# danpovey/quantization

Measured on AMD Instinct MI355X. Metric: vectors encoded/sec at dim=512, 8 codebooks; uint8 codes bit-exact vs ref, higher is better.
Workload: dtype f32 (products: exact 30-bit fixed point on the i8 MFMA); 1 GPU; Quantizer.encode, dim=512, bytes_per_frame=8, codebook_size=256, refine_indexes_iters=5, batch=65536 fp32 Gaussian vectors per GPU (BASELINE.json configs[1]), seeded synthetic codebooks; global_batch=65536, parallelism=batch-sharded x1, no collective

## Files before the change

include/mcq.h:

```cpp
#ifndef MCQ_H
#define MCQ_H

#include <stddef.h>
#include <stdint.h>

#ifdef __cplusplus
extern "C" {
#endif

#define MCQ_EINVAL (-1)
#define MCQ_EUNSUPPORTED (-2)
#define MCQ_EWORKSPACE (-3)

#define MCQ_ABI_VERSION 7
int mcq_abi_version(void);

int mcq_padded_dim(int D);

size_t mcq_prepared_bytes(int N, int K, int D);
size_t mcq_prepared_decode_bytes(int N, int K, int D);
size_t mcq_prepared_mean_offset(int N, int K, int D);
int mcq_prepare(const float *centers, float cscale_exp, const float *weight, const float *bias,
                int N, int K, int D, void *prepared, void *stream);

int mcq_prepare_dev(const float *centers, const float *scales_exp, const float *weight, const float *bias,
                    int N, int K, int D, void *prepared, void *stream);

int mcq_prepare_params(const float *centers, const float *centers_scale, const float *logits_scale, float speed,
                       const float *weight, const float *bias, int N, int K, int D, void *prepared,
                       float *scales_exp_out, void *stream);

size_t mcq_encode_workspace_bytes(long B, int N, int K, int D);
int mcq_encode(const float *x, long B, const void *prepared, float lscale_exp, int N, int K, int D,
               int refine_iters, uint8_t *out_u8, int64_t *out_i64, void *workspace,
               size_t workspace_bytes, void *stream);

#define MCQ_ENCODE_SKIP_FIXED_POINTS 1u
#define MCQ_ENCODE_LSCALE_FROM_PREPARED 2u
#define MCQ_ENCODE_X_FP16 4u
int mcq_encode_ex(const float *x, long B, const void *prepared, float lscale_exp, int N, int K, int D,
                  int refine_iters, uint8_t *out_u8, int64_t *out_i64, void *workspace,
                  size_t workspace_bytes, void *stream, unsigned flags);

int mcq_refine_indexes(const float *x, long B, const void *prepared, int N, int K, int D, int refine_iters,
                       const int64_t *idx_in, int64_t *idx_out, void *workspace, size_t workspace_bytes,
                       void *stream);

int mcq_decode(const void *codes, int code_bytes, int codes_per_row, long B, const void *prepared,
               int N, int K, int D, float *out, void *stream);

int mcq_decode_backward(const float *grad_out, const int64_t *idx, long B, int N, int K, int D, float *gC,
                        void *stream);

int mcq_logits_argmax(const float *x, long B, const void *prepared, float lscale_exp, int N, int K, int D,
                      float *logits_out, int64_t *argmax_out, void *workspace, size_t workspace_bytes,
                      void *stream, unsigned flags);

int mcq_logits_refine(const float *x, long B, const void *prepared, float lscale_exp, int N, int K, int D,
                      int refine_iters, float *logits_out, int64_t *idx_out, void *workspace, size_t workspace_bytes,
                      void *stream, unsigned flags);
int mcq_logits_refine_codes(const float *x, long B, const void *prepared, float lscale_exp, int N, int K, int D,
                            int refine_iters, float *logits_out, int64_t *idx_out, uint8_t *codes_out, void *workspace,
                            size_t workspace_bytes, void *stream, unsigned flags);

size_t mcq_loss_workspace_bytes(long B, int N, int K);
int mcq_loss_fwd(const float *logits, const int64_t *idx, long B, int N, int K, float *lse, float *chosen_sum,
                 float *prob_sum, float *count, void *workspace, size_t workspace_bytes, void *stream);

int mcq_loss_bwd(const float *logits, const int64_t *idx, const float *lse, long B, int N, int K,
                 const float *g_chosen, const float *g_prob, float *grad_logits, void *stream);

int mcq_loss_tail(const float *sums, const float *prob_sum, const float *count, int N, int K, float entropy_scale,
                  float *losses, float *g, float *g_prob, void *stream);

int mcq_recon_fwd(const float *x, const int64_t *idx, long B, const void *prepared, const float *mean, int N,
                  int K, int D, float *err, float *num_part, float *den_part, void *stream);


size_t mcq_weight_grad_workspace_bytes(long B, int M, int D);
int mcq_weight_grad(const float *G, const float *x, long B, int M, int D, const float *scale_dev, float *gW, float *gb,
                    void *workspace, size_t workspace_bytes, void *stream);
int mcq_adam_step(float *p, const float *g, float *m, float *v, long n, double lr, double beta1, double beta2, double eps,
                  double weight_decay, double bias_correction1, double bias_correction2_sqrt, void *stream);
int mcq_loss_head(const float *num_part, const float *den_part, long nparts, const float *chosen_n, int N, float batch,
                  float *head, void *stream);
int mcq_scales_exp(const float *centers_scale, const float *logits_scale, float speed, float *out2, void *stream);
int mcq_loss_head_tail(const float *num_part, const float *den_part, long nparts, const float *chosen_n, int N, float batch,
                       float *head, const float *prob_sum, const float *count, int K, float entropy_scale, float *losses,
                       float *g, float *g_prob, void *stream);

long mcq_decode_backward_waves(int N, int K, int D);
int mcq_decode_backward_u8_ex(const float *grad_out, const uint8_t *codes, long B, int N, int K, int D, float *gC,
                              const float *sa, const float *sb, float sc, const float *dotw, float *dot_part, void *stream);
long mcq_loss_bwd_waves(long B, int N, int K);
int mcq_loss_bwd_ex(const float *logits, const int64_t *idx, const float *lse, long B, int N, int K, const float *g_chosen,
                    const float *g_prob, float *grad_logits, const float *bias, float *dot_part, void *stream);
int mcq_grad_tail(const float *part_c, long n_c, const float *sa, const float *sb, float sc, const float *part_l, long n_l,
                  float speed, float *out_c, float *out_l, void *stream);

int mcq_jcl_prefix_fwd(const float *hp, const float *emb, const int64_t *idx, long B, int N, int K, int H,
                       float scale, float *A, void *stream);
int mcq_jcl_prefix_bwd(const float *A, const float *gA, long B, int N, int H, float scale, float *g_hp, float *gE,
                       void *stream);
int mcq_scatter_rows(const float *grad, long stride_b, long stride_n, const int64_t *idx, int idx_stride, long B,
                     int N, int K, int D, float *out, void *stream);

int mcq_decode_backward_u8(const float *grad_out, const uint8_t *codes, long B, int N, int K, int D, float *gC,
                           void *stream);

size_t mcq_logits_workspace_bytes(long B, int N, int D);
int mcq_logits(const float *x, long B, const void *prepared, float lscale_exp, int N, int K, int D,
               float *out, void *workspace, size_t workspace_bytes, void *stream);

int mcq_test_select(const float *scores, int cases, int per_lane, int cnt, float *out_v, int *out_p, void *stream);

int mcq_last_encode_launches(void);

int mcq_profile_encode(const float *x, long B, const void *prepared, float lscale_exp, int N, int K,
                       int D, int refine_iters, void *workspace, size_t workspace_bytes, void *stream,
                       float *ms_out, int *launches_out, int cap);
// ... 7 lines not shown
```

quantization_amd/_lib.py:

```python
import ctypes
import os

_HERE = os.path.dirname(os.path.abspath(__file__))
_ALT = os.environ.get("MCQ_LIB_PATH") if os.environ.get("MCQ_ALLOW_LIB_PATH") == "1" else None
LIB_PATH = _ALT or os.path.join(_HERE, "lib", "libmcq_hip.so")

SYMBOLS = (
    "mcq_abi_version", "mcq_padded_dim", "mcq_prepared_bytes", "mcq_prepared_decode_bytes", "mcq_prepared_mean_offset", "mcq_prepare", "mcq_prepare_dev", "mcq_prepare_params", "mcq_encode_workspace_bytes",
    "mcq_encode", "mcq_encode_ex", "mcq_refine_indexes", "mcq_decode", "mcq_decode_backward", "mcq_logits", "mcq_logits_workspace_bytes", "mcq_last_encode_launches", "mcq_test_select", "mcq_profile_encode", "mcq_profile_category_name",
    "mcq_logits_argmax", "mcq_logits_refine", "mcq_logits_refine_codes", "mcq_loss_workspace_bytes", "mcq_loss_fwd", "mcq_loss_bwd", "mcq_recon_fwd", "mcq_loss_tail",
    "mcq_jcl_prefix_fwd", "mcq_jcl_prefix_bwd", "mcq_scatter_rows", "mcq_decode_backward_u8",
    "mcq_weight_grad", "mcq_weight_grad_workspace_bytes", "mcq_adam_step", "mcq_loss_head", "mcq_loss_head_tail", "mcq_scales_exp",
    "mcq_decode_backward_waves", "mcq_decode_backward_u8_ex", "mcq_loss_bwd_waves", "mcq_loss_bwd_ex", "mcq_grad_tail",
)

MCQ_EINVAL, MCQ_EUNSUPPORTED, MCQ_EWORKSPACE = -1, -2, -3
_lib = None


class McqError(RuntimeError):
    pass


def lib():
    global _lib
    if _lib is not None:
        return _lib
    if not os.path.exists(LIB_PATH):
        raise McqError(f"{LIB_PATH} is missing: build it with `python -c 'import __graft_entry__ as g; g.build()'` "
                       "(hipcc --offload-arch=gfx950); quantization_amd has no CPU fallback")
    L = ctypes.CDLL(LIB_PATH)
    vp, f32, i32, i64, sz = ctypes.c_void_p, ctypes.c_float, ctypes.c_int, ctypes.c_long, ctypes.c_size_t
    L.mcq_abi_version.restype = i32
    L.mcq_padded_dim.restype = i32
    L.mcq_padded_dim.argtypes = [i32]
    L.mcq_prepared_bytes.restype = sz
    L.mcq_prepared_bytes.argtypes = [i32, i32, i32]
    L.mcq_prepared_decode_bytes.restype = sz
    L.mcq_prepared_decode_bytes.argtypes = [i32, i32, i32]
    L.mcq_prepare.restype = i32
    L.mcq_prepare.argtypes = [vp, f32, vp, vp, i32, i32, i32, vp, vp]
    L.mcq_prepare_dev.restype = i32
    L.mcq_prepare_dev.argtypes = [vp, vp, vp, vp, i32, i32, i32, vp, vp]
    L.mcq_prepare_params.restype = i32
    L.mcq_prepare_params.argtypes = [vp, vp, vp, f32, vp, vp, i32, i32, i32, vp, vp, vp]
    L.mcq_prepared_mean_offset.restype = sz
    L.mcq_prepared_mean_offset.argtypes = [i32, i32, i32]
    L.mcq_encode_workspace_bytes.restype = sz
    L.mcq_encode_workspace_bytes.argtypes = [i64, i32, i32, i32]
    L.mcq_encode.restype = i32
    L.mcq_encode.argtypes = [vp, i64, vp, f32, i32, i32, i32, i32, vp, vp, vp, sz, vp]
    L.mcq_encode_ex.restype = i32
    L.mcq_encode_ex.argtypes = [vp, i64, vp, f32, i32, i32, i32, i32, vp, vp, vp, sz, vp, ctypes.c_uint]
    L.mcq_refine_indexes.restype = i32
    L.mcq_refine_indexes.argtypes = [vp, i64, vp, i32, i32, i32, i32, vp, vp, vp, sz, vp]
    L.mcq_decode.restype = i32
    L.mcq_decode.argtypes = [vp, i32, i32, i64, vp, i32, i32, i32, vp, vp]
    L.mcq_decode_backward.restype = i32
    L.mcq_decode_backward.argtypes = [vp, vp, i64, i32, i32, i32, vp, vp]
    L.mcq_logits.restype = i32
    L.mcq_logits.argtypes = [vp, i64, vp, f32, i32, i32, i32, vp, vp, sz, vp]
    L.mcq_test_select.restype = i32
    L.mcq_test_select.argtypes = [vp, i32, i32, i32, vp, vp, vp]
    L.mcq_logits_workspace_bytes.restype = sz
    L.mcq_logits_workspace_bytes.argtypes = [i64, i32, i32]
    L.mcq_logits_argmax.restype = i32
    L.mcq_logits_argmax.argtypes = [vp, i64, vp, f32, i32, i32, i32, vp, vp, vp, sz, vp, ctypes.c_uint]
    L.mcq_logits_refine.restype = i32
    L.mcq_logits_refine.argtypes = [vp, i64, vp, f32, i32, i32, i32, i32, vp, vp, vp, sz, vp, ctypes.c_uint]
    L.mcq_logits_refine_codes.restype = i32
    L.mcq_logits_refine_codes.argtypes = [vp, i64, vp, f32, i32, i32, i32, i32, vp, vp, vp, vp, sz, vp, ctypes.c_uint]
    L.mcq_loss_workspace_bytes.restype = sz
    L.mcq_loss_workspace_bytes.argtypes = [i64, i32, i32]
    L.mcq_loss_fwd.restype = i32
    L.mcq_loss_fwd.argtypes = [vp, vp, i64, i32, i32, vp, vp, vp, vp, vp, sz, vp]
    L.mcq_loss_bwd.restype = i32
    L.mcq_loss_bwd.argtypes = [vp, vp, vp, i64, i32, i32, vp, vp, vp, vp]
    L.mcq_loss_tail.restype = i32
    L.mcq_loss_tail.argtypes = [vp, vp, vp, i32, i32, f32, vp, vp, vp, vp]
    L.mcq_recon_fwd.restype = i32
    L.mcq_recon_fwd.argtypes = [vp, vp, i64, vp, vp, i32, i32, i32, vp, vp, vp, vp]
    L.mcq_jcl_prefix_fwd.restype = i32
    L.mcq_jcl_prefix_fwd.argtypes = [vp, vp, vp, i64, i32, i32, i32, f32, vp, vp]
    L.mcq_jcl_prefix_bwd.restype = i32
    L.mcq_jcl_prefix_bwd.argtypes = [vp, vp, i64, i32, i32, f32, vp, vp, vp]
    L.mcq_decode_backward_u8.restype = i32
    L.mcq_decode_backward_u8.argtypes = [vp, vp, i64, i32, i32, i32, vp, vp]
    L.mcq_scatter_rows.restype = i32
    L.mcq_scatter_rows.argtypes = [vp, i64, i64, vp, i32, i64, i32, i32, i32, vp, vp]
    L.mcq_weight_grad.restype = i32
    L.mcq_weight_grad.argtypes = [vp, vp, i64, i32, i32, vp, vp, vp, vp, sz, vp]
    L.mcq_weight_grad_workspace_bytes.restype = sz
    L.mcq_weight_grad_workspace_bytes.argtypes = [i64, i32, i32]
    f64 = ctypes.c_double
    L.mcq_adam_step.restype = i32
    L.mcq_adam_step.argtypes = [vp, vp, vp, vp, i64, f64, f64, f64, f64, f64, f64, f64, vp]
    L.mcq_loss_head.restype = i32
    L.mcq_loss_head.argtypes = [vp, vp, i64, vp, i32, f32, vp, vp]
    L.mcq_loss_head_tail.restype = i32
# ... 30 lines not shown
```

quantization_amd/csrc/mcq_api.hip:

```cpp
#include "../../include/mcq.h"
#include "mcq_kernels.h"
#include "mcq_fix_kernels.h"
#include "mcq_loss_kernels.h"
#include "mcq_tf_kernels.h"
#include "mcq_pass16_kernels.h"
#include "mcq_train_kernels.h"

#include <cstdlib>
#include <vector>

using namespace mcq;

namespace {

inline int round_up16(int d) { return (d + 15) & ~15; }
inline size_t align256(size_t v) { return (v + 255) & ~size_t(255); }
inline bool is_pow2(int v) { return v > 0 && (v & (v - 1)) == 0; }

int k_cutoff(int K, int L) {
    int kc = (K <= 16) ? 8 : 16;
    while (L >= 4) { L /= 4; kc *= 2; }
    return kc < 128 ? kc : 128;
}

struct Prepared {
    const float *C, *Q, *bias, *scales, *G, *mean, *wmu;
    const int8_t *Cf, *Wf;
    const int *Ce, *We;
};

struct PreparedLayout {
    size_t offC, offQ, offCf, offCe, offWf, offWe, offWmu, offBias, offScales, offMean, offCMean, offG, total;
};

PreparedLayout prepared_layout(int N, int K, int D) {
    const size_t nk = (size_t)N * K, Dp = round_up16(D);
    const size_t planes = fix_plane_bytes((long)nk, D), exps = (size_t)fix_round_rows((long)nk) * 4;
    PreparedLayout l;
    l.offC = 0;
    l.offQ = align256(l.offC + nk * Dp * 4);
    l.offCf = align256(l.offQ + nk * 4);
    l.offCe = align256(l.offCf + planes);
    l.offWf = align256(l.offCe + exps);
    l.offWe = align256(l.offWf + planes);
    l.offWmu = align256(l.offWe + exps);
    l.offBias = align256(l.offWmu + nk * 4);
    l.offScales = align256(l.offBias + nk * 4);
    l.offMean = align256(l.offScales + 8);
    l.offCMean = align256(l.offMean + Dp * 4);
    l.offG = align256(l.offCMean + (size_t)N * Dp * 4);
    l.total = align256(l.offG + nk * nk * 4);
    static_assert(kFixTile == 128, "");
    if (l.total < l.offBias + (nk + kFixTile) * 4) l.total = align256(l.offBias + (nk + kFixTile) * 4);
    return l;
}

Prepared prepared_view(const void *p, int N, int K, int D) {
    const PreparedLayout l = prepared_layout(N, K, D);
    const char *b = static_cast<const char *>(p);
    return Prepared{reinterpret_cast<const float *>(b + l.offC), reinterpret_cast<const float *>(b + l.offQ),
                    reinterpret_cast<const float *>(b + l.offBias), reinterpret_cast<const float *>(b + l.offScales),
                    reinterpret_cast<const float *>(b + l.offG), reinterpret_cast<const float *>(b + l.offMean),
                    reinterpret_cast<const float *>(b + l.offWmu),
                    reinterpret_cast<const int8_t *>(b + l.offCf), reinterpret_cast<const int8_t *>(b + l.offWf),
                    reinterpret_cast<const int *>(b + l.offCe), reinterpret_cast<const int *>(b + l.offWe)};
}

template <typename CT>
struct WorkspaceT {
    CT *idx, *idxB, *idxC, *final_idx;
    int *map[2], *cnt;
    float *E, *R, *xx, *XC;
    float *gterms;
    int8_t *xf;
    int *xe;
    float *tabs[2];
    TfLists tf;
};

int tf_levels(int N) { int v = 0; while ((1 << v) < N) ++v; return v; }

size_t tf_tab_floats(int N, int K) {
    const int nlev = tf_levels(N);
    size_t best = 0;
    for (int v = 2; v < nlev; ++v) {
        const size_t groups = (size_t)N >> (v + 1);
        for (int u = 1; u < v; ++u) {
            const size_t per = (size_t)1 << (v - u), kc = k_cutoff(K, 1 << u);
            const size_t f = groups * per * per * kc * kc;
            best = f > best ? f : best;
        }
    }
    return best;
}

inline size_t code_bytes_of(int K) { return K > 256 ? 2 : 1; }

size_t workspace_per_vector(int N, int K, int D) {
    const size_t cb = code_bytes_of(K);
    return 4 * cb * (size_t)N + 8 + 8 + 4 * (size_t)N + 4 * (size_t)N * K + (size_t)tf_levels(N) * N * (16 * cb + 2 * 16 + 4 * 16) + 64 +
           2 * 4 * tf_tab_floats(N, K) + 4 * (size_t)fix_round_cols(D) + 4 + 4 * (size_t)N * N;
}
size_t workspace_slack(int D) { return 48 * 256 + (size_t)kFixTile * (4 * (size_t)fix_round_cols(D) + 4); }

long default_chunk(int N, int K, int D) {
    long c = (long)(((size_t)2 << 30) / workspace_per_vector(N, K, D));
    c = c > 65536 ? 65536 : c;
    c = c < 1024 ? 1024 : c;
    return c & ~127L;
}

template <typename CT>
WorkspaceT<CT> carve(void *ws, long Bc, int N, int K, int D) {
    char *p = static_cast<char *>(ws);
    size_t off = 0;
    auto take = [&](size_t bytes) { char *q = p + off; off = align256(off + bytes); return q; };
    WorkspaceT<CT> w;
    w.idx = reinterpret_cast<CT *>(take((size_t)Bc * N * sizeof(CT)));
    w.idxB = reinterpret_cast<CT *>(take((size_t)Bc * N * sizeof(CT)));
    w.idxC = reinterpret_cast<CT *>(take((size_t)Bc * N * sizeof(CT)));
    w.final_idx = reinterpret_cast<CT *>(take((size_t)Bc * N * sizeof(CT)));
    for (int i = 0; i < 2; ++i) w.map[i] = reinterpret_cast<int *>(take((size_t)Bc * 4));
    w.cnt = reinterpret_cast<int *>(take(64 * 4));
    w.E = reinterpret_cast<float *>(take((size_t)Bc * 4));
    w.R = reinterpret_cast<float *>(take((size_t)Bc * N * 4));
    w.xx = reinterpret_cast<float *>(take((size_t)Bc * 4));
    w.gterms = reinterpret_cast<float *>(take((size_t)Bc * N * N * 4));
    w.XC = reinterpret_cast<float *>(take((size_t)Bc * N * K * 4));
    w.xf = reinterpret_cast<int8_t *>(take(fix_plane_bytes(Bc, D)));
    w.xe = reinterpret_cast<int *>(take((size_t)fix_round_rows(Bc) * 4));
    const int nlev = tf_levels(N);
    w.tf.ent = nullptr;
    w.tf.out_i64 = nullptr;
    w.tf.out_u8 = nullptr;
    w.tf.erG = w.tf.erXC = w.tf.erxx = nullptr;
    w.tf.erE = w.tf.erR = nullptr;
    w.tf.erK = 0;
    for (int v = 0; v < kTfLevels; ++v) {
        w.tf.kc[v] = k_cutoff(K, 1 << v);
        w.tf.pos[v] = nullptr;
        w.tf.S[v] = nullptr;
        if (v >= nlev) continue;
        const int kc = w.tf.kc[v];
        if (v == 0) w.tf.ent = reinterpret_cast<uint8_t *>(take((size_t)Bc * N * kc * sizeof(CT)));
        else w.tf.pos[v] = reinterpret_cast<uint8_t *>(take((size_t)Bc * (N >> v) * kc * 2));
        w.tf.S[v] = reinterpret_cast<float *>(take((size_t)Bc * (N >> v) * kc * 4));
    }
    const size_t tf = tf_tab_floats(N, K);
    for (int i = 0; i < 2; ++i) w.tabs[i] = tf ? reinterpret_cast<float *>(take((size_t)Bc * tf * 4)) : nullptr;
    return w;
}

bool domain_ok(int N, int K, int D) {
    return is_pow2(K) && K >= 16 && K <= 1024 && is_pow2(N) && N <= 64 && (long)N * K <= 16384 && D >= 1 && D <= 16384;
}
int domain_err(int N, int K, int D = 1) {
    return (K < 16 || K > 1024 || N > 64 || (long)N * K > 16384 || D > 16384) ? MCQ_EUNSUPPORTED : MCQ_EINVAL;
}

struct Prof {
    hipStream_t stream;
    int only = -1;
    std::vector<hipEvent_t> ev;
    std::vector<int> cat, first, last;
    int open = -1;
    void begin(int category) {
        if (only >= 0 && category != only) { open = -1; return; }
        if (ev.empty() || open != (int)ev.size() - 1) {
            hipEvent_t e;
            (void)hipEventCreate(&e);
            (void)hipEventRecord(e, stream);
            ev.push_back(e);
        }
        open = (int)ev.size() - 1;
    }
    void untimed() { open = -1; }
    void end(int category) {
        if (only >= 0 && category != only) { open = -1; return; }
        hipEvent_t e;
        (void)hipEventCreate(&e);
        (void)hipEventRecord(e, stream);
        ev.push_back(e);
        first.push_back(open);
        last.push_back((int)ev.size() - 1);
        cat.push_back(category);
        open = (int)ev.size() - 1;
    }
};

thread_local int g_last_launches = 0;

#define MCQ_LAUNCH_CHECK()                               \
    do {                                                 \
        hipError_t e_ = hipGetLastError();               \
        if (e_ != hipSuccess) return (int)e_;            \
        ++g_last_launches;                               \
    } while (0)

FixRowsArgs fix_rows_args(const float *src, int xh, long R, int D, long ld, int8_t *planes, int *exps, float *xx,
                          const float *bias_src = nullptr, float *bias_dst = nullptr, const float *sub = nullptr,
                          long sub_per = 0, long sub_ld = 0, const float *dot_vec = nullptr, float *dot_out = nullptr) {
    return FixRowsArgs{src, xh, R, fix_round_rows(R), D, ld, fix_round_cols(D), planes, exps, xx, bias_src, bias_dst,
                       sub, sub_per, sub_ld, dot_vec, dot_out};
}

int launch_fix_rows(const float *src, int xh, long R, int D, long ld, int8_t *planes, int *exps, float *xx, hipStream_t st,
                    const float *sub = nullptr) {
    const FixRowsArgs a = fix_rows_args(src, xh, R, D, ld, planes, exps, xx, nullptr, nullptr, sub, 0, 0);
    hipLaunchKernelGGL(k_fix_rows<4>, dim3((unsigned)(a.Rp / 4)), dim3(256), 0, st, a);
    MCQ_LAUNCH_CHECK();
    return 0;
}

int launch_fix_rows2(const FixRowsArgs &a, const FixRowsArgs &b, hipStream_t st) {
    const unsigned na = (unsigned)(a.Rp / 4), nb = (unsigned)(b.Rp / 4);
    hipLaunchKernelGGL(k_fix_rows2<4>, dim3(na + nb), dim3(256), 0, st, a, b, na);
    MCQ_LAUNCH_CHECK();
    return 0;
}

template <int MODE>
int launch_fgemm(FixGemm g, hipStream_t st) {
    static bool allowed[64] = {};
    int dev = 0;
    if (hipGetDevice(&dev) != hipSuccess || dev < 0 || dev >= 64) dev = 63;
    if (!allowed[dev] || dev == 63) {
        const hipError_t attr = hipFuncSetAttribute(reinterpret_cast<const void *>(&k_fgemm<MODE>),
                                                    hipFuncAttributeMaxDynamicSharedMemorySize, kFixLds);
        if (attr != hipSuccess) return (int)attr;
        allowed[dev] = true;
    }
    const long MT = g.RA / kFixTile, NT = g.RB / kFixTile;
    const int H = (MODE == FG_LOGITS && g.K > kFixTile) ? g.K / kFixTile : 1;
    const long big = g.walk_rows ? NT : MT, small_units = (g.walk_rows ? MT : NT) / H;
    long units = (big + 7) / 8 * small_units;
    if (units > 32) units = 32;
    hipLaunchKernelGGL((k_fgemm<MODE>), dim3((unsigned)(8 * units)), dim3(512), kFixLds, st, g);
    MCQ_LAUNCH_CHECK();
    return 0;
}

int launch_xc(const int8_t *xf, const int *xe, long B, const int8_t *Cf, const int *Ce, long nk, int D, float *out,
              hipStream_t st) {
    FixGemm g{};
    g.A = xf; g.ea = xe; g.RA = fix_round_rows(B); g.M = B;
    g.B = Cf; g.eb = Ce; g.RB = fix_round_rows(nk); g.N = nk;
    g.Dq = fix_round_cols(D);
    g.walk_rows = 0;
    g.out = out; g.ldo = nk;
    return launch_fgemm<FG_STORE>(g, st);
}

int launch_logits(const int8_t *xf, const int *xe, long B, const Prepared &P, int N, int K, int D, float lscale,
                  const float *lscale_ptr, float *logits, void *idx, hipStream_t st) {
    const long nk = (long)N * K;
    FixGemm g{};
    g.A = P.Wf; g.ea = P.We; g.RA = fix_round_rows(nk); g.M = nk;
    g.B = xf; g.eb = xe; g.RB = fix_round_rows(B); g.N = B;
    g.Dq = fix_round_cols(D);
    g.walk_rows = 1;
    g.bias = P.bias; g.wmu = P.wmu; g.lscale = lscale; g.lscale_ptr = lscale_ptr;
    g.logits = logits; g.ldo = nk; g.idx = idx; g.idx_wide = K > 256 ? 1 : 0; g.K = K; g.ncb = N;
    return launch_fgemm<FG_LOGITS>(g, st);
}

template <int K>
int launch_tf_stage0_k(int N, const float *G, const float *XC, const tf_code_of<K> *idx, const float *R, const float *Q, long B,
                       int keep, tf_code_of<K> *ent, float *S, tf_code_of<K> *fin, const int *nact, const int *map, hipStream_t st) {
    const dim3 grid((unsigned)(((B + 3) / 4) * N)), block(256);
#define MCQ_S0_CASE(NN) \
    case NN: hipLaunchKernelGGL((k_tf_stage0<K, NN>), grid, block, 0, st, G, XC, idx, R, Q, B, keep, ent, S, fin, nact, map); break;
    switch (N) {
        MCQ_S0_CASE(1) MCQ_S0_CASE(2) MCQ_S0_CASE(4) MCQ_S0_CASE(8) MCQ_S0_CASE(16) MCQ_S0_CASE(32) MCQ_S0_CASE(64)
        default: return MCQ_EUNSUPPORTED;
    }
#undef MCQ_S0_CASE
    MCQ_LAUNCH_CHECK();
    return 0;
}

int launch_tf_stage0(int K, int N, const float *G, const float *XC, const uint16_t *idx, const float *R, const float *Q,
                     long B, int keep, uint16_t *ent, float *S, uint16_t *fin, const int *nact, const int *map, hipStream_t st) {
    switch (K) {
        case 512: return launch_tf_stage0_k<512>(N, G, XC, idx, R, Q, B, keep, ent, S, fin, nact, map, st);
        case 1024: return launch_tf_stage0_k<1024>(N, G, XC, idx, R, Q, B, keep, ent, S, fin, nact, map, st);
        default: return MCQ_EUNSUPPORTED;
    }
}

int launch_tf_stage0(int K, int N, const float *G, const float *XC, const uint8_t *idx, const float *R, const float *Q,
                     long B, int keep, uint8_t *ent, float *S, uint8_t *fin, const int *nact, const int *map, hipStream_t st) {
    if (K == 16 && N >= 4 && keep <= 16) {
        const dim3 grid((unsigned)((B * (N / 4) + 3) / 4)), block(256);
#define MCQ_S16_CASE(NN) \
    case NN: hipLaunchKernelGGL((k_tf_stage0_k16<NN>), grid, block, 0, st, G, XC, idx, R, Q, B, keep, ent, S, nact, map); break;
        switch (N) {
            MCQ_S16_CASE(4) MCQ_S16_CASE(8) MCQ_S16_CASE(16) MCQ_S16_CASE(32) MCQ_S16_CASE(64)
            default: return MCQ_EUNSUPPORTED;
        }
#undef MCQ_S16_CASE
        MCQ_LAUNCH_CHECK();
        return 0;
    }
    switch (K) {
        case 16: return launch_tf_stage0_k<16>(N, G, XC, idx, R, Q, B, keep, ent, S, fin, nact, map, st);
        case 32: return launch_tf_stage0_k<32>(N, G, XC, idx, R, Q, B, keep, ent, S, fin, nact, map, st);
        case 64: return launch_tf_stage0_k<64>(N, G, XC, idx, R, Q, B, keep, ent, S, fin, nact, map, st);
        case 128: return launch_tf_stage0_k<128>(N, G, XC, idx, R, Q, B, keep, ent, S, fin, nact, map, st);
        case 256: return launch_tf_stage0_k<256>(N, G, XC, idx, R, Q, B, keep, ent, S, fin, nact, map, st);
        default: return MCQ_EUNSUPPORTED;
    }
}

template <typename CT>
int launch_tf_er(int N, const float *G, const float *XC, const CT *idx, const float *xx, long B, int K, float *E, float *R,
                 float *gterms, const int *nact, const int *map, hipStream_t st) {
    const dim3 grid((unsigned)((B + 3) / 4)), block(256);
    const bool direct = B <= 8192;
#define MCQ_ER_CASE(NN)                                                                                                  \
    case NN:                                                                                                             \
        if (!direct) {                                                                                                   \
            hipLaunchKernelGGL((k_tf_gram_terms<NN, CT>), dim3((unsigned)(((B + 4 * (64 / NN) - 1) / (4 * (64 / NN))) * NN)), block, 0, st, G, idx, \
                               B, K, gterms, nact);                                                                      \
            MCQ_LAUNCH_CHECK();                                                                                          \
        }                                                                                                                \
        hipLaunchKernelGGL((k_tf_er<NN, CT>), grid, block, 0, st, gterms, XC, idx, xx, B, K, E, R, nact, map,              \
                           direct ? G : static_cast<const float *>(nullptr));                                           \
        break;
    switch (N) {
        MCQ_ER_CASE(1) MCQ_ER_CASE(2) MCQ_ER_CASE(4) MCQ_ER_CASE(8) MCQ_ER_CASE(16) MCQ_ER_CASE(32) MCQ_ER_CASE(64)
        default: return MCQ_EUNSUPPORTED;
    }
#undef MCQ_ER_CASE
    MCQ_LAUNCH_CHECK();
    return 0;
}

int launch_tf_up(int kh, int kc, const TfLists &L, long B, int N, int u, int ntab, int per, const float *in, float *out,
                 const int *nact, hipStream_t st) {
    const dim3 grid((unsigned)(B * ntab)), block(64);
#define MCQ_UP_CASE(A, C) \
    if (kh == A && kc == C) { hipLaunchKernelGGL((k_tf_up<A, C>), grid, block, 0, st, L, B, N, u, ntab, per, in, out, nact); MCQ_LAUNCH_CHECK(); return 0; }
    MCQ_UP_CASE(16, 32) MCQ_UP_CASE(32, 32) MCQ_UP_CASE(32, 64) MCQ_UP_CASE(8, 16) MCQ_UP_CASE(16, 16)
#undef MCQ_UP_CASE
    return MCQ_EUNSUPPORTED;
}

template <typename CT>
int launch_tf_comb(int kh, int kc, const float *E, const TfLists &L, long B, int N, int v, int keep, const float *tabs,
                   CT *fin, const int *nact, hipStream_t st) {
    const dim3 grid((unsigned)(B * (N >> (v + 1)))), block(64);
#define MCQ_COMB_CASE(A, C)                                                                                                        \
    if (kh == A && kc == C) {                                                                                                     \
        if (fin) hipLaunchKernelGGL((k_tf_comb<A, C, true, CT>), grid, block, 0, st, E, L, B, N, v, keep, tabs, fin, nact);       \
        else hipLaunchKernelGGL((k_tf_comb<A, C, false, CT>), grid, block, 0, st, E, L, B, N, v, keep, tabs, fin, nact);          \
        MCQ_LAUNCH_CHECK();                                                                                                       \
        return 0;                                                                                                                 \
    }
    MCQ_COMB_CASE(16, 32) MCQ_COMB_CASE(32, 32) MCQ_COMB_CASE(32, 64) MCQ_COMB_CASE(64, 64)
    if constexpr (sizeof(CT) == 1) { MCQ_COMB_CASE(8, 16) MCQ_COMB_CASE(16, 16) }
#undef MCQ_COMB_CASE
    return MCQ_EUNSUPPORTED;
}

enum { CAT_LOGITS = 0, CAT_XX = 1, CAT_STAGE0 = 2, CAT_XC = 3, CAT_LEVEL0 = 4, CAT_LEVEL1 = 5, CAT_TABLES = 6, CAT_COMBINE = 7,
       CAT_TABLES_UP = 8, CAT_COMBINE_UP = 9, CAT_ER = 10, CAT_LEVEL1_FUSED = 11, CAT_TAIL = 12, CAT_COUNT = 13 };
const char *const kCatNames[CAT_COUNT] = {
    "logits_product_argmax",
    "frames_to_limbs",
    "stage0_tables",
    "xc_product",
    "combine_level0",
    "combine_level1",
    "tables_level1",
    "combine_level2",
    "tables_upper_levels",
    "combine_upper_levels",
    "residual_energies",
    "level1_combines_and_tables",
    "encode_tail",
};

#define MCQ_TF_LAUNCH2(SMALLK, BIGK, grid, block, ...)                                                       \
    do {                                                                                                     \
        bool s_ = false;                                                                                     \
        if constexpr (sizeof(CT) == 1) {                                                                     \
            if (small) { hipLaunchKernelGGL(SMALLK, grid, block, 0, st, __VA_ARGS__); s_ = true; }           \
        }                                                                                                    \
        if (!s_) hipLaunchKernelGGL(BIGK, grid, block, 0, st, __VA_ARGS__);                                  \
    } while (0)
inline bool pass16_enabled() {
    static const bool on = !(getenv("MCQ_PASS16") && atoi(getenv("MCQ_PASS16")) == 0);
    return on;
}

template <typename CT>
int run_tf_combines(const float *G, const CT *idx_cur, CT *idx_new, const WorkspaceT<CT> &w, const TfLists &L, long B, int N,
                    int K, const int *nact, hipStream_t st, Prof *prof) {
    const bool small = (K == 16);
    const int nlev = tf_levels(N);
    {
        const int keep = (N == 2) ? 1 : L.kc[1];
        CT *fin = (N == 2) ? idx_new : nullptr;
        const dim3 grid((unsigned)(B * (N / 2)));
        if (prof) prof->begin(CAT_LEVEL0);
        bool done0 = false;
        if constexpr (sizeof(CT) == 1) {
            if (!small) {
                hipLaunchKernelGGL(k_tf_pair0s, grid, dim3(64), 0, st, G, idx_cur, w.E, L, B, N, K, keep, fin, nact);
                done0 = true;
            }
        }
        if (!done0) MCQ_TF_LAUNCH2((k_tf_pair0<8, CT>), (k_tf_pair0<16, CT>), grid, dim3(64), G, idx_cur, w.E, L, B, N, K, keep, fin, nact);
        MCQ_LAUNCH_CHECK();
        if (prof) prof->end(CAT_LEVEL0);
    }
    const bool fuse_l1 = (N >= 8);
    const bool fuse_l3 = fuse_l1 && N == 16 && small;
    if (fuse_l1) {
        const int keep = L.kc[2];
        const int groups2 = N >> 3, per1 = 2, ntab1 = groups2 * per1 * per1;
        const unsigned pair_blocks = (unsigned)(B * (N / 4)), tab_blocks = (unsigned)(B * ntab1);
        const int ntab3 = fuse_l3 ? 16 : 1, per3 = fuse_l3 ? 4 : 1;
        const dim3 grid(pair_blocks + tab_blocks + (fuse_l3 ? (unsigned)(B * ntab3) : 0u));
        if (prof) prof->begin(CAT_LEVEL1_FUSED);
        MCQ_TF_LAUNCH2((k_tf_level1<8, 8, CT>), (k_tf_level1<16, 16, CT>), grid, dim3(64), G, idx_cur, w.E, L, B, N, K, keep, ntab1, per1, w.tabs[0],
                       nact, pair_blocks, tab_blocks, ntab3, per3, w.tabs[1]);
        MCQ_LAUNCH_CHECK();
        if (prof) prof->end(CAT_LEVEL1_FUSED);
    } else if (N >= 4) {
        const int keep = (N == 4) ? 1 : L.kc[2];
        CT *fin = (N == 4) ? idx_new : nullptr;
        const dim3 grid((unsigned)(B * (N / 4)));
        if (prof) prof->begin(CAT_LEVEL1);
        MCQ_TF_LAUNCH2((k_tf_pair1<8, 8, CT>), (k_tf_pair1<16, 16, CT>), grid, dim3(64), G, idx_cur, w.E, L, B, N, K, keep, fin, nact);
        MCQ_LAUNCH_CHECK();
        if (prof) prof->end(CAT_LEVEL1);
    }
    for (int v = 2; v < nlev; ++v) {
        const int groups = N >> (v + 1);
        const bool last = (v == nlev - 1);
        const int keep = last ? 1 : L.kc[v + 1];
        CT *fin = last ? idx_new : nullptr;
        const int per1 = 1 << (v - 1), ntab1 = groups * per1 * per1;
        const int cat_tab = (v == 2) ? CAT_TABLES : CAT_TABLES_UP, cat_comb = (v == 2) ? CAT_COMBINE : CAT_COMBINE_UP;
        if (!(fuse_l1 && v == 2) && !(fuse_l3 && v == 3)) {
            if (prof) prof->begin(cat_tab);
            MCQ_TF_LAUNCH2((k_tf_table1<8, 8, CT>), (k_tf_table1<16, 16, CT>), dim3((unsigned)(B * ntab1)), dim3(64), G, idx_cur, L, B, N, K, ntab1, per1,
                           w.tabs[0], nact);
            MCQ_LAUNCH_CHECK();
            if (prof) prof->end(cat_tab);
        }
        if (N == 16 && v == 3) {
            if (prof) prof->begin(cat_comb);
            const float *t3 = fuse_l3 ? w.tabs[1] : w.tabs[0];
            MCQ_TF_LAUNCH2((k_tf_comb3<8, 16, 16, CT>), (k_tf_comb3<16, 32, 32, CT>), dim3((unsigned)B), dim3(256), idx_cur, w.E, L, B, N, t3, idx_new, nact);
            MCQ_LAUNCH_CHECK();
            if (prof) prof->end(cat_comb);
            continue;
        }
        int cur = 0;
        for (int u = 2; u < v; ++u) {
            const int per = 1 << (v - u), ntab = groups * per * per;
            if (prof) prof->begin(cat_tab);
            const int rc = launch_tf_up(L.kc[u - 1], L.kc[u], L, B, N, u, ntab, per, w.tabs[cur], w.tabs[cur ^ 1], nact, st);
            if (rc) return rc;
            if (prof) prof->end(cat_tab);
            cur ^= 1;
        }
        if (prof) prof->begin(cat_comb);
        const int rc = launch_tf_comb<CT>(L.kc[v - 1], L.kc[v], w.E, L, B, N, v, keep, w.tabs[cur], fin, nact, st);
        if (rc) return rc;
        if (prof) prof->end(cat_comb);
    }
    return 0;
}
#undef MCQ_TF_LAUNCH2

template <typename CT>
int run_encode_t(const float *x, long B, const void *prepared, float lscale, int N, int K, int D, int iters,
                 uint8_t *out_u8, int64_t *out_i64, void *workspace, size_t workspace_bytes, hipStream_t st,
                 Prof *prof, const int64_t *init_idx, unsigned flags, float *logits_out,
                 uint8_t *codes_also ) {
    g_last_launches = 0;
    if (!domain_ok(N, K, D)) return domain_err(N, K, D);
    if (B < 0 || iters < 0 || iters > 60 || (out_u8 == nullptr) == (out_i64 == nullptr)) return MCQ_EINVAL;
    if (sizeof(CT) > 1 && (out_u8 != nullptr || codes_also != nullptr)) return MCQ_EINVAL;
    if (B == 0) return 0;
    if (!x || !prepared || !workspace) return MCQ_EINVAL;
    const size_t per = workspace_per_vector(N, K, D), slack = workspace_slack(D);
    if (workspace_bytes < slack + per) return MCQ_EWORKSPACE;
    long chunk = (long)((workspace_bytes - slack) / per);
    if (chunk > B) chunk = B;
    if (chunk < B && chunk < 128) return MCQ_EWORKSPACE;
    if (chunk < B) chunk &= ~127L;
    const Prepared P = prepared_view(prepared, N, K, D);
    const int pack = (out_u8 != nullptr && K == 16 && N >= 2) ? 2 : 1;
    const bool skip = (flags & MCQ_ENCODE_SKIP_FIXED_POINTS) != 0 && iters >= 2;

    for (long lo = 0; lo < B; lo += chunk) {
        const long Bc = (B - lo < chunk) ? (B - lo) : chunk;
        const WorkspaceT<CT> w = carve<CT>(workspace, Bc, N, K, D);
        const int xh = (flags & MCQ_ENCODE_X_FP16) ? 1 : 0;
        const float *xc = xh ? reinterpret_cast<const float *>(reinterpret_cast<const uint16_t *>(x) + lo * D) : x + lo * D;
        int rc;
        if (init_idx == nullptr || iters > 0) {
            if (prof) prof->begin(CAT_XX);
            rc = launch_fix_rows(xc, xh, Bc, D, D, w.xf, w.xe, w.xx, st, P.mean);
            if (rc) return rc;
            if (prof) prof->end(CAT_XX);
        }
        if (init_idx != nullptr) {
            hipLaunchKernelGGL(k_import_indexes<CT>, dim3((unsigned)((Bc * N + 255) / 256)), dim3(256), 0, st,
                               init_idx + lo * N, Bc * N, K, w.idx);
            MCQ_LAUNCH_CHECK();
            if (prof) prof->untimed();
        } else {
            if (prof) prof->begin(CAT_LOGITS);
            rc = launch_logits(w.xf, w.xe, Bc, P, N, K, D, lscale,
                               (flags & MCQ_ENCODE_LSCALE_FROM_PREPARED) ? P.scales + 1 : nullptr,
                               logits_out ? logits_out + lo * N * K : nullptr, w.idx, st);
            if (rc) return rc;
            if (prof) prof->end(CAT_LOGITS);
        }
        if (iters > 0) {
            if (prof) prof->begin(CAT_XC);
            rc = launch_xc(w.xf, w.xe, Bc, P.Cf, P.Ce, (long)N * K, D, w.XC, st);
            if (rc) return rc;
            if (prof) prof->end(CAT_XC);
        }
        int iters_left = iters;
        CT *idx_cur = w.idx, *idx_new = skip ? w.idxB : w.idx, *idx_pk = w.idxC;
        const int *map_cur = nullptr, *nact = nullptr;
        int *map_nxt = w.map[0], *map_spare = w.map[1];
        if (skip) {
            hipError_t e = hipMemsetAsync(w.cnt, 0, 64 * sizeof(int), st);
            if (e != hipSuccess) return (int)e;
            if (prof) prof->untimed();
        }
        bool wrote_direct = false;
        if constexpr (sizeof(CT) == 1) {
            if (K == 16 && (N == 16 || N == 8) && iters > 0 && !skip && prof == nullptr && pass16_enabled()) {
                static bool allowed16[64] = {};
                int dev = 0;
                if (hipGetDevice(&dev) != hipSuccess || dev < 0 || dev >= 64) dev = 63;
                if (!allowed16[dev] || dev == 63) {
                    hipError_t attr = hipFuncSetAttribute(reinterpret_cast<const void *>(&k_tf_pass16<16>),
                                                          hipFuncAttributeMaxDynamicSharedMemorySize, p16_lds_bytes<16>());
                    if (attr == hipSuccess)
                        attr = hipFuncSetAttribute(reinterpret_cast<const void *>(&k_tf_pass16<8>),
                                                   hipFuncAttributeMaxDynamicSharedMemorySize, p16_lds_bytes<8>());
                    if (attr != hipSuccess) return (int)attr;
                    allowed16[dev] = true;
                }
                Pass16Args a;
                a.G = P.G; a.XC = w.XC; a.xx = w.xx; a.Q = P.Q; a.idx = w.idx; a.B = Bc; a.iters = iters;
                const bool direct_out = pack == 1;
                a.out_i64 = (direct_out && out_i64) ? out_i64 + lo * N : nullptr;
                a.out_u8 = direct_out ? (out_u8 ? out_u8 + lo * N : (codes_also ? codes_also + lo * N : nullptr)) : nullptr;
                const long wgs = (Bc + kP16Waves - 1) / kP16Waves;
                if (N == 16)
                    hipLaunchKernelGGL(k_tf_pass16<16>, dim3((unsigned)(wgs < 256 ? wgs : 256)), dim3(64 * kP16Waves), p16_lds_bytes<16>(), st, a);
                else
                    hipLaunchKernelGGL(k_tf_pass16<8>, dim3((unsigned)(wgs < 512 ? wgs : 512)), dim3(64 * kP16Waves), p16_lds_bytes<8>(), st, a);
                MCQ_LAUNCH_CHECK();
                if (direct_out) continue;
                iters_left = 0;
            }
        }
        const bool er_in_emit = !skip && (N == 4 || N == 8 || N == 16);
        bool er_ready = false;
        for (int it = 0; it < iters_left; ++it) {
            if (!er_ready) {
                if (prof) prof->begin(CAT_ER);
                rc = launch_tf_er<CT>(N, P.G, w.XC, idx_cur, w.xx, Bc, K, w.E, w.R, w.gterms, nact, map_cur, st);
                if (rc) return rc;
                if (prof) prof->end(CAT_ER);
            }
            er_ready = false;
            if (prof) prof->begin(CAT_STAGE0);
            rc = launch_tf_stage0(K, N, P.G, w.XC, idx_cur, w.R, P.Q, Bc, (N == 1) ? 1 : w.tf.kc[0], reinterpret_cast<CT *>(w.tf.ent),
                                  w.tf.S[0], (N == 1) ? idx_new : static_cast<CT *>(nullptr), nact, map_cur, st);
            if (rc) return rc;
            if (prof) prof->end(CAT_STAGE0);
            if (N >= 2) {
                TfLists L = w.tf;
                if (er_in_emit && it + 1 < iters) {
                    L.erG = P.G; L.erXC = w.XC; L.erxx = w.xx; L.erE = w.E; L.erR = w.R; L.erK = K;
                    er_ready = true;
                }
                const bool direct_out = (it + 1 == iters) && !skip && pack == 1;
                if (direct_out) {
                    L.out_i64 = out_i64 ? out_i64 + lo * N : nullptr;
                    L.out_u8 = out_u8 ? out_u8 + lo * N : (codes_also ? codes_also + lo * N : nullptr);
                    wrote_direct = true;
                }
                rc = run_tf_combines<CT>(P.G, idx_cur, idx_new, w, L, Bc, N, K, nact, st, prof);
                if (rc) return rc;
            }
            if (skip) {
                const int last = (it + 1 == iters) ? 1 : 0;
                if (prof) prof->begin(CAT_TAIL);
                hipLaunchKernelGGL(k_compact<CT>, dim3((unsigned)((Bc + 255) / 256)), dim3(256), 0, st, idx_cur, idx_new,
                                   map_cur, nact, Bc, N, last, w.final_idx, idx_pk, map_nxt, w.cnt + it);
                MCQ_LAUNCH_CHECK();
                if (prof) prof->end(CAT_TAIL);
                CT *t = idx_cur; idx_cur = idx_pk; idx_pk = t;
                int *old_map = const_cast<int *>(map_cur);
                map_cur = map_nxt;
                map_nxt = old_map ? old_map : map_spare;
                nact = w.cnt + it;
            }
        }
        if (wrote_direct) continue;
        const CT *result = (skip && iters > 0) ? w.final_idx : w.idx;
        const long outn = (out_i64 != nullptr) ? Bc * N : Bc * (N / pack);
        if (prof) prof->begin(CAT_TAIL);
        hipLaunchKernelGGL(k_finalize<CT>, dim3((unsigned)((outn + 255) / 256)), dim3(256), 0, st, result, Bc, N, pack,
                           out_u8 ? out_u8 + lo * (N / pack) : nullptr, out_i64 ? out_i64 + lo * N : nullptr,
                           codes_also ? codes_also + lo * N : nullptr);
        MCQ_LAUNCH_CHECK();
        if (prof) prof->end(CAT_TAIL);
    }
    return 0;
}

int run_encode(const float *x, long B, const void *prepared, float lscale, int N, int K, int D, int iters,
               uint8_t *out_u8, int64_t *out_i64, void *workspace, size_t workspace_bytes, hipStream_t st,
               Prof *prof, const int64_t *init_idx = nullptr, unsigned flags = 0, float *logits_out = nullptr,
               uint8_t *codes_also = nullptr) {
    if (K > 256)
        return run_encode_t<uint16_t>(x, B, prepared, lscale, N, K, D, iters, out_u8, out_i64, workspace, workspace_bytes, st, prof,
                                      init_idx, flags, logits_out, codes_also);
    return run_encode_t<uint8_t>(x, B, prepared, lscale, N, K, D, iters, out_u8, out_i64, workspace, workspace_bytes, st, prof,
                                 init_idx, flags, logits_out, codes_also);
}

int db_cw_of(int D, int K) {
    if ((D & 3) != 0) return 1;
    if (K >= 64) return 4;
    return D >= 1024 ? 4 : (D >= 512 ? 2 : 1);
}
int db_cw(const void *g, const void *out, int D, int K, long gsb, long gsn, const void *dotw = nullptr) {
    const bool al = ((D & 3) == 0) && ((gsb & 3) == 0) && ((gsn & 3) == 0) && ((reinterpret_cast<uintptr_t>(g) & 15) == 0) &&
                    ((reinterpret_cast<uintptr_t>(out) & 15) == 0) && ((reinterpret_cast<uintptr_t>(dotw) & 15) == 0);
    return al ? db_cw_of(D, K) : 1;
}
int db_chunks(int D, int cw) { return (D + 64 * cw - 1) / (64 * cw); }

template <typename IdxT>
int launch_decode_backward(const float *g, const IdxT *idx, long B, int N, int K, int D, float *out, long gsb, long gsn,
                           int idx_stride, hipStream_t st, const float *sa = nullptr, const float *sb = nullptr, float sc = 1.0f,
                           const float *dotw = nullptr, float *dot_part = nullptr) {
    const int cw = db_cw(g, out, D, K, gsb, gsn, dotw), chunks = db_chunks(D, cw);
    const long rowgroups = ((long)N * K + 3) / 4;
    long blocks;
    if (chunks <= 8 && (8 % chunks) == 0) blocks = ((rowgroups + (8 / chunks) - 1) / (8 / chunks)) * 8;
    else blocks = ((long)N * K * chunks + 3) / 4;
    const dim3 grid((unsigned)blocks), block(256);
    if (cw == 4) hipLaunchKernelGGL((k_decode_backward<IdxT, 4>), grid, block, 0, st, g, idx, B, N, K, D, chunks, out, gsb, gsn, idx_stride, sa, sb, sc, dotw, dot_part);
    else if (cw == 2) hipLaunchKernelGGL((k_decode_backward<IdxT, 2>), grid, block, 0, st, g, idx, B, N, K, D, chunks, out, gsb, gsn, idx_stride, sa, sb, sc, dotw, dot_part);
    else hipLaunchKernelGGL((k_decode_backward<IdxT, 1>), grid, block, 0, st, g, idx, B, N, K, D, chunks, out, gsb, gsn, idx_stride, sa, sb, sc, dotw, dot_part);
    hipError_t e = hipGetLastError();
    return e == hipSuccess ? 0 : (int)e;
}
}

extern "C" {

int mcq_abi_version(void) { return MCQ_ABI_VERSION; }

int mcq_padded_dim(int D) { return round_up16(D); }

size_t mcq_prepared_bytes(int N, int K, int D) {
    if (N <= 0 || K <= 0 || D <= 0) return 0;
    return prepared_layout(N, K, D).total;
}

static int prepare_impl(const float *centers, float cscale_exp, const float *scales_dev, const float *weight,
                        const float *bias, int N, int K, int D, void *prepared, void *stream, const float *raw_cs = nullptr,
                        const float *raw_ls = nullptr, float speed = 0.f, float *scales_out2 = nullptr) {
    if (!domain_ok(N, K, D)) return domain_err(N, K, D);
    if (!centers || !prepared || ((weight == nullptr) != (bias == nullptr))) return MCQ_EINVAL;
    hipStream_t st = static_cast<hipStream_t>(stream);
    const PreparedLayout l = prepared_layout(N, K, D);
    char *b = static_cast<char *>(prepared);
    const long rows = (long)N * K;
    const int Dp = round_up16(D);
    const unsigned grid = (unsigned)((rows + 3) / 4);
    hipLaunchKernelGGL(k_prepare_rows, dim3(grid), dim3(256), 0, st, centers, cscale_exp, 1, rows, D, Dp,
                       reinterpret_cast<float *>(b + l.offC), static_cast<float *>(nullptr) , scales_dev,
                       (scales_dev || raw_cs) ? reinterpret_cast<float *>(b + l.offScales) : static_cast<float *>(nullptr), raw_cs,
                       raw_ls, speed, scales_out2);
    hipError_t e = hipGetLastError();
    if (e != hipSuccess) return (int)e;
    if (!weight) return 0;
    const float *C = reinterpret_cast<const float *>(b + l.offC);
    float *cmean = reinterpret_cast<float *>(b + l.offCMean);
    hipLaunchKernelGGL(k_centers_mean, dim3((unsigned)(Dp / 16)), dim3(1024), 0, st, C, N, K, Dp,
                       reinterpret_cast<float *>(b + l.offMean), cmean);
    e = hipGetLastError();
// ... 232 lines not shown
    if (B == 0) return 0;
    if (!A || !gA || !g_hp || !gE) return MCQ_EINVAL;
    hipLaunchKernelGGL(k_jcl_prefix_bwd, dim3((unsigned)((B + 3) / 4)), dim3(256), 0, static_cast<hipStream_t>(stream), A,
                       gA, B, N, H, scale, g_hp, gE);
    hipError_t e = hipGetLastError();
    return e == hipSuccess ? 0 : (int)e;
}

namespace {
struct LogitsWs {
    uint8_t *idx8;
    int8_t *xf;
    int *xe;
    size_t total;
};
LogitsWs logits_ws(void *ws, long B, int N, int D) {
    char *p = static_cast<char *>(ws);
    LogitsWs w;
    size_t off = 0;
    w.idx8 = reinterpret_cast<uint8_t *>(p + off);
    off = align256(off + (size_t)B * N);
    w.xf = reinterpret_cast<int8_t *>(p + off);
    off = align256(off + fix_plane_bytes(B, D));
    w.xe = reinterpret_cast<int *>(p + off);
    off = align256(off + (size_t)fix_round_rows(B) * 4);
    w.total = off;
    return w;
}
}

size_t mcq_logits_workspace_bytes(long B, int N, int D) {
    if (B <= 0 || N <= 0 || D <= 0) return 256;
    return logits_ws(nullptr, B, N, D).total;
}

int mcq_logits(const float *x, long B, const void *prepared, float lscale_exp, int N, int K, int D, float *out,
               void *workspace, size_t workspace_bytes, void *stream) {
    if (!domain_ok(N, K, D)) return MCQ_EUNSUPPORTED;
    if (B == 0) return 0;
    if (!x || !prepared || !out || B < 0 || !workspace) return MCQ_EINVAL;
    if (workspace_bytes < mcq_logits_workspace_bytes(B, N, D)) return MCQ_EWORKSPACE;
    hipStream_t st = static_cast<hipStream_t>(stream);
    const Prepared P = prepared_view(prepared, N, K, D);
    const LogitsWs w = logits_ws(workspace, B, N, D);
    int rc = launch_fix_rows(x, 0, B, D, D, w.xf, w.xe, nullptr, st, P.mean);
    if (rc) return rc;
    return launch_logits(w.xf, w.xe, B, P, N, K, D, lscale_exp, nullptr, out, nullptr, st);
}

int mcq_logits_argmax(const float *x, long B, const void *prepared, float lscale_exp, int N, int K, int D,
                      float *logits_out, int64_t *argmax_out, void *workspace, size_t workspace_bytes, void *stream,
                      unsigned flags) {
    if (!domain_ok(N, K, D) || K > 256) return MCQ_EUNSUPPORTED;
    if (B < 0) return MCQ_EINVAL;
    if (B == 0) return 0;
    if (!x || !prepared || !logits_out || !argmax_out || !workspace) return MCQ_EINVAL;
    if (workspace_bytes < mcq_logits_workspace_bytes(B, N, D)) return MCQ_EWORKSPACE;
    hipStream_t st = static_cast<hipStream_t>(stream);
    const Prepared P = prepared_view(prepared, N, K, D);
    const LogitsWs w = logits_ws(workspace, B, N, D);
    int rc = launch_fix_rows(x, (flags & MCQ_ENCODE_X_FP16) ? 1 : 0, B, D, D, w.xf, w.xe, nullptr, st, P.mean);
    if (rc) return rc;
    rc = launch_logits(w.xf, w.xe, B, P, N, K, D, lscale_exp,
                       (flags & MCQ_ENCODE_LSCALE_FROM_PREPARED) ? P.scales + 1 : nullptr, logits_out, w.idx8, st);
    if (rc) return rc;
    hipLaunchKernelGGL(k_export_indexes, dim3((unsigned)((B * N + 255) / 256)), dim3(256), 0, st, w.idx8, B * N, argmax_out);
    MCQ_LAUNCH_CHECK();
    return 0;
}

int mcq_logits_refine(const float *x, long B, const void *prepared, float lscale_exp, int N, int K, int D, int refine_iters,
                      float *logits_out, int64_t *idx_out, void *workspace, size_t workspace_bytes, void *stream,
                      unsigned flags) {
    return mcq_logits_refine_codes(x, B, prepared, lscale_exp, N, K, D, refine_iters, logits_out, idx_out, nullptr, workspace,
                                   workspace_bytes, stream, flags);
}

int mcq_logits_refine_codes(const float *x, long B, const void *prepared, float lscale_exp, int N, int K, int D, int refine_iters,
                            float *logits_out, int64_t *idx_out, uint8_t *codes_out, void *workspace, size_t workspace_bytes,
                            void *stream, unsigned flags) {
    if (K > 256) return MCQ_EUNSUPPORTED;
    if (B > 0 && (!logits_out || !idx_out)) return MCQ_EINVAL;
    return run_encode(x, B, prepared, lscale_exp, N, K, D, refine_iters, nullptr, idx_out, workspace, workspace_bytes,
                      static_cast<hipStream_t>(stream), nullptr, nullptr, flags & ~MCQ_ENCODE_SKIP_FIXED_POINTS, logits_out,
                      codes_out);
}

namespace {
long loss_rows_per_chunk(long B) {
    long r = (B + 1023) / 1024;
    r = r < 64 ? 64 : r;
    return (r + 15) / 16 * 16;
}
long loss_chunks(long B) { const long r = loss_rows_per_chunk(B); return (B + r - 1) / r; }
}

size_t mcq_loss_workspace_bytes(long B, int N, int K) {
    if (B <= 0) return 256;
    return (size_t)loss_chunks(B) * N * (2 * (size_t)K + 1) * sizeof(float) + 256;
}

int mcq_loss_fwd(const float *logits, const int64_t *idx, long B, int N, int K, float *lse, float *chosen_sum,
                 float *prob_sum, float *count, void *workspace, size_t workspace_bytes, void *stream) {
    if (!is_pow2(K) || K < 16 || K > 256 || N < 1) return MCQ_EUNSUPPORTED;
    if (B <= 0) return MCQ_EINVAL;
    if (!logits || !idx || !lse || !chosen_sum || !prob_sum || !count || !workspace) return MCQ_EINVAL;
    if (workspace_bytes < mcq_loss_workspace_bytes(B, N, K)) return MCQ_EWORKSPACE;
    hipStream_t st = static_cast<hipStream_t>(stream);
    const long rpc = loss_rows_per_chunk(B), chunks = loss_chunks(B);
    float *pp = static_cast<float *>(workspace);
    float *pc = pp + chunks * N * K;
    float *ph = pc + chunks * N * K;
    const dim3 grid((unsigned)(chunks * N)), block(64 * kLossWaves);
#define MCQ_LOSS_CASE(KK)                                                                                             \
    case KK: hipLaunchKernelGGL((k_loss_fwd<KK>), grid, block, 0, st, logits, idx, B, N, rpc, lse, pp, pc, ph); break;
    switch (K) {
        MCQ_LOSS_CASE(16) MCQ_LOSS_CASE(32) MCQ_LOSS_CASE(64) MCQ_LOSS_CASE(128) MCQ_LOSS_CASE(256)
        default: return MCQ_EUNSUPPORTED;
    }
#undef MCQ_LOSS_CASE
    MCQ_LAUNCH_CHECK();
    hipLaunchKernelGGL(k_loss_reduce, dim3((unsigned)N), dim3(256), 0, st, pp, pc, ph, chunks, N, K, prob_sum, count,
                       chosen_sum);
    MCQ_LAUNCH_CHECK();
    return 0;
}

int mcq_loss_bwd(const float *logits, const int64_t *idx, const float *lse, long B, int N, int K, const float *g_chosen,
                 const float *g_prob, float *grad_logits, void *stream) {
    if (!is_pow2(K) || K < 16 || K > 256 || N < 1) return MCQ_EUNSUPPORTED;
    if (B <= 0) return MCQ_EINVAL;
    if (!logits || !idx || !lse || !g_chosen || !g_prob || !grad_logits) return MCQ_EINVAL;
    hipStream_t st = static_cast<hipStream_t>(stream);
    const int rpw = K < 64 ? 64 / K : 1;
    const long rows = B * N;
    const dim3 grid((unsigned)((rows + (long)kLossWaves * rpw - 1) / ((long)kLossWaves * rpw))), block(64 * kLossWaves);
#define MCQ_LOSS_CASE(KK)                                                                                             \
    case KK: hipLaunchKernelGGL((k_loss_bwd<KK>), grid, block, 0, st, logits, idx, lse, B, N, g_chosen, g_prob, grad_logits); break;
    switch (K) {
        MCQ_LOSS_CASE(16) MCQ_LOSS_CASE(32) MCQ_LOSS_CASE(64) MCQ_LOSS_CASE(128) MCQ_LOSS_CASE(256)
        default: return MCQ_EUNSUPPORTED;
    }
#undef MCQ_LOSS_CASE
    MCQ_LAUNCH_CHECK();
    return 0;
}

int mcq_loss_tail(const float *sums, const float *prob_sum, const float *count, int N, int K, float entropy_scale,
                  float *losses, float *g, float *g_prob, void *stream) {
    if (!is_pow2(K) || K < 16 || K > 256 || N < 1) return MCQ_EUNSUPPORTED;
    if (!sums || !prob_sum || !count || !losses || !g || !g_prob) return MCQ_EINVAL;
    hipLaunchKernelGGL(k_loss_tail, dim3(1), dim3(256), 0, static_cast<hipStream_t>(stream), sums, prob_sum, count, N, K,
                       entropy_scale, losses, g, g_prob);
    MCQ_LAUNCH_CHECK();
    return 0;
}

int mcq_recon_fwd(const float *x, const int64_t *idx, long B, const void *prepared, const float *mean, int N, int K,
                  int D, float *err, float *num_part, float *den_part, void *stream) {
    if (!domain_ok(N, K, D) || K > 256) return MCQ_EUNSUPPORTED;
    if (B <= 0) return MCQ_EINVAL;
    if (!x || !idx || !prepared || !mean || !err || !num_part || !den_part) return MCQ_EINVAL;
    const Prepared P = prepared_view(prepared, N, K, D);
    hipLaunchKernelGGL(k_recon_fwd, dim3((unsigned)((B + 3) / 4)), dim3(256), 0, static_cast<hipStream_t>(stream), x, idx, B,
                       P.C, mean, N, K, D, round_up16(D), err, num_part, den_part);
    MCQ_LAUNCH_CHECK();
    return 0;
// ... 117 lines not shown
int mcq_loss_bwd_ex(const float *logits, const int64_t *idx, const float *lse, long B, int N, int K, const float *g_chosen,
                    const float *g_prob, float *grad_logits, const float *bias, float *dot_part, void *stream) {
    if (!is_pow2(K) || K < 16 || K > 256 || N < 1) return MCQ_EUNSUPPORTED;
    if (B <= 0) return MCQ_EINVAL;
    if (!logits || !idx || !lse || !g_chosen || !g_prob || !grad_logits || !bias || !dot_part) return MCQ_EINVAL;
    hipStream_t st = static_cast<hipStream_t>(stream);
    const int rpw = K < 64 ? 64 / K : 1;
    const long rows = B * N;
    const dim3 grid((unsigned)((rows + (long)kLossWaves * rpw - 1) / ((long)kLossWaves * rpw))), block(64 * kLossWaves);
#define MCQ_LOSS_CASE(KK)                                                                                             \
    case KK: hipLaunchKernelGGL((k_loss_bwd<KK>), grid, block, 0, st, logits, idx, lse, B, N, g_chosen, g_prob, grad_logits, bias, dot_part); break;
    switch (K) {
        MCQ_LOSS_CASE(16) MCQ_LOSS_CASE(32) MCQ_LOSS_CASE(64) MCQ_LOSS_CASE(128) MCQ_LOSS_CASE(256)
        default: return MCQ_EUNSUPPORTED;
    }
#undef MCQ_LOSS_CASE
    MCQ_LAUNCH_CHECK();
    return 0;
}

int mcq_grad_tail(const float *part_c, long n_c, const float *sa, const float *sb, float sc, const float *part_l, long n_l,
                  float speed, float *out_c, float *out_l, void *stream) {
    if (n_c < 0 || n_l < 0 || (n_c > 0 && !part_c) || (n_l > 0 && !part_l)) return MCQ_EINVAL;
    hipLaunchKernelGGL(k_grad_tail, dim3(1), dim3(1024), 0, static_cast<hipStream_t>(stream), part_c, n_c, sa, sb, sc, part_l, n_l,
                       speed, out_c, out_l);
    MCQ_LAUNCH_CHECK();
    return 0;
}

int mcq_last_encode_launches(void) { return g_last_launches; }

int mcq_test_select(const float *scores, int cases, int per_lane, int cnt, float *out_v, int *out_p, void *stream) {
    if (!scores || !out_v || !out_p || cases <= 0 || cnt < 1 || cnt > 64) return MCQ_EINVAL;
    hipStream_t st = static_cast<hipStream_t>(stream);
    switch (per_lane) {
        case 1: hipLaunchKernelGGL((k_test_select<1>), dim3(cases), dim3(64), 0, st, scores, cnt, out_v, out_p); break;
        case 4: hipLaunchKernelGGL((k_test_select<4>), dim3(cases), dim3(64), 0, st, scores, cnt, out_v, out_p); break;
        case 16: hipLaunchKernelGGL((k_test_select<16>), dim3(cases), dim3(64), 0, st, scores, cnt, out_v, out_p); break;
        case -4: hipLaunchKernelGGL((k_test_select<4, kSlotMajor>), dim3(cases), dim3(64), 0, st, scores, cnt, out_v, out_p); break;
        case -16: hipLaunchKernelGGL((k_test_select<16, kSlotMajor>), dim3(cases), dim3(64), 0, st, scores, cnt, out_v, out_p); break;
        case -1004: hipLaunchKernelGGL((k_test_select<4, kAnyOrder>), dim3(cases), dim3(64), 0, st, scores, cnt, out_v, out_p); break;
        default: return MCQ_EINVAL;
    }
    hipError_t e = hipGetLastError();
    return e == hipSuccess ? 0 : (int)e;
}

#ifdef MCQ_STAMPS
int mcq_debug_stamps(unsigned long long *host_dst, long count, int clear) {
    const long total = (long)kStampKernels * kStampWaves * kStampSlots;
    if (count > total) count = total;
    if (hipDeviceSynchronize() != hipSuccess) return MCQ_EINVAL;
    if (host_dst && count > 0 &&
        hipMemcpyFromSymbol(host_dst, HIP_SYMBOL(g_stamps), (size_t)count * 8, 0, hipMemcpyDeviceToHost) != hipSuccess) return MCQ_EINVAL;
    if (clear) {
        void *p = nullptr;
        if (hipGetSymbolAddress(&p, HIP_SYMBOL(g_stamps)) != hipSuccess || hipMemset(p, 0, (size_t)total * 8) != hipSuccess) return MCQ_EINVAL;
    }
    return (int)kStampSlots;
}
#endif

const char *mcq_profile_category_name(int category) {
    return (category >= 0 && category < CAT_COUNT) ? kCatNames[category] : nullptr;
}

int mcq_profile_encode(const float *x, long B, const void *prepared, float lscale_exp, int N, int K, int D,
                       int refine_iters, void *workspace, size_t workspace_bytes, void *stream, float *ms_out,
                       int *launches_out, int cap) {
    hipStream_t st = static_cast<hipStream_t>(stream);
    const bool wide = K > 256;
    const size_t need = (size_t)B * N * (wide ? 8 : 1);
    uint8_t *dummy = nullptr;
    if (!ms_out || cap <= 0) return MCQ_EINVAL;
    const hipError_t me = hipMalloc(reinterpret_cast<void **>(&dummy), need ? need : 1);
    if (me != hipSuccess) return (int)me;
    for (int i = 0; i < cap; ++i) { ms_out[i] = 0.f; if (launches_out) launches_out[i] = 0; }
    int rc = 0;
    for (int only = 0; only < CAT_COUNT && rc == 0; ++only) {
        Prof prof;
        prof.stream = st;
        prof.only = only;
        rc = run_encode(x, B, prepared, lscale_exp, N, K, D, refine_iters, wide ? nullptr : dummy,
                        wide ? reinterpret_cast<int64_t *>(dummy) : nullptr, workspace, workspace_bytes, st, &prof);
        (void)hipStreamSynchronize(st);
        for (size_t i = 0; rc == 0 && i < prof.cat.size(); ++i) {
            float ms = 0.f;
            (void)hipEventElapsedTime(&ms, prof.ev[prof.first[i]], prof.ev[prof.last[i]]);
            if (prof.cat[i] < cap) { ms_out[prof.cat[i]] += ms; if (launches_out) launches_out[prof.cat[i]] += 1; }
        }
        for (hipEvent_t e : prof.ev) (void)hipEventDestroy(e);
    }
    (void)hipFree(dummy);
    return rc == 0 ? CAT_COUNT : rc;
}

}
```

quantization_amd/csrc/mcq_kernels.h:

```cpp
#pragma once
#include <hip/hip_runtime.h>
#include <stdint.h>
#include <type_traits>

namespace mcq {

typedef float f32x4 __attribute__((ext_vector_type(4)));

constexpr int kWave = 64;
constexpr int kBigPos = 0x7fffffff;

__device__ __forceinline__ int lane_id() { return threadIdx.x & 63; }

__device__ __forceinline__ float wave_sum_butterfly(float p) {
#pragma unroll
    for (int m = 32; m >= 1; m >>= 1) p = p + __shfl_xor(p, m, 64);
    return p;
}

template <int CTRL>
__device__ __forceinline__ float dpp_f(float x) {
    return __int_as_float(__builtin_amdgcn_update_dpp(0, __float_as_int(x), CTRL, 0xf, 0xf, true));
}
template <int CTRL>
// ... 375 lines not shown
    wave_lds_fence();
    out_v = __uint_as_float(ev);
    out_p = (int)ep;
    dst = lane;
    if constexpr (LAYOUT == kAnyOrder) {
        const int mine = has ? out_p : kBigPos;
        int r = 0;
        for (int j = 0; j < nsel; ++j) r += (__builtin_amdgcn_readlane(mine, j) < mine) ? 1 : 0;
        dst = r;
    }
    return nsel;
}

template <int VPL, int LAYOUT = kLaneMajor>
__global__ void __launch_bounds__(64)
k_test_select(const float *__restrict__ scores, int cnt, float *__restrict__ out_v, int *__restrict__ out_p) {
    __shared__ u64 scratch[kSelectLdsU64];
    const float *sc = scores + (size_t)blockIdx.x * 64 * VPL;
    float v[VPL];
    int p[VPL];
#pragma unroll
    for (int i = 0; i < VPL; ++i) {
        p[i] = (LAYOUT == kSlotMajor) ? 64 * i + lane_id() : VPL * lane_id() + i;
        v[i] = sc[p[i]];
    }
    bool has;
    int dst, op;
    float ov;
    const int nsel = wave_select_set<VPL, LAYOUT>(v, p, cnt, 64 * VPL, scratch, has, dst, ov, op);
    if (has) {
        out_v[(size_t)blockIdx.x * 64 + dst] = ov;
        out_p[(size_t)blockIdx.x * 64 + dst] = op;
    }
    if (lane_id() >= nsel && lane_id() < cnt) {
        out_v[(size_t)blockIdx.x * 64 + lane_id()] = INFINITY;
        out_p[(size_t)blockIdx.x * 64 + lane_id()] = 64 * VPL - 1;
    }
}

__global__ void k_prepare_rows(const float *__restrict__ src, float scale, int apply_scale, long rows, int D,
                               int Dp, float *__restrict__ dst, float *__restrict__ Q,
                               const float *__restrict__ scale_ptr ,
                               float *__restrict__ scales_out ,
                               const float *__restrict__ raw_cs = nullptr, const float *__restrict__ raw_ls = nullptr,
                               float speed = 0.f, float *__restrict__ scales_out2 = nullptr) {
    const long row = (long)blockIdx.x * (blockDim.x >> 6) + (threadIdx.x >> 6);
    if (row >= rows) return;
    const int lane = lane_id();
    if (scale_ptr) {
        scale = *scale_ptr;
        if (scales_out && row == 0 && lane < 2) scales_out[lane] = scale_ptr[lane];
    }
    if (raw_cs) {
        scale = expf(*raw_cs * speed);
        if (row == 0 && lane == 0) {
            const float ls = expf(*raw_ls * speed);
            if (scales_out) { scales_out[0] = scale; scales_out[1] = ls; }
            if (scales_out2) { scales_out2[0] = scale; scales_out2[1] = ls; }
        }
    }
    const float *s = src + row * D;
    float *d = dst + row * Dp;
    float part = 0.f;
    for (int q = lane; q < Dp / 4; q += 64) {
        f32x4 o;
#pragma unroll
        for (int c = 0; c < 4; ++c) {
            const int k = 4 * q + c;
            float val = (k < D) ? s[k] : 0.f;
            if (apply_scale) val = scale * val;
            o[c] = val;
            part = fmaf(val, val, part);
        }
        *reinterpret_cast<f32x4 *>(d + 4 * q) = o;
    }
    part = wave_sum_butterfly(part);
    if (Q != nullptr && lane == 0) Q[row] = part;
}


template <typename CT>
__global__ void k_compact(const CT *__restrict__ idx_old, const CT *__restrict__ idx_new,
                          const int *__restrict__ map_cur, const int *__restrict__ nact, long B, int N, int last,
                          CT *__restrict__ final_idx, CT *__restrict__ idx_packed, int *__restrict__ map_next,
                          int *__restrict__ cnt_next) {
    const long s = (long)blockIdx.x * blockDim.x + threadIdx.x;
    if (nact) B = *nact;
    if (s >= B) return;
    const int orig = map_cur ? map_cur[s] : (int)s;
    bool changed = false;
    if (!last)
        for (int n = 0; n < N; ++n) changed = changed || (idx_old[s * N + n] != idx_new[s * N + n]);
    if (changed) {
        const int slot = atomicAdd(cnt_next, 1);
        for (int n = 0; n < N; ++n) idx_packed[(long)slot * N + n] = idx_new[s * N + n];
        map_next[slot] = orig;
    } else {
        for (int n = 0; n < N; ++n) final_idx[(long)orig * N + n] = idx_new[s * N + n];
    }
}

template <typename CT>
__global__ void k_finalize(const CT *__restrict__ idx, long B, int N, int pack, uint8_t *__restrict__ out_u8,
                           int64_t *__restrict__ out_i64, uint8_t *__restrict__ codes_also) {
    const long i = (long)blockIdx.x * blockDim.x + threadIdx.x;
    if (out_i64 != nullptr) {
        if (i < B * N) {
            out_i64[i] = idx[i];
            if (codes_also) codes_also[i] = (uint8_t)idx[i];
        }
    } else {
        const int per = N / pack;
        if (i < B * per) {
            if (pack == 1) out_u8[i] = (uint8_t)idx[i];
            else out_u8[i] = (uint8_t)(idx[2 * i] + 16 * idx[2 * i + 1]);
        }
    }
}

template <typename CT>
__global__ void k_import_indexes(const int64_t *__restrict__ in, long n, int K, CT *__restrict__ out) {
    const long i = (long)blockIdx.x * blockDim.x + threadIdx.x;
    if (i < n) {
        long v = in[i];
        v = v < 0 ? 0 : (v > K - 1 ? K - 1 : v);
        out[i] = (CT)v;
    }
}

template <typename CodeT>
__global__ void k_decode(const CodeT *__restrict__ codes, int per_row, long B, const float *__restrict__ C, int N,
                         int K, int D, int Dp, float *__restrict__ out) {
    const long b = (long)blockIdx.x * (blockDim.x >> 6) + (threadIdx.x >> 6);
    if (b >= B) return;
    const int lane = lane_id();
    const int rep = N / per_row;
    const CodeT *cb = codes + b * per_row;
    float *ob = out + b * D;
    const bool vec_ok = ((D & 3) == 0) && ((reinterpret_cast<uintptr_t>(out) & 15) == 0);
    for (int q = lane; q < Dp / 4; q += 64) {
        f32x4 t = (f32x4){0.f, 0.f, 0.f, 0.f};
        for (int n = 0; n < N; ++n) {
            long code = (long)cb[n / rep];
            int digit = n % rep;
            for (int d = 0; d < digit; ++d) code /= K;
            const int k = (int)(code % K) & (K - 1);
            const f32x4 c = *reinterpret_cast<const f32x4 *>(C + ((long)n * K + k) * Dp + 4 * q);
            t = (n == 0) ? c : t + c;
        }
        if (vec_ok && 4 * q + 3 < D) {
            *reinterpret_cast<f32x4 *>(ob + 4 * q) = t;
        } else {
#pragma unroll
            for (int c = 0; c < 4; ++c)
                if (4 * q + c < D) ob[4 * q + c] = t[c];
        }
    }
}

template <typename CodeT, int CH, int LPV>
__global__ void __launch_bounds__(256)
k_decode_sliced(const CodeT *__restrict__ codes, long B, const float *__restrict__ C, int N, int K, int D, int Dp,
                float *__restrict__ out) {
    constexpr int VPW = 64 / LPV;
    const int slice = blockIdx.x & 7;
    const long vb = blockIdx.x >> 3;
    const int wave = threadIdx.x >> 6, lane = threadIdx.x & 63;
    const int v = lane / LPV, q = lane % LPV;
    const long b = (vb * 4 + wave) * VPW + v;
    const int off = slice * (LPV * 4) + 4 * q;
    if (b >= B || off >= Dp) return;
    const CodeT *cb = codes + b * N;
    const float *Cq = C + off;
    f32x4 t = (f32x4){0.f, 0.f, 0.f, 0.f};
    for (int n0 = 0; n0 < N; n0 += CH) {
        f32x4 rows[CH];
#pragma unroll
        for (int j = 0; j < CH; ++j) {
            const int n = (n0 + j < N) ? n0 + j : N - 1;
            const int k = (int)cb[n] & (K - 1);
            rows[j] = *reinterpret_cast<const f32x4 *>(Cq + ((long)n * K + k) * Dp);
// ... 275 lines not shown
```

quantization_amd/csrc/mcq_pass16_kernels.h:

```cpp
#pragma once
#include "mcq_tf_kernels.h"

namespace mcq {

struct Pass16Args {
    const float *G;
    const float *XC;
    const float *xx;
    const float *Q;
    uint8_t *idx;
    long B;
    int iters;
    int64_t *out_i64;
    uint8_t *out_u8;
};

constexpr int kP16Waves = 8;
template <int N> constexpr int p16_blocks() { return N * (N - 1) / 2; }
template <int N> constexpr int p16_gram_floats() { return p16_blocks<N>() * 256 + 2 * N * 16; }
constexpr int kP16Ent0 = 0;
constexpr int kP16Pos1 = 128;
constexpr int kP16Pos2 = 256;
constexpr int kP16Pos3 = 384;
constexpr int kP16S0 = 512;
// ... 2 lines not shown
constexpr int kP16S3 = 1536;
constexpr int kP16T1 = 1664;
constexpr int kP16T2 = 1952;
constexpr int kP16Sel = 3040;
constexpr int kP16Scratch = 4096;
template <int N> constexpr int p16_lds_bytes() { return p16_gram_floats<N>() * 4 + kP16Waves * kP16Scratch; }
static_assert(kP16Sel + kSelectLdsU64 * 8 <= kP16Scratch && kP16T2 + 16 * 17 * 4 <= kP16Sel && kP16T1 + 8 * 9 * 4 <= kP16T2, "");

__device__ __forceinline__ int shfl_i(int v, int src) { return __builtin_amdgcn_ds_bpermute(src << 2, v); }

template <int N>
__device__ __forceinline__ int p16_blk(int n, int m) { return ((n * (2 * N - 1 - n)) / 2 + m - n - 1) * 256; }

template <int N>
__device__ __forceinline__ float p16_g(const float *Gt, int n, int i, int m, int j) {
    const bool lt = n < m;
    const int lo = lt ? n : m, hi = lt ? m : n, a = lt ? i : j, b = lt ? j : i;
    return Gt[p16_blk<N>(lo, hi) + a * 16 + b];
}

__device__ __forceinline__ float p16_leaf(const float *blk, int ea, int eb, int on, int om) {
    const float g = blk[ea * 16 + eb], u = blk[ea * 16 + om], v = blk[on * 16 + eb], w = blk[on * 16 + om];
    return ((g - u) - v) + w;
}

template <int N>
__device__ __forceinline__ float p16_t1(const float *Gt, const uint8_t *ent0, const uint8_t *pos1, int e, int X, int Y, int i, int j) {
    const unsigned pi = *reinterpret_cast<const uint16_t *>(pos1 + (X * 8 + i) * 2), pj = *reinterpret_cast<const uint16_t *>(pos1 + (Y * 8 + j) * 2);
    const int i0 = pi & 0xff, i1 = pi >> 8, j0 = pj & 0xff, j1 = pj >> 8;
    const int ea0 = ent0[(2 * X) * 8 + i0], ea1 = ent0[(2 * X + 1) * 8 + i1], eb0 = ent0[(2 * Y) * 8 + j0], eb1 = ent0[(2 * Y + 1) * 8 + j1];
    const int on0 = __builtin_amdgcn_readlane(e, 2 * X), on1 = __builtin_amdgcn_readlane(e, 2 * X + 1);
    const int om0 = __builtin_amdgcn_readlane(e, 2 * Y), om1 = __builtin_amdgcn_readlane(e, 2 * Y + 1);
    const float d00 = p16_leaf(Gt + p16_blk<N>(2 * X, 2 * Y), ea0, eb0, on0, om0);
    const float d01 = p16_leaf(Gt + p16_blk<N>(2 * X, 2 * Y + 1), ea0, eb1, on0, om1);
    const float d10 = p16_leaf(Gt + p16_blk<N>(2 * X + 1, 2 * Y), ea1, eb0, on1, om0);
    const float d11 = p16_leaf(Gt + p16_blk<N>(2 * X + 1, 2 * Y + 1), ea1, eb1, on1, om1);
    return ((d00 + d01) + d10) + d11;
}

template <int N>
__global__ void __launch_bounds__(64 * kP16Waves)
k_tf_pass16(Pass16Args a) {
    static_assert(N == 16 || N == 8, "");
    constexpr int NK = N * 16, XS = NK / 64, NT = N * N / 64;
    extern __shared__ __attribute__((aligned(16))) float p16_smem[];
    float *Gt = p16_smem;
    float *Gd = Gt + p16_blocks<N>() * 256;
    float *Qs = Gd + NK;
    const int tid = threadIdx.x, lane = tid & 63;
    const int wave = __builtin_amdgcn_readfirstlane(tid >> 6);
    char *ws = reinterpret_cast<char *>(Qs + NK) + wave * kP16Scratch;
    uint8_t *ent0 = reinterpret_cast<uint8_t *>(ws + kP16Ent0), *pos1 = reinterpret_cast<uint8_t *>(ws + kP16Pos1);
    uint8_t *pos2 = reinterpret_cast<uint8_t *>(ws + kP16Pos2), *pos3 = reinterpret_cast<uint8_t *>(ws + kP16Pos3);
    float *S0 = reinterpret_cast<float *>(ws + kP16S0), *S1 = reinterpret_cast<float *>(ws + kP16S1);
    float *S2 = reinterpret_cast<float *>(ws + kP16S2), *S3 = reinterpret_cast<float *>(ws + kP16S3);
    float *T1a = reinterpret_cast<float *>(ws + kP16T1), *T2a = reinterpret_cast<float *>(ws + kP16T2);
    u64 *sel = reinterpret_cast<u64 *>(ws + kP16Sel);

    {
        const unsigned vrow = (unsigned)(lane >> 2), vpart = (unsigned)(lane & 3);
        int cnt = 0;
        for (int n = 0; n < N - 1; ++n)
            for (int m = n + 1; m < N; ++m, ++cnt) {
                if ((cnt & (kP16Waves - 1)) != wave) continue;
                const unsigned go = (((unsigned)(n * 16) + vrow) * (unsigned)NK + (unsigned)(m * 16) + 4u * vpart) * 4u;
                const unsigned d = (unsigned)(size_t)Gt + (unsigned)cnt * 1024u;
                asm volatile("s_mov_b32 m0, %[d]\n\ts_nop 0\n\tglobal_load_lds_dwordx4 %[vo], %[p]" : : [vo] "v"(go), [p] "s"(a.G), [d] "s"(d) : "memory");
            }
        if (tid < NK) {
            Gd[tid] = a.G[(size_t)tid * NK + tid];
            Qs[tid] = a.Q[tid];
        }
        asm volatile("s_waitcnt vmcnt(0)" ::: "memory");
        __syncthreads();
    }

    const int q4 = lane >> 4, k16 = lane & 15;
    for (long b = (long)blockIdx.x * kP16Waves + wave; b < a.B; b += (long)gridDim.x * kP16Waves) {
        float xcv[XS];
#pragma unroll
        for (int r = 0; r < XS; ++r) xcv[r] = a.XC[(size_t)b * NK + 64 * r + lane];
        int e = lane < N ? (int)a.idx[b * N + lane] & 15 : 0;
        const float xxb = a.xx[b];
        for (int pass = 0; pass < a.iters; ++pass) {
            float E, Rv;
            {
                float gt[NT];
#pragma unroll
                for (int j = 0; j < NT; ++j) {
                    const int t = lane + 64 * j, m = t / N, m2 = t % N;
                    const int om = shfl_i(e, m), om2 = shfl_i(e, m2);
                    const bool dg = m == m2;
                    const float gd = Gd[m * 16 + om];
                    const float go = p16_g<N>(Gt, m, om, dg ? (m ^ 1) : m2, om2);
                    gt[j] = dg ? gd : go;
                }
                const int qrow = (lane < N ? lane : 0) * 16 + e;
                float xt = 0.f;
#pragma unroll
                for (int r = 0; r < XS; ++r) {
                    const float v = shfl_f(xcv[r], qrow & 63);
                    xt = ((qrow >> 6) == r) ? v : xt;
                }
                xt = lane < N ? xt : 0.f;
                float gp = gt[0];
#pragma unroll
                for (int j = 1; j < NT; ++j) gp = gp + gt[j];
                const float gsum = wave_sum_butterfly(gp), xsum = wave_sum_butterfly(xt);
                E = (gsum - 2.0f * xsum) + xxb;
                const int n = lane < N ? lane : 0;
                float col = 0.f, gnn = 0.f;
#pragma unroll
                for (int m = 0; m < N; ++m) {
                    const float v = shfl_f(gt[(m * N) / 64], (m * N + n) & 63);
                    col = (m == 0) ? v : col + v;
                    if (m == n) gnn = v;
                }
                const float xo = col - xt;
                Rv = (E - 2.0f * xo) + gnn;
            }
#pragma unroll
            for (int r = 0; r < N / 4; ++r) {
                const int n = 4 * r + q4;
                float t = 0.f;
                bool started = false;
#pragma unroll
                for (int m = 0; m < N; ++m) {
                    const int om = __builtin_amdgcn_readlane(e, m);
                    const bool use = m != n;
                    const float gv = p16_g<N>(Gt, m, om, use ? n : (n ^ 1), k16);
                    const float sum = t + gv;
                    t = use ? (started ? sum : gv) : t;
                    started = started || use;
                }
                const float X = t - xcv[r];
                const float Rn = shfl_f(Rv, n);
                const float sv = (Rn + Qs[64 * r + lane]) + 2.0f * X;
                const uint32_t hi = ord32(sv), lo = (uint32_t)k16;
                const u64 key = ((u64)hi << 32) | lo;
                int rnk = 0;
#define MCQ_ROR(rr)                                                                                                     \
    {                                                                                                                   \
        const u64 o = ((u64)(uint32_t)dpp_i<0x120 + rr>((int)hi) << 32) | (uint32_t)dpp_i<0x120 + rr>((int)lo);         \
        rnk += (o < key) ? 1 : 0;                                                                                       \
    }
                MCQ_ROR(1) MCQ_ROR(2) MCQ_ROR(3) MCQ_ROR(4) MCQ_ROR(5) MCQ_ROR(6) MCQ_ROR(7) MCQ_ROR(8)
                MCQ_ROR(9) MCQ_ROR(10) MCQ_ROR(11) MCQ_ROR(12) MCQ_ROR(13) MCQ_ROR(14) MCQ_ROR(15)
#undef MCQ_ROR
                const bool take = rnk < 8;
                const u64 tm = __ballot(take);
                const uint32_t rowbits = (uint32_t)(tm >> (lane & 48)) & 0xffffu;
                const int dst = __popc(rowbits & ((1u << k16) - 1u));
                if (take) {
                    ent0[n * 8 + dst] = (uint8_t)k16;
                    S0[n * 8 + dst] = sv;
                }
            }
            wave_lds_fence();
            const int i8 = lane >> 3, j8 = lane & 7;
            for (int g = 0; g < N / 2; ++g) {
                const int n = 2 * g, m = n + 1;
                const int on = __builtin_amdgcn_readlane(e, n), om = __builtin_amdgcn_readlane(e, m);
                const float d = p16_leaf(Gt + p16_blk<N>(n, m), ent0[n * 8 + i8], ent0[m * 8 + j8], on, om);
                float sv[1] = {((S0[n * 8 + i8] + S0[m * 8 + j8]) - E) + 2.0f * d};
                int sp[1] = {lane};
                bool has;
// ... 48 lines not shown
                int sp[4];
                const float sx = S2[P * 16 + i16];
#pragma unroll
                for (int v = 0; v < 4; ++v) {
                    sv[v] = ((sx + S2[Q2 * 16 + jb + v]) - E) + 2.0f * part[v];
                    sp[v] = 4 * lane + v;
                }
                if constexpr (N == 8) {
                    float bv = INFINITY;
                    int bp = kBigPos;
#pragma unroll
                    for (int v = 0; v < 4; ++v) lexmin(bv, bp, sv[v], sp[v]);
                    wave_lexmin(bv, bp);
                    win = __builtin_amdgcn_readfirstlane(bp);
                    if (win > 255) win = 255;
                } else {
                    bool has;
                    int dst, op;
                    float ov;
                    wave_select_set<4>(sv, sp, 16, 256, sel, has, dst, ov, op);
                    if (has) {
                        pos3[(q * 16 + dst) * 2] = (uint8_t)(op >> 4);
                        pos3[(q * 16 + dst) * 2 + 1] = (uint8_t)(op & 15);
                        S3[q * 16 + dst] = ov;
                    }
                }
            }
            wave_lds_fence();
            if constexpr (N == 16) {
                const unsigned pi3 = *reinterpret_cast<const uint16_t *>(pos3 + i16 * 2);
                const uint64_t pj3 = *reinterpret_cast<const uint64_t *>(pos3 + (16 + jb) * 2);
                float part[4];
#pragma unroll
                for (int t2 = 0; t2 < 4; ++t2) {
                    const int xc = t2 >> 1, yc = t2 & 1;
                    const unsigned pa = *reinterpret_cast<const uint16_t *>(pos2 + (xc * 16 + i16) * 2);
                    const uint64_t pb = *reinterpret_cast<const uint64_t *>(pos2 + ((2 + yc) * 16 + jb) * 2);
                    float p2[4];
#pragma unroll
                    for (int tb = 0; tb < 4; ++tb) {
                        const int aa = tb >> 1, cc = tb & 1;
                        T1a[i8 * 9 + j8] = p16_t1<N>(Gt, ent0, pos1, e, 2 * xc + aa, 4 + 2 * yc + cc, i8, j8);
                        wave_lds_fence();
                        const int ri = (int)((pa >> (8 * aa)) & 0xffu);
#pragma unroll
                        for (int v = 0; v < 4; ++v) {
                            const int rj = (int)((pb >> (16 * v + 8 * cc)) & 0xffull);
                            const float val = T1a[ri * 9 + rj];
                            p2[v] = (tb == 0) ? val : p2[v] + val;
                        }
                        wave_lds_fence();
                    }
#pragma unroll
                    for (int v = 0; v < 4; ++v) T2a[i16 * 17 + jb + v] = p2[v];
                    wave_lds_fence();
                    const int ri = (int)((pi3 >> (8 * xc)) & 0xffu);
#pragma unroll
                    for (int v = 0; v < 4; ++v) {
                        const int rj = (int)((pj3 >> (16 * v + 8 * yc)) & 0xffull);
                        const float val = T2a[ri * 17 + rj];
                        part[v] = (t2 == 0) ? val : part[v] + val;
                    }
                    wave_lds_fence();
                }
                float bv = INFINITY;
                int bp = kBigPos;
                const float sx = S3[i16];
#pragma unroll
                for (int v = 0; v < 4; ++v) lexmin(bv, bp, ((sx + S3[16 + jb + v]) - E) + 2.0f * part[v], 4 * lane + v);
                wave_lexmin(bv, bp);
                win = __builtin_amdgcn_readfirstlane(bp);
                if (win > 255) win = 255;
            }
            {
                int en = 0;
                if (lane < N) {
                    const int n = lane;
                    int p = (n >> (N == 16 ? 3 : 2)) ? (win & 15) : (win >> 4);
                    if constexpr (N == 16) p = pos3[((n >> 3) * 16 + p) * 2 + ((n >> 2) & 1)];
                    p = pos2[((n >> 2) * 16 + p) * 2 + ((n >> 1) & 1)];
                    p = pos1[((n >> 1) * 8 + p) * 2 + (n & 1)];
                    en = ent0[n * 8 + p];
                }
                e = en;
            }
            wave_lds_fence();
        }
        if (lane < N) {
            a.idx[b * N + lane] = (uint8_t)e;
            if (a.out_i64) a.out_i64[b * N + lane] = e;
            if (a.out_u8) a.out_u8[b * N + lane] = (uint8_t)e;
        }
    }
}

}
```

quantization_amd/csrc/mcq_tf_kernels.h:

```cpp
#pragma once
#include "mcq_kernels.h"

#include <type_traits>

namespace mcq {

constexpr int kTfLevels = 6;

template <int K>
using tf_code_of = std::conditional_t<(K > 256), uint16_t, uint8_t>;

struct TfLists {
    uint8_t *ent;
    uint8_t *pos[kTfLevels];
    float *S[kTfLevels];
    int kc[kTfLevels];
    int64_t *out_i64;
    uint8_t *out_u8;
    const float *erG, *erXC, *erxx;
    float *erE, *erR;
    int erK;
};

__device__ __forceinline__ float shfl_f(float v, int src) {
    return __int_as_float(__builtin_amdgcn_ds_bpermute(src << 2, __float_as_int(v)));
}

#ifdef MCQ_STAMPS
constexpr int kStampSlots = 8, kStampWaves = 1 << 14, kStampKernels = 4;
__device__ unsigned long long g_stamps[kStampKernels * kStampWaves * kStampSlots];
struct Stamps {
    unsigned long long t[kStampSlots];
    __device__ __forceinline__ Stamps() { for (int i = 0; i < kStampSlots; ++i) t[i] = 0; t[0] = __builtin_amdgcn_s_memtime(); }
    __device__ __forceinline__ void at(int k) { asm volatile("s_waitcnt vmcnt(0) lgkmcnt(0)" ::: "memory"); t[k] = __builtin_amdgcn_s_memtime(); }
    __device__ __forceinline__ void flush(int kernel, unsigned wg, int every) {
        if (wg % (unsigned)every != 0 || (threadIdx.x & 63) != 0 || (threadIdx.x >> 6) != 0) return;
        const unsigned slot = (wg / (unsigned)every) & (kStampWaves - 1);
        unsigned long long *d = g_stamps + ((size_t)kernel * kStampWaves + slot) * kStampSlots;
        t[kStampSlots - 1] = __builtin_amdgcn_s_memtime();
        for (int i = 0; i < kStampSlots; ++i) d[i] = t[i];
    }
};
#else
struct Stamps {
    __device__ __forceinline__ void at(int) {}
    __device__ __forceinline__ void flush(int, unsigned, int) {}
};
#endif


template <int N, typename CT = uint8_t>
__global__ void __launch_bounds__(256)
k_tf_gram_terms(const float *__restrict__ G, const CT *__restrict__ idx, long B, int K, float *__restrict__ gterms,
                const int *__restrict__ nact) {
    constexpr int VW = 64 / N;
    if (nact) B = *nact;
    const int m = (int)(blockIdx.x % N);
    const long b = ((long)(blockIdx.x / N) * 4 + (threadIdx.x >> 6)) * VW + lane_id() / N;
    const int m2 = lane_id() % N;
    if (b >= B) return;
    const CT *id = idx + b * N;
    const int NK = N * K;
    gterms[(b * N + m) * N + m2] = G[((size_t)(m * K + id[m]) << __builtin_ctz((unsigned)NK)) + m2 * K + id[m2]];
}

template <int N, bool FROM_REG, typename CT = uint8_t>
__device__ __forceinline__ void tf_er_wave(long b, long bx, const CT *__restrict__ id, int e_reg,
                                           const float *__restrict__ gterms, const float *__restrict__ Gdirect,
                                           const float *__restrict__ XC, const float *__restrict__ xx, int K,
                                           float *__restrict__ E_out, float *__restrict__ R_out) {
    constexpr int NT = (N * N + 63) / 64;
    const int lane = lane_id();
    const int NK = N * K;
#define MCQ_ER_CODE(m) (FROM_REG ? __builtin_amdgcn_ds_bpermute((m) << 2, e_reg) : (int)id[FROM_REG ? 0 : (m)])
    float gt[NT];
#pragma unroll
    for (int j = 0; j < NT; ++j) {
        const int t = lane + 64 * j;
        const int tc = t < N * N ? t : 0;
        const float g = Gdirect ? Gdirect[(size_t)((tc / N) * K + MCQ_ER_CODE(tc / N)) * NK + (tc % N) * K + MCQ_ER_CODE(tc % N)]
                                : gterms[b * (N * N) + tc];
        gt[j] = t < N * N ? g : 0.f;
    }
    const int lm = lane < N ? lane : 0;
    const int clm = MCQ_ER_CODE(lm);
#undef MCQ_ER_CODE
    const float xt = lane < N ? XC[(size_t)bx * NK + lm * K + clm] : 0.f;
    const float xxb = xx[bx];
    float gp = gt[0];
#pragma unroll
    for (int j = 1; j < NT; ++j) gp = gp + gt[j];
    const float gsum = wave_sum_butterfly(gp), xsum = wave_sum_butterfly(xt);
    const float E = (gsum - 2.0f * xsum) + xxb;
    const int n = lane < N ? lane : 0;
    float col = 0.f, gnn = 0.f;
#pragma unroll
    for (int m = 0; m < N; ++m) {
        const float v = shfl_f(gt[(m * N) / 64], (m * N + n) & 63);
        col = (m == 0) ? v : col + v;
        if (m == n) gnn = v;
    }
    const float xo = col - xt;
    const float Rv = (E - 2.0f * xo) + gnn;
    if (lane < N) R_out[b * N + lane] = Rv;
    if (lane == 0) E_out[b] = E;
}

template <int N, typename CT = uint8_t>
__global__ void __launch_bounds__(256)
k_tf_er(const float *__restrict__ gterms, const float *__restrict__ XC, const CT *__restrict__ idx,
        const float *__restrict__ xx, long B, int K, float *__restrict__ E_out, float *__restrict__ R_out,
        const int *__restrict__ nact, const int *__restrict__ map, const float *__restrict__ Gdirect) {
    if (nact) B = *nact;
    const long b = (long)blockIdx.x * 4 + (threadIdx.x >> 6);
    if (b >= B) return;
    const long bx = map ? (long)map[b] : b;
    tf_er_wave<N, false, CT>(b, bx, idx + b * N, 0, gterms, Gdirect, XC, xx, K, E_out, R_out);
}

template <int K, int N>
__global__ void __launch_bounds__(256)
k_tf_stage0(const float *__restrict__ G, const float *__restrict__ XC, const tf_code_of<K> *__restrict__ idx,
            const float *__restrict__ R, const float *__restrict__ Q, long B, int keep,
            tf_code_of<K> *__restrict__ ent_out, float *__restrict__ S_out, tf_code_of<K> *__restrict__ idx_final ,
            const int *__restrict__ nact, const int *__restrict__ map) {
    using CT = tf_code_of<K>;
    constexpr int CB = (int)sizeof(CT);
    constexpr int VPL = (K >= 64) ? K / 64 : 1;
    constexpr int NK = N * K;
    constexpr int CH = (N - 1 < 8) ? (N > 1 ? N - 1 : 1) : 8;
    __shared__ u64 sel[4][kSelectLdsU64];
    Stamps stp;
    if (nact) B = *nact;
    int n;
    long b;
    if constexpr (N > 8) {
        const unsigned per_phase = gridDim.x / (N / 8);
        const unsigned ph = blockIdx.x / per_phase, r = blockIdx.x - ph * per_phase;
        n = (int)(r & 7u) + 8 * (int)ph;
        b = (long)(r >> 3) * 4 + (threadIdx.x >> 6);
    } else {
        n = blockIdx.x & (N - 1);
        b = (long)(blockIdx.x / N) * 4 + (threadIdx.x >> 6);
    }
    if (b >= B) return;
    const int lane = lane_id();
    const bool act = VPL * lane < K;
    const int k0 = act ? VPL * lane : 0;
    const CT *id = idx + b * N;
    const float *xc = XC + ((size_t)(map ? (long)map[b] : b) * NK + n * K + k0);
    const float *q = Q + n * K + k0;
    float xcv[VPL], qv[VPL];
    if constexpr (VPL == 4) {
        const f32x4 x4 = __builtin_nontemporal_load(reinterpret_cast<const f32x4 *>(xc)), q4 = *reinterpret_cast<const f32x4 *>(q);
#pragma unroll
        for (int i = 0; i < 4; ++i) { xcv[i] = x4[i]; qv[i] = q4[i]; }
    } else if constexpr (VPL % 4 == 0) {
#pragma unroll
        for (int i4 = 0; i4 < VPL / 4; ++i4) {
            const f32x4 x4 = reinterpret_cast<const f32x4 *>(xc)[i4], q4 = reinterpret_cast<const f32x4 *>(q)[i4];
#pragma unroll
            for (int i = 0; i < 4; ++i) { xcv[4 * i4 + i] = x4[i]; qv[4 * i4 + i] = q4[i]; }
        }
    } else {
#pragma unroll
        for (int i = 0; i < VPL; ++i) { xcv[i] = xc[i]; qv[i] = q[i]; }
    }
    const float Rv = R[(long)__builtin_amdgcn_readfirstlane((int)b) * N + n];
    __builtin_amdgcn_sched_barrier(0);
    unsigned long long iw[N * CB >= 8 ? N * CB / 8 : 1];
    if constexpr (N * CB >= 8) {
        const unsigned long long *ip =
            reinterpret_cast<const unsigned long long *>(idx) + (size_t)__builtin_amdgcn_readfirstlane((int)b) * (N * CB / 8);
#pragma unroll
        for (int q8 = 0; q8 < N * CB / 8; ++q8) iw[q8] = ip[q8];
    }
    auto code = [&](int m) -> int {
        if constexpr (N * CB >= 8) return (int)((iw[(m * CB) >> 3] >> (8 * ((m * CB) & 7))) & (CB == 1 ? 0xffull : 0xffffull));
        else return (int)id[m];
    };
    float t[VPL];
#pragma unroll
    for (int i = 0; i < VPL; ++i) t[i] = 0.f;
#pragma unroll
    for (int j0 = 0; j0 < N - 1; j0 += CH) {
        float gv[CH][VPL];
#pragma unroll
        for (int u = 0; u < CH; ++u) {
            const int j = j0 + u < N - 1 ? j0 + u : N - 2;
            const int m = j < n ? j : j + 1;
            const float *p = G + ((size_t)(m * K + code(m)) * NK + n * K + k0);
            if constexpr (VPL % 4 == 0) {
#pragma unroll
                for (int i4 = 0; i4 < VPL / 4; ++i4) {
                    const f32x4 t4 = reinterpret_cast<const f32x4 *>(p)[i4];
#pragma unroll
                    for (int i = 0; i < 4; ++i) gv[u][4 * i4 + i] = t4[i];
                }
            } else {
#pragma unroll
                for (int i = 0; i < VPL; ++i) gv[u][i] = p[i];
            }
        }
#pragma unroll
        for (int u = 0; u < CH; ++u)
            if (j0 + u < N - 1) {
#pragma unroll
                for (int i = 0; i < VPL; ++i) t[i] = (j0 + u == 0) ? gv[u][i] : t[i] + gv[u][i];
            }
    }
    float sv[VPL];
    int sp[VPL];
#pragma unroll
    for (int i = 0; i < VPL; ++i) {
        const float X = t[i] - xcv[i];
        sv[i] = act ? (Rv + qv[i]) + 2.0f * X : INFINITY;
        sp[i] = act ? k0 + i : kBigPos;
    }
    stp.at(1);
    float ov;
    int op, dst;
    bool has;
    wave_select_set<VPL>(sv, sp, keep, K, sel[threadIdx.x >> 6], has, dst, ov, op);
    stp.at(2);
    stp.flush(0, blockIdx.x, 16);
    if (N == 1) {
        if (lane == 0) idx_final[b] = (CT)op;
        return;
    }
    if (has) {
        ent_out[(b * N + n) * keep + dst] = (CT)op;
        S_out[(b * N + n) * keep + dst] = ov;
    }
}

template <int N>
__global__ void __launch_bounds__(256)
k_tf_stage0_k16(const float *__restrict__ G, const float *__restrict__ XC, const uint8_t *__restrict__ idx,
                const float *__restrict__ R, const float *__restrict__ Q, long B, int keep,
                uint8_t *__restrict__ ent_out, float *__restrict__ S_out, const int *__restrict__ nact,
                const int *__restrict__ map) {
    static_assert(N >= 4, "");
    constexpr int K = 16, NK = N * K, NG = N / 4;
    if (nact) B = *nact;
    const long w = (long)blockIdx.x * 4 + (threadIdx.x >> 6);
    const long b = w / NG;
    const int n0 = 4 * (int)(w % NG);
    if (b >= B) return;
    const int lane = lane_id();
    const int n = n0 + (lane >> 4), k = lane & 15;
    const float xcv = XC[(size_t)(map ? (long)map[b] : b) * NK + n0 * K + lane];
    const float qv = Q[n0 * K + lane];
    const float Rv = R[b * N + n];
    const long bu = __builtin_amdgcn_readfirstlane((int)b);
    unsigned long long iw[N >= 8 ? N / 8 : 1];
    if constexpr (N >= 8) {
        const unsigned long long *ip = reinterpret_cast<const unsigned long long *>(idx) + (size_t)bu * (N / 8);
#pragma unroll
        for (int q8 = 0; q8 < N / 8; ++q8) iw[q8] = ip[q8];
    } else {
        iw[0] = (unsigned long long)reinterpret_cast<const uint32_t *>(idx)[bu];
    }
    auto code = [&](int m) -> int { return (int)((iw[m >> 3] >> (8 * (m & 7))) & 0xffull) & (K - 1); };
    constexpr int CH = N < 8 ? N : 8;
    float t = 0.f;
    bool started = false;
#pragma unroll
    for (int m0 = 0; m0 < N; m0 += CH) {
        float gv[CH];
#pragma unroll
        for (int u = 0; u < CH; ++u) gv[u] = G[(size_t)((m0 + u) * K + code(m0 + u)) * NK + n0 * K + lane];
#pragma unroll
        for (int u = 0; u < CH; ++u) {
            const bool use = (m0 + u) != n;
            const float sum = t + gv[u];
            t = use ? (started ? sum : gv[u]) : t;
            started = started || use;
        }
    }
    const float X = t - xcv;
    const float sv = (Rv + qv) + 2.0f * X;
    const uint32_t hi = ord32(sv), lo = (uint32_t)k;
    const u64 key = ((u64)hi << 32) | lo;
    int rnk = 0;
#define MCQ_ROR(r)                                                                                                      \
    {                                                                                                                   \
        const u64 o = ((u64)(uint32_t)dpp_i<0x120 + r>((int)hi) << 32) | (uint32_t)dpp_i<0x120 + r>((int)lo);           \
        rnk += (o < key) ? 1 : 0;                                                                                       \
    }
    MCQ_ROR(1) MCQ_ROR(2) MCQ_ROR(3) MCQ_ROR(4) MCQ_ROR(5) MCQ_ROR(6) MCQ_ROR(7) MCQ_ROR(8)
    MCQ_ROR(9) MCQ_ROR(10) MCQ_ROR(11) MCQ_ROR(12) MCQ_ROR(13) MCQ_ROR(14) MCQ_ROR(15)
#undef MCQ_ROR
    const bool take = rnk < keep;
    const u64 tm = __ballot(take);
    const uint32_t rowbits = (uint32_t)(tm >> (lane & 48)) & 0xffffu;
    const int dst = __popc(rowbits & ((1u << k) - 1u));
    if (take) {
        ent_out[(b * N + n) * keep + dst] = (uint8_t)k;
        S_out[(b * N + n) * keep + dst] = sv;
    }
}

template <int KC, typename CT = uint8_t>
__device__ __forceinline__ void tf_leaf(const float *__restrict__ G, int NK, int K, int n, int m,
                                        const CT *__restrict__ en, const CT *__restrict__ em, int old_n,
                                        int old_m, float (&d)[KC * KC / 64]) {
    constexpr int VPL = KC * KC / 64;
    const int lane = lane_id();
    const int i = (VPL * lane) / KC, j0 = (VPL * lane) % KC;
    const uint32_t rown = (uint32_t)(n * K), colm = (uint32_t)(m * K);
    const int nksh = __builtin_ctz((unsigned)NK);
    const int bl = lane < 2 * KC ? lane : 2 * KC;
    const CT *bp = bl < KC ? en + bl : em + (bl < 2 * KC ? bl - KC : 0);
    int e_i = en[i], e_b = *bp;
    uint32_t w4 = 0;
    int ej[VPL];
    constexpr bool kPacked = (VPL == 4 && sizeof(CT) == 1);
    if constexpr (kPacked) {
        w4 = *reinterpret_cast<const uint32_t *>(em + j0);
        asm volatile("" : "+v"(e_i), "+v"(e_b), "+v"(w4));
    } else {
#pragma unroll
        for (int v = 0; v < VPL; ++v) ej[v] = em[j0 + v];
        asm volatile("" : "+v"(e_i), "+v"(e_b), "+v"(ej[0]));
    }
    const uint32_t si = rown + (uint32_t)e_i;
    const uint32_t br = bl < KC ? rown + (uint32_t)e_b : rown + (uint32_t)old_n;
    const uint32_t bc = (bl >= KC && bl < 2 * KC) ? colm + (uint32_t)e_b : colm + (uint32_t)old_m;
    float g[VPL];
    if constexpr (kPacked) {
#pragma unroll
        for (int v = 0; v < 4; ++v) g[v] = G[(si << nksh) + colm + ((w4 >> (8 * v)) & 0xffu)];
    } else {
#pragma unroll
        for (int v = 0; v < VPL; ++v) g[v] = G[(si << nksh) + colm + (uint32_t)ej[v]];
    }
    const float bv = G[(br << nksh) + bc];
    const float u = shfl_f(bv, i), w = shfl_f(bv, 2 * KC);
#pragma unroll
    for (int v = 0; v < VPL; ++v) {
        const float vj = shfl_f(bv, KC + j0 + v);
        d[v] = ((g[v] - u) - vj) + w;
    }
}

__device__ __attribute__((noinline)) void tf_er_next(const float *G, const float *XC, const float *xx, int K, float *E, float *R,
                                                     long b, int N, int e) {
    if (N == 8) tf_er_wave<8, true, uint8_t>(b, b, nullptr, e, nullptr, G, XC, xx, K, E, R);
    else if (N == 4) tf_er_wave<4, true, uint8_t>(b, b, nullptr, e, nullptr, G, XC, xx, K, E, R);
    else if (N == 16) tf_er_wave<16, true, uint8_t>(b, b, nullptr, e, nullptr, G, XC, xx, K, E, R);
}

template <typename CT>
__device__ __forceinline__ void tf_emit(const TfLists &L, long b, int N, int nlev, int win, CT *__restrict__ idx_out) {
    const int n = lane_id();
    int e = 0;
    if (n < N) {
        int v = nlev - 1;
        int g = n >> v;
        int p = (g & 1) ? win % L.kc[v] : win / L.kc[v];
        while (v > 0) {
            const int child = (n >> (v - 1)) & 1;
            p = L.pos[v][((b * (N >> v) + g) * L.kc[v] + p) * 2 + child];
            --v;
            g = n >> v;
        }
        e = reinterpret_cast<const CT *>(L.ent)[(b * N + n) * L.kc[0] + p];
        idx_out[b * N + n] = (CT)e;
        if (L.out_i64) L.out_i64[b * N + n] = e;
        if (L.out_u8) L.out_u8[b * N + n] = (uint8_t)e;
    }
    if (L.erE) tf_er_next(L.erG, L.erXC, L.erxx, L.erK, L.erE, L.erR, b, N, e);
}

template <int VPL, typename CT = uint8_t, int LAYOUT = kLaneMajor>
__device__ __forceinline__ void tf_finish(const float (&sv)[VPL], const int (&sp)[VPL], int keep, int KCin, u64 *scratch,
                                          const TfLists &L, int vout , long b, int N,
                                          int gout, CT *__restrict__ idx_final) {
    if (idx_final != nullptr) {
        float bv = INFINITY;
        int bp = kBigPos;
#pragma unroll
        for (int i = 0; i < VPL; ++i) lexmin(bv, bp, sv[i], sp[i]);
        wave_lexmin(bv, bp);
        int win = __builtin_amdgcn_readfirstlane(bp);
        if (win > KCin * KCin - 1) win = KCin * KCin - 1;
        tf_emit(L, b, N, vout, win, idx_final);
        return;
    }
    float ov;
    int op, dst;
    bool has;
    wave_select_set<VPL, LAYOUT>(sv, sp, keep, KCin * KCin, scratch, has, dst, ov, op);
    if (has) {
        const long o = (b * (N >> vout) + gout) * keep + dst;
        L.pos[vout][2 * o] = (uint8_t)(op / KCin);
        L.pos[vout][2 * o + 1] = (uint8_t)(op % KCin);
        L.S[vout][o] = ov;
    }
}

template <int KC, typename CT = uint8_t>
__global__ void __launch_bounds__(64)
k_tf_pair0(const float *__restrict__ G, const CT *__restrict__ idx, const float *__restrict__ E, TfLists L, long B,
           int N, int K, int keep, CT *__restrict__ idx_final, const int *__restrict__ nact) {
    constexpr int VPL = KC * KC / 64;
    __shared__ u64 scratch[kSelectLdsU64];
    Stamps stp;
    if (nact) B = *nact;
    const int Gout = N >> 1;
    const int g = (int)(blockIdx.x & (unsigned)(Gout - 1));
    const long b = (long)(blockIdx.x >> __builtin_ctz((unsigned)Gout));
    if (b >= B) return;
    const int lane = lane_id();
    const int n = 2 * g, m = n + 1;
    const CT *en = reinterpret_cast<const CT *>(L.ent) + (b * N + n) * KC, *em = reinterpret_cast<const CT *>(L.ent) + (b * N + m) * KC;
    const int i = (VPL * lane) / KC, j0 = (VPL * lane) % KC;
    const float Eb = E[b];
    const float se = L.S[0][(b * N + n) * KC + i];
    float so[VPL];
#pragma unroll
    for (int v = 0; v < VPL; ++v) so[v] = L.S[0][(b * N + m) * KC + j0 + v];
    float d[VPL];
    stp.at(1);
    tf_leaf<KC, CT>(G, N * K, K, n, m, en, em, idx[b * N + n], idx[b * N + m], d);
    float sv[VPL];
    int sp[VPL];
#pragma unroll
    for (int v = 0; v < VPL; ++v) {
        sv[v] = ((se + so[v]) - Eb) + 2.0f * d[v];
        sp[v] = VPL * lane + v;
    }
    stp.at(2);
    tf_finish<VPL, CT>(sv, sp, keep, KC, scratch, L, 1, b, N, g, idx_final);
    stp.at(3);
    stp.flush(1, blockIdx.x, 64);
}

__global__ void __launch_bounds__(64)
k_tf_pair0s(const float *__restrict__ G, const uint8_t *__restrict__ idx, const float *__restrict__ E, TfLists L, long B,
            int N, int K, int keep, uint8_t *__restrict__ idx_final, const int *__restrict__ nact) {
    constexpr int KC = 16, VPL = 4;
    __shared__ u64 scratch[kSelectLdsU64];
    Stamps stp;
    if (nact) B = *nact;
    const int Gout = N >> 1;
    const int g = (int)(blockIdx.x & (unsigned)(Gout - 1));
    const long b = (long)(blockIdx.x >> __builtin_ctz((unsigned)Gout));
    if (b >= B) return;
    const int lane = lane_id();
    const int n = 2 * g, m = n + 1;
    const int q4 = lane >> 4, c = lane & 15;
    const uint8_t *en = L.ent + (b * N + n) * KC, *em = en + KC;
    const float *Sn = L.S[0] + (b * N + n) * KC, *Sm = Sn + KC;
    const uint32_t *enw = reinterpret_cast<const uint32_t *>(en);
    uint32_t rw[VPL];
#pragma unroll
    for (int v = 0; v < VPL; ++v) rw[v] = enw[v];
    int e_j = em[c];
    int e_b = en[c];
    int old_n = idx[b * N + n], old_m = idx[b * N + m];
    const float sn_c = Sn[c], so = Sm[c];
    const float Eb = E[b];
    asm volatile("" : "+v"(e_j), "+v"(e_b), "+v"(old_n), "+v"(old_m));
    stp.at(1);
    const int nksh = __builtin_ctz((unsigned)(N * K));
    const uint32_t rown = (uint32_t)(n * K), colm = (uint32_t)(m * K);
    float gq[VPL];
#pragma unroll
    for (int v = 0; v < VPL; ++v) {
        const uint32_t e_i = (rw[v] >> (8 * q4)) & 0xffu;
        gq[v] = G[((rown + e_i) << nksh) + colm + (uint32_t)e_j];
    }
    const uint32_t br = lane < KC ? rown + (uint32_t)e_b : rown + (uint32_t)old_n;
    const uint32_t bc = (lane >= KC && lane < 2 * KC) ? colm + (uint32_t)e_j : colm + (uint32_t)old_m;
    const float bv = G[(br << nksh) + bc];
    const float vj = shfl_f(bv, KC + c), w = shfl_f(bv, 2 * KC);
    float sv[VPL];
    int sp[VPL];
#pragma unroll
    for (int v = 0; v < VPL; ++v) {
        const int i = 4 * v + q4;
        const float u = shfl_f(bv, i), se = shfl_f(sn_c, i);
        const float d = ((gq[v] - u) - vj) + w;
        sv[v] = ((se + so) - Eb) + 2.0f * d;
        sp[v] = 64 * v + lane;
    }
    stp.at(2);
    tf_finish<VPL, uint8_t, kSlotMajor>(sv, sp, keep, KC, scratch, L, 1, b, N, g, idx_final);
    stp.at(3);
    stp.flush(1, blockIdx.x, 64);
}

template <int KCH, int KC, typename CT = uint8_t>
__device__ __forceinline__ void tf_table1(const float *__restrict__ G, const CT *__restrict__ idx, const TfLists &L,
                                          long b, int N, int K, int X, int Y, float *leaf ,
                                          float (&t)[KC * KC / 64], Stamps &stp) {
    constexpr int VPLH = KCH * KCH / 64, VPL = KC * KC / 64, MH = KCH * KCH;
    const int lane = lane_id();
    const CT *id = idx + b * N;
    const CT *ent = reinterpret_cast<const CT *>(L.ent);
    const int G1 = N >> 1;
    const uint8_t *px = L.pos[1] + ((b * G1 + X) * KC) * 2, *py = L.pos[1] + ((b * G1 + Y) * KC) * 2;
    if constexpr (KCH == 16 && KC == 16) {
        constexpr int RS = KCH + 1, BO = KCH * RS;
        constexpr int LS = BO + 36;
        CT *cent = reinterpret_cast<CT *>(leaf + 4 * LS);
        uint8_t *crank = reinterpret_cast<uint8_t *>(cent + 64);
        const int NK = N * K;
        const int nksh = __builtin_ctz((unsigned)NK);
        const int w = lane >> 4, c = lane & 15;
        const int cb = (w < 2) ? 2 * X + w : 2 * Y + (w - 2);
        int mypos = (w < 2 ? px : py)[2 * c + (w & 1)];
        int myent = ent[(b * N + cb) * KCH + c];
        int oldv = id[cb];
        asm volatile("" : "+v"(mypos), "+v"(myent), "+v"(oldv));
        stp.at(1);
        int oldq[4];
#pragma unroll
        for (int qq = 0; qq < 4; ++qq) oldq[qq] = __builtin_amdgcn_readlane(oldv, 16 * qq);
        uint32_t m = 1u << mypos;
        m |= (uint32_t)dpp_i<0x121>((int)m);
        m |= (uint32_t)dpp_i<0x122>((int)m);
        m |= (uint32_t)dpp_i<0x124>((int)m);
        m |= (uint32_t)dpp_i<0x128>((int)m);
        crank[lane] = (uint8_t)__popc(m & ((1u << mypos) - 1u));
        if ((m >> c) & 1u) cent[w * 16 + __popc(m & ((1u << c) - 1u))] = (CT)myent;
        uint32_t mq[4];
        mq[0] = (uint32_t)__builtin_amdgcn_readlane((int)m, 0);
        mq[1] = (uint32_t)__builtin_amdgcn_readlane((int)m, 16);
        mq[2] = (uint32_t)__builtin_amdgcn_readlane((int)m, 32);
        mq[3] = (uint32_t)__builtin_amdgcn_readlane((int)m, 48);
        wave_lds_fence();
        int na_[4], nc_[4];
        uint32_t rown_[4], colm_[4];
        float bv[4];
#pragma unroll
        for (int tb = 0; tb < 4; ++tb) {
            const int a = tb >> 1, cc = tb & 1;
            const int n = 2 * X + a, mcb = 2 * Y + cc;
            na_[tb] = __popc(mq[a]);
            nc_[tb] = __popc(mq[2 + cc]);
            rown_[tb] = (uint32_t)(n * K);
            colm_[tb] = (uint32_t)(mcb * K);
            const bool isu = lane < na_[tb], isv = lane >= na_[tb] && lane < na_[tb] + nc_[tb];
            const uint32_t br = rown_[tb] + (uint32_t)(isu ? cent[a * 16 + lane] : oldq[a]);
            const uint32_t bc = colm_[tb] + (uint32_t)(isv ? cent[(2 + cc) * 16 + (lane - na_[tb])] : oldq[2 + cc]);
            bv[tb] = G[isu ? (bc << nksh) + br : (br << nksh) + bc];
        }
        float g[4][4];
        int rr[4][4];
#pragma unroll
        for (int tb = 0; tb < 4; ++tb) {
            const int a = tb >> 1, cc = tb & 1;
            const int na = na_[tb], nc = nc_[tb];
            const float rnc = 1.0f / (float)nc;
#pragma unroll
            for (int it = 0; it < 4; ++it) {
                const int q = lane + 64 * it;
                rr[tb][it] = -1;
                g[tb][it] = 0.f;
                if (64 * it < na * nc) {
                    const int qc = q < na * nc ? q : 0;
                    int ra = (int)((float)qc * rnc);
                    ra -= (ra * nc > qc);
                    ra += ((ra + 1) * nc <= qc);
                    const int rc = qc - ra * nc;
                    g[tb][it] = G[((rown_[tb] + (uint32_t)cent[a * 16 + ra]) << nksh) + colm_[tb] + (uint32_t)cent[(2 + cc) * 16 + rc]];
                    rr[tb][it] = q < na * nc ? ra * 16 + rc : -1;
                }
            }
        }
        stp.at(2);
#pragma unroll
// ... 92 lines not shown


constexpr int tf_leaf_lds_floats(int KCH, int code_bytes = 1) { return 4 * (KCH * (KCH + 1) + 36) + 16 + 16 * code_bytes; }

template <int KCH, int KC, typename CT = uint8_t>
__device__ __forceinline__ void tf_pair1_body(unsigned bid, float *leaf, const float *__restrict__ G, const CT *__restrict__ idx,
                                              const float *__restrict__ E, const TfLists &L, long B, int N, int K, int keep,
                                              CT *__restrict__ idx_final, const int *__restrict__ nact) {
    constexpr int VPL = KC * KC / 64;
    static_assert(tf_leaf_lds_floats(KCH, sizeof(CT)) * 4 >= kSelectLdsU64 * 8, "");
    u64 *scratch = reinterpret_cast<u64 *>(leaf);
    Stamps stp;
    if (nact) B = *nact;
    const int Gout = N >> 2;
    const int g = (int)(bid & (unsigned)(Gout - 1));
    const long b = (long)(bid >> __builtin_ctz((unsigned)Gout));
    if (b >= B) return;
    const int lane = lane_id();
    const int X = 2 * g, Y = X + 1, G1 = N >> 1;
    const int i = (VPL * lane) / KC, j0 = (VPL * lane) % KC;
    const float Eb = E[b];
    const float se = L.S[1][(b * G1 + X) * KC + i];
    float so[VPL];
#pragma unroll
    for (int v = 0; v < VPL; ++v) so[v] = L.S[1][(b * G1 + Y) * KC + j0 + v];
    float t[VPL];
    tf_table1<KCH, KC, CT>(G, idx, L, b, N, K, X, Y, leaf, t, stp);
    float sv[VPL];
    int sp[VPL];
#pragma unroll
    for (int v = 0; v < VPL; ++v) {
        sv[v] = ((se + so[v]) - Eb) + 2.0f * t[v];
        sp[v] = VPL * lane + v;
    }
    wave_lds_fence();
    tf_finish<VPL, CT>(sv, sp, keep, KC, scratch, L, 2, b, N, g, idx_final);
    stp.at(4);
    stp.flush(2, bid, 64);
}

template <int KCH, int KC, typename CT = uint8_t>
__global__ void __launch_bounds__(64)
k_tf_pair1(const float *__restrict__ G, const CT *__restrict__ idx, const float *__restrict__ E, TfLists L, long B,
           int N, int K, int keep, CT *__restrict__ idx_final, const int *__restrict__ nact) {
    __shared__ __attribute__((aligned(16))) float leaf[tf_leaf_lds_floats(KCH, sizeof(CT))];
    tf_pair1_body<KCH, KC, CT>(blockIdx.x, leaf, G, idx, E, L, B, N, K, keep, idx_final, nact);
}

template <int KCH, int KC, typename CT = uint8_t>
__device__ __forceinline__ void tf_table1_body(unsigned bid, float *leaf, const float *__restrict__ G, const CT *__restrict__ idx,
                                               const TfLists &L, long B, int N, int K, int ntab, int per, float *__restrict__ tabs,
                                               const int *__restrict__ nact) {
    constexpr int VPL = KC * KC / 64;
    Stamps stp;
    if (nact) B = *nact;
    const int t = (int)(bid & (unsigned)(ntab - 1));
    const long b = (long)(bid >> __builtin_ctz((unsigned)ntab));
    if (b >= B) return;
    const int lane = lane_id();
    const int psh = __builtin_ctz((unsigned)per);
    const int c = t & (per - 1), a = (t >> psh) & (per - 1), g = t >> (2 * psh);
    const int X = 2 * g * per + a, Y = (2 * g + 1) * per + c;
    float tv[VPL];
    tf_table1<KCH, KC, CT>(G, idx, L, b, N, K, X, Y, leaf, tv, stp);
    float *dst = tabs + ((size_t)(b * ntab + t) * (KC * KC) + VPL * lane);
    if constexpr (VPL == 4) {
        __builtin_nontemporal_store((f32x4){tv[0], tv[1], tv[2], tv[3]}, reinterpret_cast<f32x4 *>(dst));
    } else {
#pragma unroll
        for (int v = 0; v < VPL; ++v) dst[v] = tv[v];
    }
    stp.at(4);
    stp.flush(3, bid, 64);
}

template <int KCH, int KC, typename CT = uint8_t>
__global__ void __launch_bounds__(64)
k_tf_table1(const float *__restrict__ G, const CT *__restrict__ idx, TfLists L, long B, int N, int K, int ntab,
            int per, float *__restrict__ tabs, const int *__restrict__ nact) {
    __shared__ __attribute__((aligned(16))) float leaf[tf_leaf_lds_floats(KCH, sizeof(CT))];
    tf_table1_body<KCH, KC, CT>(blockIdx.x, leaf, G, idx, L, B, N, K, ntab, per, tabs, nact);
}

template <int KCH, int KC, typename CT = uint8_t>
__global__ void __launch_bounds__(64)
k_tf_level1(const float *__restrict__ G, const CT *__restrict__ idx, const float *__restrict__ E, TfLists L, long B, int N,
            int K, int keep, int ntab, int per, float *__restrict__ tabs, const int *__restrict__ nact, unsigned pair_blocks,
            unsigned tab_blocks, int ntab2, int per2, float *__restrict__ tabs2) {
    __shared__ __attribute__((aligned(16))) float leaf[tf_leaf_lds_floats(KCH, sizeof(CT))];
    if (blockIdx.x < pair_blocks) tf_pair1_body<KCH, KC, CT>(blockIdx.x, leaf, G, idx, E, L, B, N, K, keep, nullptr, nact);
    else if (blockIdx.x < pair_blocks + tab_blocks) tf_table1_body<KCH, KC, CT>(blockIdx.x - pair_blocks, leaf, G, idx, L, B, N, K, ntab, per, tabs, nact);
    else tf_table1_body<KCH, KC, CT>(blockIdx.x - pair_blocks - tab_blocks, leaf, G, idx, L, B, N, K, ntab2, per2, tabs2, nact);
}

template <int KH>
constexpr int tf_tab_stride() { return KH * (KH + 1); }

template <int KH, int COUNT>
__device__ __forceinline__ void tf_load_tables(const float *__restrict__ src, float *dst) {
    constexpr int M = KH * KH, RS = KH + 1, TS = tf_tab_stride<KH>();
    const int lane = lane_id();
    if constexpr ((COUNT * M) % 256 == 0 && KH % 4 == 0) {
        constexpr int IT = COUNT * M / 256;
        constexpr int BATCH = IT < 8 ? IT : 8;
#pragma unroll
        for (int i0 = 0; i0 < IT; i0 += BATCH) {
            f32x4 r[BATCH];
#pragma unroll
            for (int i = 0; i < BATCH; ++i)
                if (i0 + i < IT) r[i] = __builtin_nontemporal_load(reinterpret_cast<const f32x4 *>(src) + lane + 64 * (i0 + i));
#pragma unroll
            for (int i = 0; i < BATCH; ++i)
                if (i0 + i < IT) {
                    const int e = 4 * (lane + 64 * (i0 + i));
                    float *d = dst + (e / M) * TS + ((e % M) / KH) * RS + (e % KH);
#pragma unroll
                    for (int c = 0; c < 4; ++c) d[c] = r[i][c];
                }
        }
    } else {
        constexpr int TOT = COUNT * M;
        constexpr int IT = (TOT + 63) / 64;
        float r[IT];
#pragma unroll
        for (int i = 0; i < IT; ++i) r[i] = (lane + 64 * i < TOT) ? src[lane + 64 * i] : 0.f;
#pragma unroll
        for (int i = 0; i < IT; ++i) {
            const int e = lane + 64 * i;
            if (e < TOT) dst[(e / M) * TS + ((e % M) / KH) * RS + (e % KH)] = r[i];
        }
    }
}

template <int KH, int KC>
__device__ __forceinline__ void tf_up(const float *t00, const float *t01, const float *t10, const float *t11,
                                      const uint8_t *__restrict__ px, const uint8_t *__restrict__ py,
                                      float (&t)[KC * KC / 64]) {
    constexpr int VPL = KC * KC / 64;
    const int lane = lane_id();
    const int i = (VPL * lane) / KC, j0 = (VPL * lane) % KC;
    const int i0 = px[2 * i], i1 = px[2 * i + 1];
#pragma unroll
    for (int v = 0; v < VPL; ++v) {
        const int jj0 = py[2 * (j0 + v)], jj1 = py[2 * (j0 + v) + 1];
        t[v] = ((t00[i0 * (KH + 1) + jj0] + t01[i0 * (KH + 1) + jj1]) + t10[i1 * (KH + 1) + jj0]) + t11[i1 * (KH + 1) + jj1];
    }
}

template <int KH, int KC>
__global__ void __launch_bounds__(64)
k_tf_up(TfLists L, long B, int N, int u, int ntab, int per, const float *__restrict__ tabs_in, float *__restrict__ tabs_out,
        const int *__restrict__ nact) {
    constexpr int VPL = KC * KC / 64, MH = KH * KH, TS = tf_tab_stride<KH>();
    __shared__ __attribute__((aligned(16))) float th[4 * TS];
    if (nact) B = *nact;
    const int t = (int)(blockIdx.x & (unsigned)(ntab - 1));
    const long b = (long)(blockIdx.x >> __builtin_ctz((unsigned)ntab));
    if (b >= B) return;
    const int lane = lane_id();
    const int psh = __builtin_ctz((unsigned)per);
    const int c = t & (per - 1), a = (t >> psh) & (per - 1), g = t >> (2 * psh);
    const int X = 2 * g * per + a, Y = (2 * g + 1) * per + c;
    const int Gu = N >> u;
    const size_t cbase = (size_t)b * (4 * ntab) + (size_t)g * (4 * per * per);
#pragma unroll
    for (int i = 0; i < 2; ++i)
#pragma unroll
        for (int j = 0; j < 2; ++j)
            tf_load_tables<KH, 1>(tabs_in + (cbase + (size_t)(2 * a + i) * (2 * per) + (2 * c + j)) * MH, th + (2 * i + j) * TS);
    wave_lds_fence();
    float tv[VPL];
    tf_up<KH, KC>(th, th + TS, th + 2 * TS, th + 3 * TS, L.pos[u] + ((b * Gu + X) * KC) * 2, L.pos[u] + ((b * Gu + Y) * KC) * 2, tv);
    float *dst = tabs_out + ((size_t)(b * ntab + t) * (KC * KC) + VPL * lane);
#pragma unroll
    for (int v = 0; v < VPL; ++v) __builtin_nontemporal_store(tv[v], dst + v);
}

template <int KH, int KC, bool LAST, typename CT = uint8_t>
__global__ void __launch_bounds__(64)
k_tf_comb(const float *__restrict__ E, TfLists L, long B, int N, int v, int keep, const float *__restrict__ tabs,
          CT *__restrict__ idx_final, const int *__restrict__ nact) {
    constexpr int MH = KH * KH, RS = KH + 1, TS = tf_tab_stride<KH>();
    constexpr int VPL = (KC * KC / 64 <= 16) ? KC * KC / 64 : 16;
    constexpr int CHUNKS = KC * KC / (64 * VPL);
    constexpr int LDSF = (4 * TS * 4 >= kSelectLdsU64 * 8) ? 4 * TS : kSelectLdsU64 * 2;
    __shared__ __attribute__((aligned(16))) float th[LDSF];
    u64 *scratch = reinterpret_cast<u64 *>(th);
    __shared__ u64 sel2_store[(KC * KC / 64 > 16) ? kSelectLdsU64 : 1];
    u64 *sel2 = sel2_store;
    if (nact) B = *nact;
    const int Gout = N >> (v + 1);
    const int h = (int)(blockIdx.x & (unsigned)(Gout - 1));
    const long b = (long)(blockIdx.x >> __builtin_ctz((unsigned)Gout));
    if (b >= B) return;
    const int lane = lane_id();
    const int P = 2 * h, Q = P + 1, Gv = N >> v;
    tf_load_tables<KH, 4>(tabs + ((size_t)b * Gout + h) * 4 * MH, th);
    const float Eb = E[b];
    const uint8_t *px = L.pos[v] + ((b * Gv + P) * KC) * 2, *py = L.pos[v] + ((b * Gv + Q) * KC) * 2;
    const float *Sx = L.S[v] + (b * Gv + P) * KC, *Sy = L.S[v] + (b * Gv + Q) * KC;
    wave_lds_fence();
    if constexpr (CHUNKS == 1 && !LAST) {
        const int i = (VPL * lane) / KC, j0 = (VPL * lane) % KC;
        const float se = Sx[i];
        float t[VPL];
        tf_up<KH, KC>(th, th + TS, th + 2 * TS, th + 3 * TS, px, py, t);
        float sv[VPL];
        int sp[VPL];
#pragma unroll
        for (int u = 0; u < VPL; ++u) {
            sv[u] = ((se + Sy[j0 + u]) - Eb) + 2.0f * t[u];
            sp[u] = VPL * lane + u;
        }
        wave_lds_fence();
        tf_finish<VPL, CT>(sv, sp, keep, KC, scratch, L, v + 1, b, N, h, idx_final);
    } else if (!LAST) {
        static_assert(CHUNKS <= 4, "");
        float cv[4];
        int cp[4];
#pragma unroll
        for (int c = 0; c < 4; ++c) { cv[c] = INFINITY; cp[c] = kBigPos; }
        for (int c = 0; c < CHUNKS; ++c) {
            const int p0 = 64 * VPL * c + VPL * lane;
            const int i = p0 / KC, j0 = p0 % KC;
            const int i0 = px[2 * i], i1 = px[2 * i + 1];
            const float se = Sx[i];
            float sv[VPL];
            int sp[VPL];
#pragma unroll
            for (int u = 0; u < VPL; ++u) {
                const int jj0 = py[2 * (j0 + u)], jj1 = py[2 * (j0 + u) + 1];
                const float t = ((th[i0 * RS + jj0] + th[TS + i0 * RS + jj1]) + th[2 * TS + i1 * RS + jj0]) + th[3 * TS + i1 * RS + jj1];
                sv[u] = ((se + Sy[j0 + u]) - Eb) + 2.0f * t;
                sp[u] = p0 + u;
            }
            float ov;
            int op, dst;
            bool got;
            wave_select_set<VPL>(sv, sp, keep, KC * KC, sel2, got, dst, ov, op);
#pragma unroll
            for (int q = 0; q < 4; ++q)
                if (q == c) { cv[q] = got ? ov : INFINITY; cp[q] = got ? op : kBigPos; }
        }
        tf_finish<4, CT, kAnyOrder>(cv, cp, keep, KC, sel2, L, v + 1, b, N, h, nullptr);
    } else {
        float bv = INFINITY;
        int bp = kBigPos;
        for (int c = 0; c < CHUNKS; ++c) {
            const int p0 = 64 * VPL * c + VPL * lane;
            const int i = p0 / KC, j0 = p0 % KC;
            const int i0 = px[2 * i], i1 = px[2 * i + 1];
            const float se = Sx[i];
#pragma unroll
            for (int u = 0; u < VPL; ++u) {
                const int jj0 = py[2 * (j0 + u)], jj1 = py[2 * (j0 + u) + 1];
                const float t = ((th[i0 * RS + jj0] + th[TS + i0 * RS + jj1]) + th[2 * TS + i1 * RS + jj0]) + th[3 * TS + i1 * RS + jj1];
                lexmin(bv, bp, ((se + Sy[j0 + u]) - Eb) + 2.0f * t, p0 + u);
            }
        }
        wave_lexmin(bv, bp);
        if (bp > KC * KC - 1) bp = KC * KC - 1;
        tf_emit(L, b, N, v + 1, bp, idx_final);
    }
}

template <int KC1, int KC2, int KC3, typename CT = uint8_t>
__global__ void __launch_bounds__(256)
k_tf_comb3(const CT *__restrict__ idx, const float *__restrict__ E, TfLists L, long B, int N,
           const float *__restrict__ tabs, CT *__restrict__ idx_final, const int *__restrict__ nact) {
    constexpr int VPL2 = KC2 * KC2 / 64, M1 = KC1 * KC1;
    constexpr int PW = KC3 * KC3 / 4, VPLW = PW / 64;
    constexpr int RS1 = KC1 + 1, TS1 = tf_tab_stride<KC1>(), RS2 = KC2 + 1, TS2 = KC2 * RS2;
    __shared__ __attribute__((aligned(16))) float t1[16 * TS1];
    __shared__ __attribute__((aligned(16))) float t2[4 * TS2];
    __shared__ float wv[4];
    __shared__ int wp[4];
    (void)idx;
    if (nact) B = *nact;
    const long b = blockIdx.x;
    if (b >= B) return;
    const int lane = lane_id(), w = threadIdx.x >> 6;
    const int G2 = N >> 2;
    const int xc = w >> 1, yc = w & 1;
    constexpr int NB2 = 2 * VPL2;
    const int i2 = (VPL2 * lane) / KC2, j2 = (VPL2 * lane) % KC2;
    const uint8_t *px2 = L.pos[2] + ((b * G2 + xc) * KC2) * 2, *py2 = L.pos[2] + ((b * G2 + 2 + yc) * KC2) * 2;
    const unsigned pxw2 = *reinterpret_cast<const uint16_t *>(px2 + 2 * i2);
    uint32_t pyw2[NB2 / 4];
#pragma unroll
    for (int u = 0; u < NB2 / 4; ++u) pyw2[u] = reinterpret_cast<const uint32_t *>(py2 + 2 * j2)[u];
    const uint8_t *px = L.pos[3] + ((b * 2 + 0) * KC3) * 2, *py = L.pos[3] + ((b * 2 + 1) * KC3) * 2;
    const float *Sx = L.S[3] + (b * 2 + 0) * KC3, *Sy = L.S[3] + (b * 2 + 1) * KC3;
    const int p0 = w * PW + VPLW * lane;
    const int i3 = p0 / KC3, j3 = p0 % KC3;
    const unsigned pxw3 = *reinterpret_cast<const uint16_t *>(px + 2 * i3);
    unsigned pyw3[VPLW];
    float sy3[VPLW];
#pragma unroll
    for (int v = 0; v < VPLW; ++v) {
        pyw3[v] = *reinterpret_cast<const uint16_t *>(py + 2 * (j3 + v));
        sy3[v] = Sy[j3 + v];
    }
    const float sx3 = Sx[i3];
    const float Eb = E[b];
    tf_load_tables<KC1, 4>(tabs + ((size_t)b * 16 + 4 * w) * M1, t1 + 4 * w * TS1);
    __builtin_amdgcn_sched_barrier(0);
    __syncthreads();
    {
        const int X0 = 2 * xc, Y0 = 2 * yc;
        const float *t00 = t1 + (4 * X0 + Y0) * TS1, *t01 = t1 + (4 * X0 + Y0 + 1) * TS1, *t10 = t1 + (4 * (X0 + 1) + Y0) * TS1,
                    *t11 = t1 + (4 * (X0 + 1) + Y0 + 1) * TS1;
        const int i0 = (int)(pxw2 & 0xffu), i1 = (int)(pxw2 >> 8);
        float *dst = t2 + w * TS2 + i2 * RS2 + j2;
#pragma unroll
        for (int v = 0; v < VPL2; ++v) {
            const uint32_t wj = pyw2[v >> 1] >> (16 * (v & 1));
            const int jj0 = (int)(wj & 0xffu), jj1 = (int)((wj >> 8) & 0xffu);
            dst[v] = ((t00[i0 * RS1 + jj0] + t01[i0 * RS1 + jj1]) + t10[i1 * RS1 + jj0]) + t11[i1 * RS1 + jj1];
        }
    }
    __syncthreads();
    float bv = INFINITY;
    int bp = kBigPos;
    {
        const int i0 = (int)(pxw3 & 0xffu), i1 = (int)(pxw3 >> 8);
#pragma unroll
        for (int v = 0; v < VPLW; ++v) {
            const int jj0 = (int)(pyw3[v] & 0xffu), jj1 = (int)(pyw3[v] >> 8);
            const float t = ((t2[i0 * RS2 + jj0] + t2[TS2 + i0 * RS2 + jj1]) + t2[2 * TS2 + i1 * RS2 + jj0]) + t2[3 * TS2 + i1 * RS2 + jj1];
            lexmin(bv, bp, ((sx3 + sy3[v]) - Eb) + 2.0f * t, p0 + v);
        }
    }
    wave_lexmin(bv, bp);
    if (lane == 0) { wv[w] = bv; wp[w] = bp; }
    __syncthreads();
    if (w == 0) {
        float rv = wv[0];
        int rp = wp[0];
#pragma unroll
        for (int u = 1; u < 4; ++u) lexmin(rv, rp, wv[u], wp[u]);
        if (rp > KC3 * KC3 - 1) rp = KC3 * KC3 - 1;
        tf_emit(L, b, N, 4, rp, idx_final);
    }
}

// ... 2 lines not shown
```

quantization_amd/quantizer.py:

```python
import binascii
import ctypes
import math
import os
import weakref

import torch
from torch import Tensor, nn

from . import _lib


_param_epoch = [0]
_quantizer_params = {}
_optimizer_hits = weakref.WeakKeyDictionary()


def _note_optimizer_step(optimizer, *_args, **_kwargs):
    try:
        nparams = sum(len(g["params"]) for g in optimizer.param_groups)
        known = _optimizer_hits.get(optimizer)
        if known is None or known[0] != nparams or known[2] != len(_quantizer_params):
            hit = False
            for g in optimizer.param_groups:
                for q in g["params"]:
                    r = _quantizer_params.get(id(q))
                    if r is not None and r() is q:
                        hit = True
                        break
                if hit:
                    break
            known = (nparams, hit, len(_quantizer_params))
            _optimizer_hits[optimizer] = known
        if known[1]:
            _param_epoch[0] += 1
    except Exception:
        _param_epoch[0] += 1


_hook_installed = [False]


def _ensure_optimizer_hook():
    if not _hook_installed[0]:
        from torch.optim.optimizer import register_optimizer_step_post_hook
        register_optimizer_step_post_hook(_note_optimizer_step)
        _hook_installed[0] = True


class _PreparedState:
    __slots__ = ("key", "blob", "flavour", "stream", "event", "scales_dev", "scale_flags", "lscale_exp", "cscale_exp")


def _is_pow2(n: int) -> bool:
    return n > 0 and (n & (n - 1)) == 0


def _scale_exp(scale: Tensor, speed: float) -> float:
    return float((scale.detach().to("cpu", torch.float32) * speed).exp())


class Quantizer(nn.Module):

    def __init__(self, dim: int, codebook_size: int, num_codebooks: int):
        super().__init__()
        assert _is_pow2(codebook_size)
        assert _is_pow2(num_codebooks)
        self.dim = dim
        self.codebook_size = codebook_size
        self.num_codebooks = num_codebooks
        self.to_logits = nn.Linear(dim, codebook_size * num_codebooks)
        self.centers = nn.Parameter(
            self.to_logits.weight.detach().clone().reshape(num_codebooks, codebook_size, dim))
        self.logits_scale = nn.Parameter(torch.zeros(()))
        self.centers_scale = nn.Parameter(torch.zeros(()))
        self.scale_speed = 10.0
        id_bytes = binascii.b2a_hex(os.urandom(4))
        self.id_str = id_bytes.decode("utf-8")
        self.register_buffer("id_buf", torch.tensor(list(id_bytes), dtype=torch.uint8))
        self.skip_fixed_points = False
        self._pinned_scales = None
        self._prep = None
        self._ws = None

    def __getstate__(self):
        st = super().__getstate__() if hasattr(super(), "__getstate__") else self.__dict__.copy()
        st = dict(st)
        st["_prep"] = None
        st["_ws"] = None
        st.pop("_host_stage", None)
        return st

    def _current_prep(self):
        if self._prep is None:
            raise RuntimeError("no derived state: call Quantizer._prepared() before reading its scale factors")
        return self._prep

    @property
    def _scale_flags(self) -> int:
        return self._current_prep().scale_flags

    @property
    def _lscale_exp(self) -> float:
        return self._current_prep().lscale_exp

    @property
    def _cscale_exp(self) -> float:
        return self._current_prep().cscale_exp

    @property
    def _scales_dev(self):
        return self._prep.scales_dev if self._prep is not None else None

    def load_state_dict(self, *args, **kwargs):
        ret = super().load_state_dict(*args, **kwargs)
        self.id_str = bytes(self.id_buf.tolist()).decode("utf-8")
        self._prep = None
        return ret

    def pin_scale_factors(self, cscale_exp=None, lscale_exp=None) -> None:
        if cscale_exp is None and lscale_exp is None:
            self._pinned_scales = None
        else:
            assert cscale_exp is not None and lscale_exp is not None
            self._pinned_scales = (float(cscale_exp), float(lscale_exp), float(self.centers_scale.detach()), float(self.logits_scale.detach()))
        self._prep = None

    def invalidate_cache(self) -> None:
        self._prep = None

    def get_id(self) -> str:
        return self.id_str

    def show_init_invocation(self) -> str:
        return (f"quantization.Quantizer(dim={self.dim}, codebook_size={self.codebook_size}, "
                f"num_codebooks={self.num_codebooks})")

    def get_centers(self) -> Tensor:
        return (self.centers_scale * self.scale_speed).exp() * self.centers

    def get_data_mean(self) -> Tensor:
        return self.get_centers().mean(dim=1).sum(dim=0).detach()

    def _prepared(self, any_flavour: bool = False) -> Tensor:
        ps = (self.centers, self.centers_scale, self.logits_scale, self.to_logits.weight, self.to_logits.bias)
        trainable = any(p.requires_grad for p in ps)
        if trainable:
            _ensure_optimizer_hook()
        training = torch.is_grad_enabled() and trainable
        for p in ps:
            if id(p) not in _quantizer_params or _quantizer_params[id(p)]() is not p:
                if len(_quantizer_params) > 4096:
                    for k_ in [k_ for k_, r_ in _quantizer_params.items() if r_() is None]:
                        del _quantizer_params[k_]
                _quantizer_params[id(p)] = weakref.ref(p)
        key = tuple((p.data_ptr(), p._version, str(p.device)) for p in ps) + (_param_epoch[0],)
        pr = self._prep
        if pr is not None and pr.key == key and (any_flavour or pr.flavour == "host" or (training and pr.flavour != "decode")):
            cur = torch.cuda.current_stream(pr.blob.device)
            if cur.cuda_stream != pr.stream:
                cur.wait_event(pr.event)
                pr.blob.record_stream(cur)
                if pr.scales_dev is not None:
# ... 14 lines not shown
        bias = self.to_logits.bias.detach().to(torch.float32).contiguous()
        with torch.cuda.device(dev):
            st = torch.cuda.current_stream(dev).cuda_stream
            if on_device:
                scales = torch.empty(2, dtype=torch.float32, device=dev)
                cs, ls = self.centers_scale.detach(), self.logits_scale.detach()
                assert cs.dtype == torch.float32 and ls.dtype == torch.float32
                scale_flags = 2
                cscale_exp = lscale_exp = 1.0
                rc = L.mcq_prepare_params(centers.data_ptr(), cs.data_ptr(), ls.data_ptr(), self.scale_speed, weight.data_ptr(),
                                          bias.data_ptr(), N, K, D, blob.data_ptr(), scales.data_ptr(), st)
            else:
                both = torch.stack([self.centers_scale.detach(), self.logits_scale.detach()]).to(torch.float32)
                both = both.to("cpu")
                scales = None
                scale_flags = 0
                pin = self._pinned_scales
                if pin is not None and (float(both[0]), float(both[1])) == pin[2:]:
                    cscale_exp, lscale_exp = pin[0], pin[1]
                else:
                    cscale_exp = _scale_exp(both[0], self.scale_speed)
                    lscale_exp = _scale_exp(both[1], self.scale_speed)
                rc = L.mcq_prepare(centers.data_ptr(), cscale_exp, None if decode_only else weight.data_ptr(),
                                   None if decode_only else bias.data_ptr(), N, K, D, blob.data_ptr(), st)
        _lib.check(rc, "mcq_prepare")
        with torch.cuda.device(dev):
            ev = torch.cuda.Event()
            cur = torch.cuda.current_stream(dev)
            ev.record(cur)
        pr = _PreparedState()
        pr.key, pr.blob, pr.stream, pr.event = key, blob, cur.cuda_stream, ev
        pr.flavour = "device" if on_device else ("decode" if decode_only else "host")
        pr.scales_dev, pr.scale_flags, pr.lscale_exp, pr.cscale_exp = scales, scale_flags, lscale_exp, cscale_exp
        self._prep = pr
        return blob

    def _check_domain(self):
        assert 16 <= self.codebook_size <= 1024, (
            "the index search needs 16 <= codebook_size <= 1024 (the reference itself fails below 16, "
            "quantization.py:506; byte codes need <= 256, :271: larger codebooks encode with as_bytes=False)")
        assert self.num_codebooks <= 64, "num_codebooks <= 64 (QuantizerTrainer produces at most 64: quantization.py:614)"
        assert self.num_codebooks * self.codebook_size <= 16384, "num_codebooks * codebook_size <= 16384 (the Gram matrix: 1 GB)"
        assert self.dim <= 16384, "dim <= 16384 (the i32 accumulators of the fixed-point products, include/mcq.h)"

    def _workspace(self, B: int, dev) -> Tensor:
        L = _lib.lib()
        need = L.mcq_encode_workspace_bytes(B, self.num_codebooks, self.codebook_size, self.dim)
        if not isinstance(self._ws, dict):
            self._ws = {}
        key = (dev.index, torch.cuda.current_stream(dev).cuda_stream)
        ws = self._ws.get(key)
        if ws is None or ws.numel() < need:
            if len(self._ws) >= 8:
                self._ws.clear()
            ws = self._ws[key] = torch.empty(need, dtype=torch.uint8, device=dev)
        return ws

    def _search(self, x2d: Tensor, iters: int, as_bytes: bool) -> Tensor:
        self._check_domain()
        if not x2d.is_cuda:
            raise _lib.McqError("quantization_amd: the index search runs on a HIP device tensor only "
                                "(no CPU fallback)")
        L = _lib.lib()
        N, K, D = self.num_codebooks, self.codebook_size, self.dim
        x_fp16 = x2d.dtype == torch.float16
        x2d = x2d.detach().contiguous() if x_fp16 else x2d.detach().to(torch.float32).contiguous()
        B = x2d.shape[0]
        dev = x2d.device
        with torch.no_grad():
            blob = self._prepared()
        pack = 2 if (as_bytes and K == 16 and N >= 2) else 1
        if as_bytes:
            out = torch.empty((B, N // pack), dtype=torch.uint8, device=dev)
        else:
            out = torch.empty((B, N), dtype=torch.int64, device=dev)
        if B == 0:
            return out
        ws = self._workspace(B, dev)
        with torch.cuda.device(dev):
            st = torch.cuda.current_stream(dev).cuda_stream
            rc = L.mcq_encode_ex(x2d.data_ptr(), B, blob.data_ptr(), self._lscale_exp, N, K, D, int(iters),
                                 out.data_ptr() if as_bytes else None, None if as_bytes else out.data_ptr(),
                                 ws.data_ptr(), ws.numel(), st,
                                 (1 if getattr(self, "skip_fixed_points", False) else 0) | self._scale_flags |
                                 (4 if x_fp16 else 0))
        _lib.check(rc, "mcq_encode")
        return out

    def encode(self, x: Tensor, refine_indexes_iters: int = 5, as_bytes: bool = True) -> Tensor:
        x2d = x.reshape(-1, self.dim)
        if as_bytes:
            assert self.codebook_size <= 256
        codes = self._search(x2d, refine_indexes_iters, as_bytes)
        return codes.reshape(*x.shape[:-1], codes.shape[-1])

    def encode_from_host(self, x: Tensor, refine_indexes_iters: int = 5, as_bytes: bool = True,
                         chunk: int = 32768) -> Tensor:
        dev = self.centers.device
        if dev.type != "cuda":
            raise _lib.McqError("quantization_amd.Quantizer runs on a HIP device only")
        x2d = x.reshape(-1, self.dim)
        if x2d.dtype != torch.float16:
            x2d = x2d.to(torch.float32)
        if not x2d.is_pinned():
            x2d = x2d.contiguous().pin_memory()
        B = x2d.shape[0]
        pack = 2 if (as_bytes and self.codebook_size == 16 and self.num_codebooks >= 2) else 1
        width = self.num_codebooks // pack
        out = torch.empty((B, width), dtype=torch.uint8 if as_bytes else torch.int64, pin_memory=True)
        compute = torch.cuda.current_stream(dev)
        rows = min(chunk, max(B, 1))
        stage = getattr(self, "_host_stage", None)
        if stage is None or stage[0].device != dev or stage[0].shape[1] < rows or stage[0].dtype != x2d.dtype:
            stage = (torch.empty((2, rows, self.dim), dtype=x2d.dtype, device=dev), torch.cuda.Stream(dev))
            self._host_stage = stage
        bufs, copy = [stage[0][0], stage[0][1]], stage[1]
        copy.wait_stream(compute)
        ready = [torch.cuda.Event() for _ in range(2)]
        freed = [torch.cuda.Event() for _ in range(2)]
        results = []
        for ci, lo in enumerate(range(0, B, chunk)):
            hi = min(lo + chunk, B)
            slot = ci & 1
            with torch.cuda.stream(copy):
                if ci >= 2:
                    copy.wait_event(freed[slot])
                bufs[slot][:hi - lo].copy_(x2d[lo:hi], non_blocking=True)
                ready[slot].record(copy)
            compute.wait_event(ready[slot])
            codes = self.encode(bufs[slot][:hi - lo], refine_indexes_iters, as_bytes)
            freed[slot].record(compute)
            out[lo:hi].copy_(codes, non_blocking=True)
            results.append(codes)
        compute.synchronize()
        del results
        return out.reshape(*x.shape[:-1], width)

    def _compute_indexes(self, x: Tensor, refine_indexes_iters: int = 3) -> Tensor:
        assert x.ndim == 2 and x.shape[1] == self.dim
        return self._search(x, refine_indexes_iters, as_bytes=False)

    def _refine_indexes(self, x: Tensor, indexes: Tensor) -> Tensor:
        self._check_domain()
        if not x.is_cuda:
            raise _lib.McqError("quantization_amd: the index search runs on a HIP device tensor only")
        L = _lib.lib()
        N, K, D = self.num_codebooks, self.codebook_size, self.dim
        x2d = x.detach().to(torch.float32).contiguous()
        B = x2d.shape[0]
        idx = indexes.to(device=x2d.device, dtype=torch.int64).contiguous()
        assert idx.shape == (B, N)
        out = torch.empty_like(idx)
        if B == 0:
            return out
        with torch.no_grad():
            blob = self._prepared()
        ws = self._workspace(B, x2d.device)
        with torch.cuda.device(x2d.device):
            st = torch.cuda.current_stream(x2d.device).cuda_stream
            rc = L.mcq_refine_indexes(x2d.data_ptr(), B, blob.data_ptr(), N, K, D, 1, idx.data_ptr(), out.data_ptr(),
                                      ws.data_ptr(), ws.numel(), st)
        _lib.check(rc, "mcq_refine_indexes")
        return out

    def _logits(self, x: Tensor) -> Tensor:
        x = (self.logits_scale * self.scale_speed).exp() * x
        return self.to_logits(x)
# ... 282 lines not shown
```

Measured before the change: 12.36 million vectors/s.

## Enable fixed-point row skipping by default with compacted ER state and strided capped grids

Makes skipping of converged rows (fixed points) the default encode path for refine iterations of 3 or more. Rows whose codes stop changing are compacted out, and later passes run only on the active set. The compaction kernel now carries the E/R refinement state along and writes final codes directly, which removes the finalize pass. From iteration 3 onward, kernels run with a capped grid and loop over blocks up to the device-side active count, so that idle blocks are not launched. The trade-offs are extra compaction kernels and memsets, plus indirection through a row map. Exactness still relies on converged rows being true fixed points.

After: 13.57 million vectors/s (median of 6 runs). 9.8% higher.

```diff
diff --git a/include/mcq.h b/include/mcq.h
--- a/include/mcq.h
+++ b/include/mcq.h
@@ -36,6 +36,7 @@
                size_t workspace_bytes, void *stream);
 
 #define MCQ_ENCODE_SKIP_FIXED_POINTS 1u
+#define MCQ_ENCODE_ALL_PASSES 8u
 #define MCQ_ENCODE_LSCALE_FROM_PREPARED 2u
 #define MCQ_ENCODE_X_FP16 4u
 int mcq_encode_ex(const float *x, long B, const void *prepared, float lscale_exp, int N, int K, int D,
diff --git a/quantization_amd/_lib.py b/quantization_amd/_lib.py
--- a/quantization_amd/_lib.py
+++ b/quantization_amd/_lib.py
@@ -15,6 +15,7 @@
 )
 
 MCQ_EINVAL, MCQ_EUNSUPPORTED, MCQ_EWORKSPACE = -1, -2, -3
+MCQ_ENCODE_ALL_PASSES = 8
 _lib = None
 
 
diff --git a/quantization_amd/csrc/mcq_api.hip b/quantization_amd/csrc/mcq_api.hip
--- a/quantization_amd/csrc/mcq_api.hip
+++ b/quantization_amd/csrc/mcq_api.hip
@@ -7,6 +7,7 @@
 #include "mcq_train_kernels.h"
 
 #include <cstdlib>
+#include <utility>
 #include <vector>
 
 using namespace mcq;
@@ -133,6 +134,8 @@
     w.tf.ent = nullptr;
     w.tf.out_i64 = nullptr;
     w.tf.out_u8 = nullptr;
+    w.tf.out_pack = 1;
+    w.tf.map = nullptr;
     w.tf.erG = w.tf.erXC = w.tf.erxx = nullptr;
     w.tf.erE = w.tf.erR = nullptr;
     w.tf.erK = 0;
@@ -264,12 +267,20 @@
     return launch_fgemm<FG_LOGITS>(g, st);
 }
 
+constexpr unsigned kCapStage0 = 32768, kCapWave = 65536;
+inline unsigned pass_grid(unsigned full, bool capped, unsigned cap) { return (capped && full > cap) ? cap : full; }
+
 template <int K>
 int launch_tf_stage0_k(int N, const float *G, const float *XC, const tf_code_of<K> *idx, const float *R, const float *Q, long B,
-                       int keep, tf_code_of<K> *ent, float *S, tf_code_of<K> *fin, const int *nact, const int *map, hipStream_t st) {
-    const dim3 grid((unsigned)(((B + 3) / 4) * N)), block(256);
-#define MCQ_S0_CASE(NN) \
-    case NN: hipLaunchKernelGGL((k_tf_stage0<K, NN>), grid, block, 0, st, G, XC, idx, R, Q, B, keep, ent, S, fin, nact, map); break;
+                       int keep, tf_code_of<K> *ent, float *S, tf_code_of<K> *fin, const int *nact, const int *map, hipStream_t st,
+                       bool capped) {
+    const unsigned vgrid = (unsigned)(((B + 3) / 4) * N);
+    const dim3 grid(pass_grid(vgrid, capped, kCapStage0)), block(256);
+#define MCQ_S0_CASE(NN)                                                                                                            \
+    case NN:                                                                                                                       \
+        if (capped) hipLaunchKernelGGL((k_tf_stage0<K, NN, true>), grid, block, 0, st, G, XC, idx, R, Q, B, keep, ent, S, fin, nact, map, vgrid); \
+        else hipLaunchKernelGGL((k_tf_stage0<K, NN, false>), grid, block, 0, st, G, XC, idx, R, Q, B, keep, ent, S, fin, nact, map, vgrid);      \
+        break;
     switch (N) {
         MCQ_S0_CASE(1) MCQ_S0_CASE(2) MCQ_S0_CASE(4) MCQ_S0_CASE(8) MCQ_S0_CASE(16) MCQ_S0_CASE(32) MCQ_S0_CASE(64)
         default: return MCQ_EUNSUPPORTED;
@@ -280,16 +291,18 @@
 }
 
 int launch_tf_stage0(int K, int N, const float *G, const float *XC, const uint16_t *idx, const float *R, const float *Q,
-                     long B, int keep, uint16_t *ent, float *S, uint16_t *fin, const int *nact, const int *map, hipStream_t st) {
+                     long B, int keep, uint16_t *ent, float *S, uint16_t *fin, const int *nact, const int *map, hipStream_t st,
+                     bool capped) {
     switch (K) {
-        case 512: return launch_tf_stage0_k<512>(N, G, XC, idx, R, Q, B, keep, ent, S, fin, nact, map, st);
-        case 1024: return launch_tf_stage0_k<1024>(N, G, XC, idx, R, Q, B, keep, ent, S, fin, nact, map, st);
+        case 512: return launch_tf_stage0_k<512>(N, G, XC, idx, R, Q, B, keep, ent, S, fin, nact, map, st, capped);
+        case 1024: return launch_tf_stage0_k<1024>(N, G, XC, idx, R, Q, B, keep, ent, S, fin, nact, map, st, capped);
         default: return MCQ_EUNSUPPORTED;
     }
 }
 
 int launch_tf_stage0(int K, int N, const float *G, const float *XC, const uint8_t *idx, const float *R, const float *Q,
-                     long B, int keep, uint8_t *ent, float *S, uint8_t *fin, const int *nact, const int *map, hipStream_t st) {
+                     long B, int keep, uint8_t *ent, float *S, uint8_t *fin, const int *nact, const int *map, hipStream_t st,
+                     bool capped) {
     if (K == 16 && N >= 4 && keep <= 16) {
         const dim3 grid((unsigned)((B * (N / 4) + 3) / 4)), block(256);
 #define MCQ_S16_CASE(NN) \
@@ -303,11 +316,11 @@
         return 0;
     }
     switch (K) {
-        case 16: return launch_tf_stage0_k<16>(N, G, XC, idx, R, Q, B, keep, ent, S, fin, nact, map, st);
-        case 32: return launch_tf_stage0_k<32>(N, G, XC, idx, R, Q, B, keep, ent, S, fin, nact, map, st);
-        case 64: return launch_tf_stage0_k<64>(N, G, XC, idx, R, Q, B, keep, ent, S, fin, nact, map, st);
-        case 128: return launch_tf_stage0_k<128>(N, G, XC, idx, R, Q, B, keep, ent, S, fin, nact, map, st);
-        case 256: return launch_tf_stage0_k<256>(N, G, XC, idx, R, Q, B, keep, ent, S, fin, nact, map, st);
+        case 16: return launch_tf_stage0_k<16>(N, G, XC, idx, R, Q, B, keep, ent, S, fin, nact, map, st, capped);
+        case 32: return launch_tf_stage0_k<32>(N, G, XC, idx, R, Q, B, keep, ent, S, fin, nact, map, st, capped);
+        case 64: return launch_tf_stage0_k<64>(N, G, XC, idx, R, Q, B, keep, ent, S, fin, nact, map, st, capped);
+        case 128: return launch_tf_stage0_k<128>(N, G, XC, idx, R, Q, B, keep, ent, S, fin, nact, map, st, capped);
+        case 256: return launch_tf_stage0_k<256>(N, G, XC, idx, R, Q, B, keep, ent, S, fin, nact, map, st, capped);
         default: return MCQ_EUNSUPPORTED;
     }
 }
@@ -348,11 +361,13 @@
 
 template <typename CT>
 int launch_tf_comb(int kh, int kc, const float *E, const TfLists &L, long B, int N, int v, int keep, const float *tabs,
-                   CT *fin, const int *nact, hipStream_t st) {
-    const dim3 grid((unsigned)(B * (N >> (v + 1)))), block(64);
+                   CT *fin, const int *nact, hipStream_t st, bool capped) {
+    if (fin == nullptr) capped = false;
+    const dim3 grid(pass_grid((unsigned)(B * (N >> (v + 1))), capped, kCapWave)), block(64);
 #define MCQ_COMB_CASE(A, C)                                                                                                        \
     if (kh == A && kc == C) {                                                                                                     \
-        if (fin) hipLaunchKernelGGL((k_tf_comb<A, C, true, CT>), grid, block, 0, st, E, L, B, N, v, keep, tabs, fin, nact);       \
+        if (fin && capped) hipLaunchKernelGGL((k_tf_comb<A, C, true, CT, true>), grid, block, 0, st, E, L, B, N, v, keep, tabs, fin, nact); \
+        else if (fin) hipLaunchKernelGGL((k_tf_comb<A, C, true, CT>), grid, block, 0, st, E, L, B, N, v, keep, tabs, fin, nact);  \
         else hipLaunchKernelGGL((k_tf_comb<A, C, false, CT>), grid, block, 0, st, E, L, B, N, v, keep, tabs, fin, nact);          \
         MCQ_LAUNCH_CHECK();                                                                                                       \
         return 0;                                                                                                                 \
@@ -393,10 +408,14 @@
     static const bool on = !(getenv("MCQ_PASS16") && atoi(getenv("MCQ_PASS16")) == 0);
     return on;
 }
+inline long skip_min_batch() {
+    const char *v = getenv("MCQ_SKIP_MIN_BATCH");
+    return v ? atol(v) : 8192;
+}
 
 template <typename CT>
 int run_tf_combines(const float *G, const CT *idx_cur, CT *idx_new, const WorkspaceT<CT> &w, const TfLists &L, long B, int N,
-                    int K, const int *nact, hipStream_t st, Prof *prof) {
+                    int K, const int *nact, hipStream_t st, Prof *prof, bool capped) {
     const bool small = (K == 16);
     const int nlev = tf_levels(N);
     {
@@ -407,7 +426,11 @@
         bool done0 = false;
         if constexpr (sizeof(CT) == 1) {
             if (!small) {
-                hipLaunchKernelGGL(k_tf_pair0s, grid, dim3(64), 0, st, G, idx_cur, w.E, L, B, N, K, keep, fin, nact);
+                if (capped)
+                    hipLaunchKernelGGL(k_tf_pair0s<true>, dim3(pass_grid(grid.x, true, kCapWave)), dim3(64), 0, st, G, idx_cur, w.E, L, B, N,
+                                       K, keep, fin, nact);
+                else
+                    hipLaunchKernelGGL(k_tf_pair0s<false>, grid, dim3(64), 0, st, G, idx_cur, w.E, L, B, N, K, keep, fin, nact);
                 done0 = true;
             }
         }
@@ -422,10 +445,15 @@
         const int groups2 = N >> 3, per1 = 2, ntab1 = groups2 * per1 * per1;
         const unsigned pair_blocks = (unsigned)(B * (N / 4)), tab_blocks = (unsigned)(B * ntab1);
         const int ntab3 = fuse_l3 ? 16 : 1, per3 = fuse_l3 ? 4 : 1;
-        const dim3 grid(pair_blocks + tab_blocks + (fuse_l3 ? (unsigned)(B * ntab3) : 0u));
+        const unsigned vgrid = pair_blocks + tab_blocks + (fuse_l3 ? (unsigned)(B * ntab3) : 0u);
+        const dim3 grid(pass_grid(vgrid, capped, kCapWave));
         if (prof) prof->begin(CAT_LEVEL1_FUSED);
-        MCQ_TF_LAUNCH2((k_tf_level1<8, 8, CT>), (k_tf_level1<16, 16, CT>), grid, dim3(64), G, idx_cur, w.E, L, B, N, K, keep, ntab1, per1, w.tabs[0],
-                       nact, pair_blocks, tab_blocks, ntab3, per3, w.tabs[1]);
+        if (capped)
+            MCQ_TF_LAUNCH2((k_tf_level1<8, 8, CT, true>), (k_tf_level1<16, 16, CT, true>), grid, dim3(64), G, idx_cur, w.E, L, B, N, K, keep, ntab1,
+                           per1, w.tabs[0], nact, pair_blocks, tab_blocks, ntab3, per3, w.tabs[1], vgrid);
+        else
+            MCQ_TF_LAUNCH2((k_tf_level1<8, 8, CT>), (k_tf_level1<16, 16, CT>), grid, dim3(64), G, idx_cur, w.E, L, B, N, K, keep, ntab1, per1, w.tabs[0],
+                           nact, pair_blocks, tab_blocks, ntab3, per3, w.tabs[1], vgrid);
         MCQ_LAUNCH_CHECK();
         if (prof) prof->end(CAT_LEVEL1_FUSED);
     } else if (N >= 4) {
@@ -469,7 +497,7 @@
             cur ^= 1;
         }
         if (prof) prof->begin(cat_comb);
-        const int rc = launch_tf_comb<CT>(L.kc[v - 1], L.kc[v], w.E, L, B, N, v, keep, w.tabs[cur], fin, nact, st);
+        const int rc = launch_tf_comb<CT>(L.kc[v - 1], L.kc[v], w.E, L, B, N, v, keep, w.tabs[cur], fin, nact, st, capped);
         if (rc) return rc;
         if (prof) prof->end(cat_comb);
     }
@@ -496,7 +524,7 @@
     if (chunk < B) chunk &= ~127L;
     const Prepared P = prepared_view(prepared, N, K, D);
     const int pack = (out_u8 != nullptr && K == 16 && N >= 2) ? 2 : 1;
-    const bool skip = (flags & MCQ_ENCODE_SKIP_FIXED_POINTS) != 0 && iters >= 2;
+    const bool want_skip = (flags & MCQ_ENCODE_ALL_PASSES) == 0 && iters >= 3;
 
     for (long lo = 0; lo < B; lo += chunk) {
         const long Bc = (B - lo < chunk) ? (B - lo) : chunk;
@@ -529,10 +557,13 @@
             if (rc) return rc;
             if (prof) prof->end(CAT_XC);
         }
+        const bool use_p16 = sizeof(CT) == 1 && K == 16 && (N == 16 || N == 8) && iters > 0 && prof == nullptr && pass16_enabled();
+        const bool skip = want_skip && !use_p16 && Bc >= skip_min_batch();
         int iters_left = iters;
         CT *idx_cur = w.idx, *idx_new = skip ? w.idxB : w.idx, *idx_pk = w.idxC;
         const int *map_cur = nullptr, *nact = nullptr;
         int *map_nxt = w.map[0], *map_spare = w.map[1];
+        float *E_cur = w.E, *R_cur = w.R, *E_alt = w.gterms, *R_alt = w.gterms + ((Bc + 3) & ~3L);
         if (skip) {
             hipError_t e = hipMemsetAsync(w.cnt, 0, 64 * sizeof(int), st);
             if (e != hipSuccess) return (int)e;
@@ -540,7 +571,7 @@
         }
         bool wrote_direct = false;
         if constexpr (sizeof(CT) == 1) {
-            if (K == 16 && (N == 16 || N == 8) && iters > 0 && !skip && prof == nullptr && pass16_enabled()) {
+            if (use_p16) {
                 static bool allowed16[64] = {};
                 int dev = 0;
                 if (hipGetDevice(&dev) != hipSuccess || dev < 0 || dev >= 64) dev = 63;
@@ -568,41 +599,51 @@
                 iters_left = 0;
             }
         }
-        const bool er_in_emit = !skip && (N == 4 || N == 8 || N == 16);
+        const bool er_in_emit = (N == 4 || N == 8 || N == 16);
         bool er_ready = false;
         for (int it = 0; it < iters_left; ++it) {
+            const bool last_pass = (it + 1 == iters);
+            const bool capped = skip && it >= 3;
             if (!er_ready) {
                 if (prof) prof->begin(CAT_ER);
-                rc = launch_tf_er<CT>(N, P.G, w.XC, idx_cur, w.xx, Bc, K, w.E, w.R, w.gterms, nact, map_cur, st);
+                rc = launch_tf_er<CT>(N, P.G, w.XC, idx_cur, w.xx, Bc, K, E_cur, R_cur, w.gterms, nact, map_cur, st);
                 if (rc) return rc;
                 if (prof) prof->end(CAT_ER);
             }
             er_ready = false;
             if (prof) prof->begin(CAT_STAGE0);
-            rc = launch_tf_stage0(K, N, P.G, w.XC, idx_cur, w.R, P.Q, Bc, (N == 1) ? 1 : w.tf.kc[0], reinterpret_cast<CT *>(w.tf.ent),
-                                  w.tf.S[0], (N == 1) ? idx_new : static_cast<CT *>(nullptr), nact, map_cur, st);
+            rc = launch_tf_stage0(K, N, P.G, w.XC, idx_cur, R_cur, P.Q, Bc, (N == 1) ? 1 : w.tf.kc[0], reinterpret_cast<CT *>(w.tf.ent),
+                                  w.tf.S[0], (N == 1) ? idx_new : static_cast<CT *>(nullptr), nact, map_cur, st, capped);
             if (rc) return rc;
             if (prof) prof->end(CAT_STAGE0);
+            bool direct_out = false;
             if (N >= 2) {
                 TfLists L = w.tf;
-                if (er_in_emit && it + 1 < iters) {
-                    L.erG = P.G; L.erXC = w.XC; L.erxx = w.xx; L.erE = w.E; L.erR = w.R; L.erK = K;
+                L.map = map_cur;
+                if (er_in_emit && !last_pass) {
+                    L.erG = P.G; L.erXC = w.XC; L.erxx = w.xx; L.erE = E_cur; L.erR = R_cur; L.erK = K;
                     er_ready = true;
                 }
-                const bool direct_out = (it + 1 == iters) && !skip && pack == 1;
+                direct_out = last_pass;
                 if (direct_out) {
                     L.out_i64 = out_i64 ? out_i64 + lo * N : nullptr;
-                    L.out_u8 = out_u8 ? out_u8 + lo * N : (codes_also ? codes_also + lo * N : nullptr);
+                    L.out_u8 = out_u8 ? out_u8 + lo * (N / pack) : (codes_also ? codes_also + lo * N : nullptr);
+                    L.out_pack = out_u8 ? pack : 1;
                     wrote_direct = true;
                 }
-                rc = run_tf_combines<CT>(P.G, idx_cur, idx_new, w, L, Bc, N, K, nact, st, prof);
+                WorkspaceT<CT> wc = w;
+                wc.E = E_cur;
+                wc.R = R_cur;
+                rc = run_tf_combines<CT>(P.G, idx_cur, idx_new, wc, L, Bc, N, K, nact, st, prof, capped);
                 if (rc) return rc;
             }
-            if (skip) {
-                const int last = (it + 1 == iters) ? 1 : 0;
+            if (skip && !direct_out) {
                 if (prof) prof->begin(CAT_TAIL);
                 hipLaunchKernelGGL(k_compact<CT>, dim3((unsigned)((Bc + 255) / 256)), dim3(256), 0, st, idx_cur, idx_new,
-                                   map_cur, nact, Bc, N, last, w.final_idx, idx_pk, map_nxt, w.cnt + it);
+                                   map_cur, nact, Bc, N, last_pass ? 1 : 0, idx_pk, map_nxt, w.cnt + it,
+                                   er_ready ? E_cur : nullptr, er_ready ? R_cur : nullptr, E_alt, R_alt, pack,
+                                   out_u8 ? out_u8 + lo * (N / pack) : nullptr, out_i64 ? out_i64 + lo * N : nullptr,
+                                   codes_also ? codes_also + lo * N : nullptr);
                 MCQ_LAUNCH_CHECK();
                 if (prof) prof->end(CAT_TAIL);
                 CT *t = idx_cur; idx_cur = idx_pk; idx_pk = t;
@@ -610,13 +651,16 @@
                 map_cur = map_nxt;
                 map_nxt = old_map ? old_map : map_spare;
                 nact = w.cnt + it;
+                if (er_ready) {
+                    std::swap(E_cur, E_alt);
+                    std::swap(R_cur, R_alt);
+                }
             }
         }
-        if (wrote_direct) continue;
-        const CT *result = (skip && iters > 0) ? w.final_idx : w.idx;
+        if (wrote_direct || skip) continue;
         const long outn = (out_i64 != nullptr) ? Bc * N : Bc * (N / pack);
         if (prof) prof->begin(CAT_TAIL);
-        hipLaunchKernelGGL(k_finalize<CT>, dim3((unsigned)((outn + 255) / 256)), dim3(256), 0, st, result, Bc, N, pack,
+        hipLaunchKernelGGL(k_finalize<CT>, dim3((unsigned)((outn + 255) / 256)), dim3(256), 0, st, w.idx, Bc, N, pack,
                            out_u8 ? out_u8 + lo * (N / pack) : nullptr, out_i64 ? out_i64 + lo * N : nullptr,
                            codes_also ? codes_also + lo * N : nullptr);
         MCQ_LAUNCH_CHECK();
@@ -1015,7 +1059,7 @@
     if (K > 256) return MCQ_EUNSUPPORTED;
     if (B > 0 && (!logits_out || !idx_out)) return MCQ_EINVAL;
     return run_encode(x, B, prepared, lscale_exp, N, K, D, refine_iters, nullptr, idx_out, workspace, workspace_bytes,
-                      static_cast<hipStream_t>(stream), nullptr, nullptr, flags & ~MCQ_ENCODE_SKIP_FIXED_POINTS, logits_out,
+                      static_cast<hipStream_t>(stream), nullptr, nullptr, flags | MCQ_ENCODE_ALL_PASSES, logits_out,
                       codes_out);
 }
 
@@ -1299,7 +1343,8 @@
         prof.stream = st;
         prof.only = only;
         rc = run_encode(x, B, prepared, lscale_exp, N, K, D, refine_iters, wide ? nullptr : dummy,
-                        wide ? reinterpret_cast<int64_t *>(dummy) : nullptr, workspace, workspace_bytes, st, &prof);
+                        wide ? reinterpret_cast<int64_t *>(dummy) : nullptr, workspace, workspace_bytes, st, &prof, nullptr,
+                        MCQ_ENCODE_ALL_PASSES);
         (void)hipStreamSynchronize(st);
         for (size_t i = 0; rc == 0 && i < prof.cat.size(); ++i) {
             float ms = 0.f;
diff --git a/quantization_amd/csrc/mcq_kernels.h b/quantization_amd/csrc/mcq_kernels.h
--- a/quantization_amd/csrc/mcq_kernels.h
+++ b/quantization_amd/csrc/mcq_kernels.h
@@ -481,21 +481,35 @@
 template <typename CT>
 __global__ void k_compact(const CT *__restrict__ idx_old, const CT *__restrict__ idx_new,
                           const int *__restrict__ map_cur, const int *__restrict__ nact, long B, int N, int last,
-                          CT *__restrict__ final_idx, CT *__restrict__ idx_packed, int *__restrict__ map_next,
-                          int *__restrict__ cnt_next) {
+                          CT *__restrict__ idx_packed, int *__restrict__ map_next, int *__restrict__ cnt_next,
+                          const float *__restrict__ E_in, const float *__restrict__ R_in, float *__restrict__ E_out,
+                          float *__restrict__ R_out, int pack, uint8_t *__restrict__ out_u8, int64_t *__restrict__ out_i64,
+                          uint8_t *__restrict__ codes_also) {
     const long s = (long)blockIdx.x * blockDim.x + threadIdx.x;
     if (nact) B = *nact;
     if (s >= B) return;
-    const int orig = map_cur ? map_cur[s] : (int)s;
+    const long orig = map_cur ? (long)map_cur[s] : s;
     bool changed = false;
     if (!last)
         for (int n = 0; n < N; ++n) changed = changed || (idx_old[s * N + n] != idx_new[s * N + n]);
     if (changed) {
-        const int slot = atomicAdd(cnt_next, 1);
-        for (int n = 0; n < N; ++n) idx_packed[(long)slot * N + n] = idx_new[s * N + n];
-        map_next[slot] = orig;
+        const long slot = atomicAdd(cnt_next, 1);
+        for (int n = 0; n < N; ++n) idx_packed[slot * N + n] = idx_new[s * N + n];
+        map_next[slot] = (int)orig;
+        if (E_in != nullptr) {
+            E_out[slot] = E_in[s];
+            for (int n = 0; n < N; ++n) R_out[slot * N + n] = R_in[s * N + n];
+        }
+    } else if (out_i64 != nullptr) {
+        for (int n = 0; n < N; ++n) {
+            const CT v = idx_new[s * N + n];
+            out_i64[orig * N + n] = v;
+            if (codes_also) codes_also[orig * N + n] = (uint8_t)v;
+        }
+    } else if (pack == 1) {
+        for (int n = 0; n < N; ++n) out_u8[orig * N + n] = (uint8_t)idx_new[s * N + n];
     } else {
-        for (int n = 0; n < N; ++n) final_idx[(long)orig * N + n] = idx_new[s * N + n];
+        for (int n = 0; n < N; n += 2) out_u8[orig * (N / 2) + n / 2] = (uint8_t)(idx_new[s * N + n] + 16 * idx_new[s * N + n + 1]);
     }
 }
 
diff --git a/quantization_amd/csrc/mcq_pass16_kernels.h b/quantization_amd/csrc/mcq_pass16_kernels.h
--- a/quantization_amd/csrc/mcq_pass16_kernels.h
+++ b/quantization_amd/csrc/mcq_pass16_kernels.h
@@ -108,6 +108,7 @@
         for (int r = 0; r < XS; ++r) xcv[r] = a.XC[(size_t)b * NK + 64 * r + lane];
         int e = lane < N ? (int)a.idx[b * N + lane] & 15 : 0;
         const float xxb = a.xx[b];
+        bool converged = false;
         for (int pass = 0; pass < a.iters; ++pass) {
             float E, Rv;
             {
@@ -322,9 +323,11 @@
                     p = pos1[((n >> 1) * 8 + p) * 2 + (n & 1)];
                     en = ent0[n * 8 + p];
                 }
+                converged = __ballot(lane < N && en != e) == 0;
                 e = en;
             }
             wave_lds_fence();
+            if (converged) break;
         }
         if (lane < N) {
             a.idx[b * N + lane] = (uint8_t)e;
diff --git a/quantization_amd/csrc/mcq_tf_kernels.h b/quantization_amd/csrc/mcq_tf_kernels.h
--- a/quantization_amd/csrc/mcq_tf_kernels.h
+++ b/quantization_amd/csrc/mcq_tf_kernels.h
@@ -17,6 +17,8 @@
     int kc[kTfLevels];
     int64_t *out_i64;
     uint8_t *out_u8;
+    int out_pack;
+    const int *map;
     const float *erG, *erXC, *erxx;
     float *erE, *erR;
     int erK;
@@ -119,11 +121,11 @@
 }
 
 template <int K, int N>
-__global__ void __launch_bounds__(256)
-k_tf_stage0(const float *__restrict__ G, const float *__restrict__ XC, const tf_code_of<K> *__restrict__ idx,
-            const float *__restrict__ R, const float *__restrict__ Q, long B, int keep,
-            tf_code_of<K> *__restrict__ ent_out, float *__restrict__ S_out, tf_code_of<K> *__restrict__ idx_final ,
-            const int *__restrict__ nact, const int *__restrict__ map) {
+__device__ __forceinline__ void
+tf_stage0_body(unsigned bid, unsigned vgrid, const float *__restrict__ G, const float *__restrict__ XC, const tf_code_of<K> *__restrict__ idx,
+               const float *__restrict__ R, const float *__restrict__ Q, long B, int keep,
+               tf_code_of<K> *__restrict__ ent_out, float *__restrict__ S_out, tf_code_of<K> *__restrict__ idx_final ,
+               const int *__restrict__ nact, const int *__restrict__ map) {
     using CT = tf_code_of<K>;
     constexpr int CB = (int)sizeof(CT);
     constexpr int VPL = (K >= 64) ? K / 64 : 1;
@@ -135,13 +137,13 @@
     int n;
     long b;
     if constexpr (N > 8) {
-        const unsigned per_phase = gridDim.x / (N / 8);
-        const unsigned ph = blockIdx.x / per_phase, r = blockIdx.x - ph * per_phase;
+        const unsigned per_phase = vgrid / (N / 8);
+        const unsigned ph = bid / per_phase, r = bid - ph * per_phase;
         n = (int)(r & 7u) + 8 * (int)ph;
         b = (long)(r >> 3) * 4 + (threadIdx.x >> 6);
     } else {
-        n = blockIdx.x & (N - 1);
-        b = (long)(blockIdx.x / N) * 4 + (threadIdx.x >> 6);
+        n = bid & (N - 1);
+        b = (long)(bid / N) * 4 + (threadIdx.x >> 6);
     }
     if (b >= B) return;
     const int lane = lane_id();
@@ -223,7 +225,7 @@
     bool has;
     wave_select_set<VPL>(sv, sp, keep, K, sel[threadIdx.x >> 6], has, dst, ov, op);
     stp.at(2);
-    stp.flush(0, blockIdx.x, 16);
+    stp.flush(0, bid, 16);
     if (N == 1) {
         if (lane == 0) idx_final[b] = (CT)op;
         return;
@@ -231,6 +233,26 @@
     if (has) {
         ent_out[(b * N + n) * keep + dst] = (CT)op;
         S_out[(b * N + n) * keep + dst] = ov;
+    }
+}
+
+template <int K, int N, bool STRIDED = false>
+__global__ void __launch_bounds__(256)
+k_tf_stage0(const float *__restrict__ G, const float *__restrict__ XC, const tf_code_of<K> *__restrict__ idx,
+            const float *__restrict__ R, const float *__restrict__ Q, long B, int keep,
+            tf_code_of<K> *__restrict__ ent_out, float *__restrict__ S_out, tf_code_of<K> *__restrict__ idx_final ,
+            const int *__restrict__ nact, const int *__restrict__ map, unsigned vgrid) {
+    if constexpr (!STRIDED) {
+        tf_stage0_body<K, N>(blockIdx.x, gridDim.x, G, XC, idx, R, Q, B, keep, ent_out, S_out, idx_final, nact, map);
+        return;
+    }
+    const unsigned per = (N > 8) ? vgrid / (N / 8) : vgrid;
+    const unsigned nr = nact ? (unsigned)((*nact + 3) / 4) * (N > 8 ? 8u : (unsigned)N) : per;
+    const unsigned need = (N > 8) ? nr * (N / 8) : nr;
+    for (unsigned c = blockIdx.x; c < need; c += gridDim.x) {
+        const unsigned vb = (N > 8) ? (c / nr) * per + c % nr : c;
+        tf_stage0_body<K, N>(vb, vgrid, G, XC, idx, R, Q, B, keep, ent_out, S_out, idx_final, nact, map);
+        wave_lds_fence();
     }
 }
 
@@ -345,10 +367,10 @@
 }
 
 __device__ __attribute__((noinline)) void tf_er_next(const float *G, const float *XC, const float *xx, int K, float *E, float *R,
-                                                     long b, int N, int e) {
-    if (N == 8) tf_er_wave<8, true, uint8_t>(b, b, nullptr, e, nullptr, G, XC, xx, K, E, R);
-    else if (N == 4) tf_er_wave<4, true, uint8_t>(b, b, nullptr, e, nullptr, G, XC, xx, K, E, R);
-    else if (N == 16) tf_er_wave<16, true, uint8_t>(b, b, nullptr, e, nullptr, G, XC, xx, K, E, R);
+                                                     long b, long bx, int N, int e) {
+    if (N == 8) tf_er_wave<8, true, uint8_t>(b, bx, nullptr, e, nullptr, G, XC, xx, K, E, R);
+    else if (N == 4) tf_er_wave<4, true, uint8_t>(b, bx, nullptr, e, nullptr, G, XC, xx, K, E, R);
+    else if (N == 16) tf_er_wave<16, true, uint8_t>(b, bx, nullptr, e, nullptr, G, XC, xx, K, E, R);
 }
 
 template <typename CT>
@@ -367,10 +389,18 @@
         }
         e = reinterpret_cast<const CT *>(L.ent)[(b * N + n) * L.kc[0] + p];
         idx_out[b * N + n] = (CT)e;
-        if (L.out_i64) L.out_i64[b * N + n] = e;
-        if (L.out_u8) L.out_u8[b * N + n] = (uint8_t)e;
-    }
-    if (L.erE) tf_er_next(L.erG, L.erXC, L.erxx, L.erK, L.erE, L.erR, b, N, e);
+    }
+    const long row = (L.map && (L.out_i64 || L.out_u8 || L.erE)) ? (long)L.map[b] : b;
+    if (L.out_i64 && n < N) L.out_i64[row * N + n] = e;
+    if (L.out_u8) {
+        if (L.out_pack == 2) {
+            const int hi = __builtin_amdgcn_ds_bpermute(((n + 1) & 63) << 2, e);
+            if (n < N && (n & 1) == 0) L.out_u8[row * (N / 2) + n / 2] = (uint8_t)(e + 16 * hi);
+        } else if (n < N) {
+            L.out_u8[row * N + n] = (uint8_t)e;
+        }
+    }
+    if (L.erE) tf_er_next(L.erG, L.erXC, L.erxx, L.erK, L.erE, L.erR, b, row, N, e);
 }
 
 template <int VPL, typename CT = uint8_t, int LAYOUT = kLaneMajor>
@@ -437,16 +467,16 @@
     stp.flush(1, blockIdx.x, 64);
 }
 
-__global__ void __launch_bounds__(64)
-k_tf_pair0s(const float *__restrict__ G, const uint8_t *__restrict__ idx, const float *__restrict__ E, TfLists L, long B,
-            int N, int K, int keep, uint8_t *__restrict__ idx_final, const int *__restrict__ nact) {
+__device__ __forceinline__ void
+tf_pair0s_body(unsigned bid, const float *__restrict__ G, const uint8_t *__restrict__ idx, const float *__restrict__ E, const TfLists &L,
+               long B, int N, int K, int keep, uint8_t *__restrict__ idx_final, const int *__restrict__ nact) {
     constexpr int KC = 16, VPL = 4;
     __shared__ u64 scratch[kSelectLdsU64];
     Stamps stp;
     if (nact) B = *nact;
     const int Gout = N >> 1;
-    const int g = (int)(blockIdx.x & (unsigned)(Gout - 1));
-    const long b = (long)(blockIdx.x >> __builtin_ctz((unsigned)Gout));
+    const int g = (int)(bid & (unsigned)(Gout - 1));
+    const long b = (long)(bid >> __builtin_ctz((unsigned)Gout));
     if (b >= B) return;
     const int lane = lane_id();
     const int n = 2 * g, m = n + 1;
@@ -489,7 +519,22 @@
     stp.at(2);
     tf_finish<VPL, uint8_t, kSlotMajor>(sv, sp, keep, KC, scratch, L, 1, b, N, g, idx_final);
     stp.at(3);
-    stp.flush(1, blockIdx.x, 64);
+    stp.flush(1, bid, 64);
+}
+
+template <bool STRIDED = false>
+__global__ void __launch_bounds__(64)
+k_tf_pair0s(const float *__restrict__ G, const uint8_t *__restrict__ idx, const float *__restrict__ E, TfLists L, long B,
+            int N, int K, int keep, uint8_t *__restrict__ idx_final, const int *__restrict__ nact) {
+    if constexpr (!STRIDED) {
+        tf_pair0s_body(blockIdx.x, G, idx, E, L, B, N, K, keep, idx_final, nact);
+        return;
+    }
+    const unsigned need = nact ? (unsigned)*nact * (unsigned)(N >> 1) : gridDim.x;
+    for (unsigned c = blockIdx.x; c < need; c += gridDim.x) {
+        tf_pair0s_body(c, G, idx, E, L, B, N, K, keep, idx_final, nact);
+        wave_lds_fence();
+    }
 }
 
 template <int KCH, int KC, typename CT = uint8_t>
@@ -748,15 +793,31 @@
     tf_table1_body<KCH, KC, CT>(blockIdx.x, leaf, G, idx, L, B, N, K, ntab, per, tabs, nact);
 }
 
-template <int KCH, int KC, typename CT = uint8_t>
+template <int KCH, int KC, typename CT = uint8_t, bool STRIDED = false>
 __global__ void __launch_bounds__(64)
 k_tf_level1(const float *__restrict__ G, const CT *__restrict__ idx, const float *__restrict__ E, TfLists L, long B, int N,
             int K, int keep, int ntab, int per, float *__restrict__ tabs, const int *__restrict__ nact, unsigned pair_blocks,
-            unsigned tab_blocks, int ntab2, int per2, float *__restrict__ tabs2) {
+            unsigned tab_blocks, int ntab2, int per2, float *__restrict__ tabs2, unsigned vgrid) {
     __shared__ __attribute__((aligned(16))) float leaf[tf_leaf_lds_floats(KCH, sizeof(CT))];
-    if (blockIdx.x < pair_blocks) tf_pair1_body<KCH, KC, CT>(blockIdx.x, leaf, G, idx, E, L, B, N, K, keep, nullptr, nact);
-    else if (blockIdx.x < pair_blocks + tab_blocks) tf_table1_body<KCH, KC, CT>(blockIdx.x - pair_blocks, leaf, G, idx, L, B, N, K, ntab, per, tabs, nact);
-    else tf_table1_body<KCH, KC, CT>(blockIdx.x - pair_blocks - tab_blocks, leaf, G, idx, L, B, N, K, ntab2, per2, tabs2, nact);
+    if constexpr (!STRIDED) {
+        if (blockIdx.x < pair_blocks) tf_pair1_body<KCH, KC, CT>(blockIdx.x, leaf, G, idx, E, L, B, N, K, keep, nullptr, nact);
+        else if (blockIdx.x < pair_blocks + tab_blocks) tf_table1_body<KCH, KC, CT>(blockIdx.x - pair_blocks, leaf, G, idx, L, B, N, K, ntab, per, tabs, nact);
+        else tf_table1_body<KCH, KC, CT>(blockIdx.x - pair_blocks - tab_blocks, leaf, G, idx, L, B, N, K, ntab2, per2, tabs2, nact);
+        return;
+    }
+    unsigned r0 = pair_blocks, r1 = tab_blocks, r2 = vgrid - pair_blocks - tab_blocks;
+    if (nact) {
+        const unsigned na = (unsigned)*nact;
+        r0 = (na * (unsigned)(N / 4) + 7u) & ~7u;
+        r1 = (na * (unsigned)ntab + 7u) & ~7u;
+        r2 = r2 ? na * (unsigned)ntab2 : 0u;
+    }
+    for (unsigned c = blockIdx.x; c < r0 + r1 + r2; c += gridDim.x) {
+        if (c < r0) tf_pair1_body<KCH, KC, CT>(c, leaf, G, idx, E, L, B, N, K, keep, nullptr, nact);
+        else if (c < r0 + r1) tf_table1_body<KCH, KC, CT>(c - r0, leaf, G, idx, L, B, N, K, ntab, per, tabs, nact);
+        else tf_table1_body<KCH, KC, CT>(c - r0 - r1, leaf, G, idx, L, B, N, K, ntab2, per2, tabs2, nact);
+        wave_lds_fence();
+    }
 }
 
 template <int KH>
@@ -843,9 +904,9 @@
 }
 
 template <int KH, int KC, bool LAST, typename CT = uint8_t>
-__global__ void __launch_bounds__(64)
-k_tf_comb(const float *__restrict__ E, TfLists L, long B, int N, int v, int keep, const float *__restrict__ tabs,
-          CT *__restrict__ idx_final, const int *__restrict__ nact) {
+__device__ __forceinline__ void
+tf_comb_body(unsigned bid, const float *__restrict__ E, const TfLists &L, long B, int N, int v, int keep, const float *__restrict__ tabs,
+             CT *__restrict__ idx_final, const int *__restrict__ nact) {
     constexpr int MH = KH * KH, RS = KH + 1, TS = tf_tab_stride<KH>();
     constexpr int VPL = (KC * KC / 64 <= 16) ? KC * KC / 64 : 16;
     constexpr int CHUNKS = KC * KC / (64 * VPL);
@@ -856,8 +917,8 @@
     u64 *sel2 = sel2_store;
     if (nact) B = *nact;
     const int Gout = N >> (v + 1);
-    const int h = (int)(blockIdx.x & (unsigned)(Gout - 1));
-    const long b = (long)(blockIdx.x >> __builtin_ctz((unsigned)Gout));
+    const int h = (int)(bid & (unsigned)(Gout - 1));
+    const long b = (long)(bid >> __builtin_ctz((unsigned)Gout));
     if (b >= B) return;
     const int lane = lane_id();
     const int P = 2 * h, Q = P + 1, Gv = N >> v;
@@ -927,6 +988,21 @@
         wave_lexmin(bv, bp);
         if (bp > KC * KC - 1) bp = KC * KC - 1;
         tf_emit(L, b, N, v + 1, bp, idx_final);
+    }
+}
+
+template <int KH, int KC, bool LAST, typename CT = uint8_t, bool STRIDED = false>
+__global__ void __launch_bounds__(64)
+k_tf_comb(const float *__restrict__ E, TfLists L, long B, int N, int v, int keep, const float *__restrict__ tabs,
+          CT *__restrict__ idx_final, const int *__restrict__ nact) {
+    if constexpr (!STRIDED) {
+        tf_comb_body<KH, KC, LAST, CT>(blockIdx.x, E, L, B, N, v, keep, tabs, idx_final, nact);
+        return;
+    }
+    const unsigned need = nact ? (unsigned)*nact * (unsigned)(N >> (v + 1)) : gridDim.x;
+    for (unsigned c = blockIdx.x; c < need; c += gridDim.x) {
+        tf_comb_body<KH, KC, LAST, CT>(c, E, L, B, N, v, keep, tabs, idx_final, nact);
+        wave_lds_fence();
     }
 }
 
diff --git a/quantization_amd/quantizer.py b/quantization_amd/quantizer.py
--- a/quantization_amd/quantizer.py
+++ b/quantization_amd/quantizer.py
@@ -77,7 +77,7 @@
         id_bytes = binascii.b2a_hex(os.urandom(4))
         self.id_str = id_bytes.decode("utf-8")
         self.register_buffer("id_buf", torch.tensor(list(id_bytes), dtype=torch.uint8))
-        self.skip_fixed_points = False
+        self.skip_fixed_points = True
         self._pinned_scales = None
         self._prep = None
         self._ws = None
@@ -258,7 +258,7 @@
             rc = L.mcq_encode_ex(x2d.data_ptr(), B, blob.data_ptr(), self._lscale_exp, N, K, D, int(iters),
                                  out.data_ptr() if as_bytes else None, None if as_bytes else out.data_ptr(),
                                  ws.data_ptr(), ws.numel(), st,
-                                 (1 if getattr(self, "skip_fixed_points", False) else 0) | self._scale_flags |
+                                 (0 if getattr(self, "skip_fixed_points", True) else _lib.MCQ_ENCODE_ALL_PASSES) | self._scale_flags |
                                  (4 if x_fp16 else 0))
         _lib.check(rc, "mcq_encode")
         return out
```
